# noway/nzcb-circom

Measured on AMD Instinct MI355X. Metric: PLONK proofs/sec for nzcp_live (~2^21 constraints) at 1/2/4/8 MI355X, higher is better.
Workload: dtype u32 limbs: BN254 Fr/Fq Montgomery, 8x32-bit and 9x29-bit (MSM, NTT twiddles, quotient); 1 GPU; nzcp_live fullProve: NZCPPubIdentity(1,351,0,4,2,4) witness on the GPU (600560 signals) + PLONK proof, n=2^21, nPublic=3, 2970 inputs; domain_size=2097152, n_public=3, n_constraints=1785813, n_vars=1782570, n_additions=1182010, proofs_per_gpu=140, total_proofs=140, parallelism=batch-shard x1 (no collective), proofs_in_flight_per_gpu=5

## Files before the change

### include/nzcb_internal.h

```cpp
#ifndef NZCB_INTERNAL_H
#define NZCB_INTERNAL_H

#include "nzcb.h"

#ifdef __cplusplus
extern "C" {
#endif

int nzcb_ctx_kernel_stats(nzcb_ctx* ctx, int enable, double out[4]);

int nzcb_debug_guard_check(int device, size_t* checked, int* damaged, nzcb_err* err);
int nzcb_debug_guard_selftest(int device, nzcb_err* err);

#define NZCB_FAULT_QUOTIENT 1
#define NZCB_DEBUG_GENERIC_K 2
#define NZCB_FAULT_LANE_ALLOC 3
int nzcb_debug_inject_fault(nzcb_ctx* ctx, int kind);

int nzcb_debug_signal_basis_cap(int per_constraint);
int nzcb_debug_signal_basis_info(const nzcb_ctx* ctx, uint64_t out[7]);
int nzcb_debug_commit_abc(nzcb_ctx* ctx, const uint8_t* witness, size_t n_witness, const uint8_t* blinding,
                          int signal_basis, uint8_t* out, nzcb_err* err);
int nzcb_debug_signal_rows(nzcb_ctx* ctx, int set, uint8_t* rows_out, uint32_t* signals_out, size_t cap,
                           nzcb_err* err);

int nzcb_debug_f29(int device, int op, const uint32_t* in, size_t count, uint32_t* out, nzcb_err* err);

int nzcb_debug_grand_product(int device, const uint8_t* abc , const uint8_t* sigma ,
                             const uint8_t* x , size_t n, const uint8_t* beta, const uint8_t* gamma,
                             const uint8_t* k1, const uint8_t* k2, int generic_k, uint8_t* z_out ,
                             uint8_t* totals_out , nzcb_err* err);
int nzcb_debug_div_pol1(int device, const uint8_t* p , size_t m, const uint8_t* d, const uint8_t* p0_adjust,
                        uint8_t* q_out , int* divides_out, nzcb_err* err);
int nzcb_debug_eval_many(int device, int np, const uint8_t* const* polys, const size_t* lens,
                         const uint8_t* xs , uint8_t* out , nzcb_err* err);
int nzcb_debug_quotient(int device, int power, int three, uint32_t npub, const uint8_t* abcz ,
                        const uint8_t* q , const uint8_t* s ,
                        const uint8_t* l , const uint8_t* apub , const uint8_t* beta,
                        const uint8_t* gamma, const uint8_t* alpha, const uint8_t* k1, const uint8_t* k2,
                        uint8_t* t_out , nzcb_err* err);

int nzcb_synth_setup(int power, int n_public, int n_inputs, uint64_t seed, uint32_t n_constraints,
                     const uint8_t* tau, int device, uint8_t** zkey_out, size_t* zkey_len, uint8_t** wtns_out,
                     size_t* wtns_len, nzcb_err* err);
#define NZCB_SYNTH_FREE_PUBLIC 1u
int nzcb_synth_setup_ex(int power, int n_public, int n_inputs, uint64_t seed, uint32_t n_constraints, uint32_t flags,
                        const uint8_t* tau, int device, uint8_t** zkey_out, size_t* zkey_len, uint8_t** wtns_out,
                        size_t* wtns_len, nzcb_err* err);
typedef struct nzcb_engine nzcb_engine;
nzcb_engine* nzcb_engine_create(int device, int max_log_ntt, size_t max_msm_points, nzcb_err* err);
void nzcb_engine_destroy(nzcb_engine* e);
int nzcb_engine_ntt(nzcb_engine* e, const uint8_t* in_lem, uint8_t* out_lem, int log_n, int inverse, nzcb_err* err);
int nzcb_engine_msm(nzcb_engine* e, const uint8_t* bases_lem, const uint8_t* scalars, size_t n, int scalars_mont,
                    uint8_t* out_affine, nzcb_err* err);
int nzcb_debug_ntt_coset(nzcb_engine* e, const uint8_t* in_lem, uint8_t* out_lem, int log_n, const uint8_t* c_lem,
                         int fold_len, nzcb_err* err);
int nzcb_engine_ntt_dev(nzcb_engine* e, const void* in, void* out, int log_n, int inverse, nzcb_err* err);
int nzcb_engine_msm_dev(nzcb_engine* e, const void* bases, const void* scalars, size_t n, int scalars_mont,
                        uint8_t* out_affine, nzcb_err* err);
int nzcb_engine_time_ntt(nzcb_engine* e, const void* in, void* out, int log_n, int inverse, int reps, double* ms,
                         nzcb_err* err);
int nzcb_engine_random_fr(nzcb_engine* e, void* dev_out, size_t n, uint64_t seed, nzcb_err* err);
int nzcb_engine_fixed_base(nzcb_engine* e, const void* dev_scalars_mont, size_t n, void* dev_out, nzcb_err* err);
int nzcb_engine_lagrange_basis(nzcb_engine* e, const void* dev_ptau, size_t ptau_n, int log_n, void* dev_out,
                               nzcb_err* err);
int nzcb_engine_time_msm(nzcb_engine* e, const void* bases, const void* scalars, size_t n, int scalars_mont, int reps,
                         double* ms, double* acc_ms, nzcb_err* err);
int nzcb_engine_msm_fixed_dev(nzcb_engine* e, const void* bases, size_t n_table, const void* scalars, size_t n,
                              int scalars_mont, uint8_t* out_affine, nzcb_err* err);
int nzcb_engine_msm_table_dev(nzcb_engine* e, const void* bases, size_t n_table, const void* scalars, size_t n,
                              int scalars_mont, int window, int sparse, int fold, uint8_t* out_affine,
                              nzcb_err* err);
int nzcb_debug_msm_plan(nzcb_engine* e, const void* bases, size_t n_table, const void* scalars, size_t n,
                        int scalars_mont, int window, int fold, uint32_t* info, uint32_t* offsets, size_t offsets_cap,
                        uint32_t* seg, size_t seg_cap, uint8_t* out_affine, nzcb_err* err);
int nzcb_engine_msm_sets_dev(nzcb_engine* e, const void* bases, size_t n_table, const void* const* scalars, int sets,
                             size_t n, int scalars_mont, int sparse, uint8_t* out_affine, nzcb_err* err);
int nzcb_engine_time_msm2(nzcb_engine* e, const void* bases, const void* scalars, size_t n, int scalars_mont,
                          int fixed_base, int reps, double* out, nzcb_err* err);
int nzcb_engine_fr_mul(nzcb_engine* e, const uint8_t* a_lem, const uint8_t* b_lem, uint8_t* out_lem, size_t n,
                       int field_q, nzcb_err* err);

int nzcb_engine_g1_lincomb(int device, const uint8_t* points, const uint8_t* scalars, const uint32_t* group_end,
                           size_t groups, uint8_t* out, nzcb_err* err);
int nzcb_engine_verify_batch(const uint8_t* vk, const uint8_t* proofs, const uint8_t* pubs, size_t pub_stride,
                             int n_public, int count, int transcript_public, int device, const uint8_t* seed,
                             int* valid_out, uint8_t* points_out, int* pairing_checks, nzcb_err* err);
int nzcb_debug_verify_batch_timings(double* ms, int cap);

nzcb_r1cs* nzcb_engine_r1cs_create(const uint8_t* r1cs, size_t len, int device, uint32_t long_row_threshold,
                                   int witness_tile, nzcb_err* err);
int nzcb_debug_r1cs_check_timings(double* ms, int cap);

nzcb_p256_key* nzcb_engine_p256_key_create(const uint8_t pub_xy[64], int device, int window, nzcb_err* err);
#define NZCB_P256_OP_ADD 0
#define NZCB_P256_OP_SUB 1
#define NZCB_P256_OP_MUL 2
#define NZCB_P256_OP_SQR 3
#define NZCB_P256_OP_INV 4
int nzcb_debug_p256_field(int device, int op, int field, const uint8_t* a, const uint8_t* b, size_t count,
                          uint8_t* out, nzcb_err* err);
int nzcb_debug_p256_mul2(nzcb_p256_key* k, const uint8_t* u1, const uint8_t* u2, size_t count, uint8_t* out_xy,
                         nzcb_err* err);
int nzcb_debug_p256_timings(double* ms, int cap);

int nzcb_debug_nzcp_decode_timings(double* ms, int cap);

int nzcb_engine_srs_check(int device, const uint8_t* points, uint64_t m, const uint8_t* g2, const uint8_t* seed,
                          uint32_t chunk_points, nzcb_key_finding* finding, uint8_t* lr_out ,
                          nzcb_err* err);
int nzcb_debug_key_check_timings(double* ms, int cap);

int nzcb_debug_ptau_timings(double* ms, int cap);
int nzcb_debug_ptau_batch_top(int level);

int nzcb_engine_groth16_rows(int device, int g2, const void* points, uint64_t n_points, const uint64_t* row_off,
                             uint64_t n_rows, const uint32_t* idx, const uint8_t* coefs, uint8_t* out,
                             nzcb_err* err);
int nzcb_debug_groth16_schedule(int chunk, int fan_in, int* prev_chunk, int* prev_fan_in);
int nzcb_debug_groth16_timings(double* out, int cap);

#ifdef __cplusplus
}
#endif
#endif
```

### nzcb-circom_amd/csrc/prover.hip

```cpp
#include <rocprofiler-sdk-roctx/roctx.h>
#include "devcall.h"
#include "lagrange.h"
#include "prover.h"
#include "sigbasis.h"
#include "transcript.h"

#include <cstring>
#include <cerrno>
#include <string>
#include <sys/random.h>

#include "keccak.h"

namespace nzcb {

static constexpr int kT = 256;
static constexpr uint32_t kZeroRef = 0xffffffffu;

__global__ void k_wit_to_mont(const Fr* __restrict__ in, Fr* __restrict__ out, size_t n) {
  size_t i = (size_t)blockIdx.x * blockDim.x + threadIdx.x;
  if (i >= n) return;
  out[i] = (i == 0) ? Fr::zero() : to_mont(in[i]);
}

__global__ void k_additions(const AddRec* __restrict__ recs, uint32_t count, Fr* __restrict__ wit) {
  uint32_t i = blockIdx.x * blockDim.x + threadIdx.x;
  if (i >= count) return;
  const AddRec r = recs[i];
  Fr a = r.ai == kZeroRef ? Fr::zero() : wit[r.ai];
  Fr b = r.bi == kZeroRef ? Fr::zero() : wit[r.bi];
  wit[r.dst] = r.ac * a + r.bc * b;
}


__global__ void k_build_abc(const uint32_t* __restrict__ am, const uint32_t* __restrict__ bm,
                            const uint32_t* __restrict__ cm, uint32_t nc, uint32_t n, const Fr* __restrict__ wit,
                            uint32_t nvars, Fr* __restrict__ A, Fr* __restrict__ B, Fr* __restrict__ C,
                            uint32_t npub, Fr* __restrict__ mb_apub, Fr* __restrict__ mb_pubw) {
  uint32_t i = blockIdx.x * blockDim.x + threadIdx.x;
  if (i < npub) {
    host_put(mb_pubw + i, 1 + i < nvars ? wit[1 + i] : Fr::zero());
  }
  if (i >= n) {
    if (i < npub) host_put_done();
    return;
  }
  Fr a = Fr::zero(), b = Fr::zero(), c = Fr::zero();
  if (i < nc) {
    uint32_t ia = am[i], ib = bm[i], ic = cm[i];
    if (ia < nvars) a = wit[ia];
    if (ib < nvars) b = wit[ib];
    if (ic < nvars) c = wit[ic];
  }
  A[i] = a;
  B[i] = b;
  C[i] = c;
  if (i < npub) {
    host_put(mb_apub + i, a);
    host_put_done();
  }
}

__global__ void k_tops(const Fr* __restrict__ pa, const Fr* __restrict__ pb, const Fr* __restrict__ pc,
                       const Fr* __restrict__ pz, size_t n, const uint32_t* __restrict__ flags, Fr* __restrict__ mb) {
  const int t = threadIdx.x;
  if (t < 24) {
    const int k = t / 6, j = t % 6;
    const Fr* src = k == 0 ? pa + (n - 4) : k == 1 ? pb + (n - 4) : k == 2 ? pc + (n - 4) : pz + (n - 3);
    host_put(mb + t, src[j]);
  } else if (t == 24) {
    Fr f = Fr::zero();
    f.v[0] = *flags;
    host_put(mb + 24, f);
  }
  host_put_done();
}

struct BlindIdx {
  int idx[3];
  int count;
};

__global__ void k_blind(Fr* pol, size_t n, const Fr* __restrict__ bl, BlindIdx bi) {
  if (threadIdx.x != 0 || blockIdx.x != 0) return;
  for (int k = 0; k < bi.count; k++) {
    Fr b = bl[bi.idx[k]];
    pol[n + k] = b;
    pol[k] = pol[k] - b;
  }
}

__global__ void k_abc_tail(Fr* A, Fr* B, Fr* C, size_t n, const Fr* __restrict__ bl) {
  if (threadIdx.x != 0 || blockIdx.x != 0) return;
  A[n] = bl[2];
  A[n + 1] = bl[1];
  B[n] = bl[4];
  B[n + 1] = bl[3];
  C[n] = bl[6];
  C[n + 1] = bl[5];
}

__global__ void k_sig_stage(const uint32_t* __restrict__ idx, uint32_t stride, uint32_t c0, uint32_t c1, uint32_t c2,
                            const Fr* __restrict__ wit, const Fr* __restrict__ bl, Fr* __restrict__ out) {
  const size_t i = (size_t)blockIdx.x * blockDim.x + threadIdx.x;
  if (i >= (size_t)3 * stride) return;
  const uint32_t set = (uint32_t)(i / stride), j = (uint32_t)(i - (size_t)set * stride);
  const uint32_t cnt = set == 0 ? c0 : set == 1 ? c1 : c2;
  Fr v = Fr::zero();
  if (j < cnt) v = from_mont(wit[idx[i]]);
  else if (j == cnt) v = from_mont(bl[2 + 2 * set]);
  else if (j == cnt + 1) v = from_mont(bl[1 + 2 * set]);
  out[i] = v;
}

static bool signal_commit_enabled() {
  static const bool v = [] {
    const char* e = std::getenv("NZCB_SIGNAL_COMMIT");
    return !e || std::atoi(e) != 0;
  }();
  return v;
}

static bool abc_sets_enabled() {
  static const bool v = [] {
    const char* e = std::getenv("NZCB_ABC_SETS");
    return !e || std::atoi(e) != 0;
  }();
  return v;
}

static bool lagrange_commit_enabled() {
  static const bool v = [] {
    const char* e = std::getenv("NZCB_LAGRANGE_COMMIT");
    return !e || std::atoi(e) != 0;
  }();
  return v;
}

__device__ __forceinline__ Fr root4(const Fr* __restrict__ lo, const Fr* __restrict__ hi, size_t i) {
  return lo[i & 4095] * hi[i >> 12];
}

struct PermArgs {
  F29 beta, beta_s;
  F29 k1beta, k1beta_s, k2beta, k2beta_s;
  F29 gamma256;
  int k23;
};
static void shoup_pair(const Fr& c, F29& w, F29& ws) {
  Fr m = c;
  for (int k = 0; k < 5; k++) m = m + m;
  w = split29(from_mont(c));
  ws = mul_lo261(split29(m), f29_const(Fr29::NINV));
}

static F29 fr29_operand(Fr c) {
  for (int k = 0; k < 5; k++) c = c + c;
  return split29(c);
}

#ifndef NZ_KPER
#define NZ_KPER 4
#endif
static constexpr int kPer = NZ_KPER;
static constexpr int kTileN = kT * kPer;
static constexpr int kStageWords = kTileN * 8 + kTileN / 4;

__device__ __forceinline__ int stage_word(int e) { return e * 8 + e / 4; }

template <class F, class U>
__device__ __forceinline__ void stage_use(F&& f, size_t base, size_t len, uint32_t* lds, U&& use) {
#pragma unroll
  for (int k = 0; k < kPer; k++) {
    const int e = k * kT + (int)threadIdx.x;
    const size_t g = base + (size_t)e;
    const Fr v = g < len ? f(g) : Fr::zero();
#pragma unroll
    for (int w = 0; w < 8; w++) lds[stage_word(e) + w] = v.v[w];
  }
  __syncthreads();
#pragma unroll
  for (int j = 0; j < kPer; j++) {
    const int e = kPer * (int)threadIdx.x + j;
    Fr x;
#pragma unroll
    for (int w = 0; w < 8; w++) x.v[w] = lds[stage_word(e) + w];
    use(j, x);
  }
  __syncthreads();
}
template <class F>
__device__ __forceinline__ void stage_in(F&& f, size_t base, size_t len, uint32_t* lds, Fr (&out)[kPer]) {
  stage_use(f, base, len, lds, [&](int j, const Fr& x) { out[j] = x; });
}

__device__ __forceinline__ void stage_out(const Fr (&v)[kPer], size_t base, size_t len, uint32_t* lds, Fr* dst) {
#pragma unroll
  for (int j = 0; j < kPer; j++) {
    const int e = kPer * (int)threadIdx.x + j;
#pragma unroll
    for (int w = 0; w < 8; w++) lds[stage_word(e) + w] = v[j].v[w];
  }
  __syncthreads();
#pragma unroll
  for (int k = 0; k < kPer; k++) {
    const int e = k * kT + (int)threadIdx.x;
    const size_t g = base + (size_t)e;
    Fr x;
#pragma unroll
    for (int w = 0; w < 8; w++) x.v[w] = lds[stage_word(e) + w];
    if (g < len) dst[g] = x;
  }
  __syncthreads();
}

__device__ __forceinline__ Fr shfl_fr(const Fr& v, int src) {
  Fr o;
#pragma unroll
  for (int w = 0; w < 8; w++) o.v[w] = __shfl(v.v[w], src, 64);
  return o;
}
__device__ __forceinline__ F29 shfl_fr(const F29& v, int src) {
  F29 o;
#pragma unroll
  for (int w = 0; w < 9; w++) o.v[w] = __shfl(v.v[w], src, 64);
  return o;
}
struct MulOp {
  using T = Fr;
  static constexpr bool kCheap = false;
  __device__ Fr operator()(const Fr& a, const Fr& b) const { return a * b; }
  __device__ static Fr id() { return Fr::one(); }
};
struct AddOp {
  using T = Fr;
  static constexpr bool kCheap = true;
  __device__ Fr operator()(const Fr& a, const Fr& b) const { return a + b; }
  __device__ static Fr id() { return Fr::zero(); }
};
struct Mul29Op {
  using T = F29;
  static constexpr bool kCheap = false;
  __device__ F29 operator()(const F29& a, const F29& b) const { return mul29<Fr29>(a, b); }
  __device__ static F29 id() { return f29_const(Fr29::ONE); }
};
template <bool kSuffix, class Op, int NT = kT>
__device__ __forceinline__ typename Op::T block_scan_excl(const typename Op::T& v, typename Op::T* sh,
                                                          typename Op::T* total) {
  using T = typename Op::T;
  constexpr int NW = NT / 64;
  static_assert(NW >= 1 && NW <= 64 && NT % 64 == 0, "whole waves, at most 64");
  const Op op;
  const int lane = (int)(threadIdx.x & 63), wv = (int)(threadIdx.x >> 6);
  T inc = v;
#pragma unroll
  for (int d = 1; d < 64; d <<= 1) {
    const int src = kSuffix ? lane + d : lane - d;
    const T o = shfl_fr(inc, src & 63);
    if (kSuffix ? lane + d < 64 : lane >= d) inc = op(inc, o);
  }
  T ex = shfl_fr(inc, (kSuffix ? lane + 1 : lane - 1) & 63);
  if (kSuffix ? lane == 63 : lane == 0) ex = Op::id();
  if (kSuffix ? lane == 0 : lane == 63) sh[wv] = inc;
  __syncthreads();
  if constexpr (NW <= 4 && Op::kCheap) {
#pragma unroll
    for (int k = 0; k < NW; k++)
      if (kSuffix ? k > wv : k < wv) ex = op(ex, sh[k]);
    if (total && threadIdx.x == 0) {
      T t = sh[0];
#pragma unroll
      for (int k = 1; k < NW; k++) t = op(t, sh[k]);
      *total = t;
    }
    __syncthreads();
  } else {
    T tot_all = Op::id();
    if (wv == 0) {
      T w = lane < NW ? sh[lane] : Op::id();
#pragma unroll
      for (int d = 1; d < NW; d <<= 1) {
        const int src = kSuffix ? lane + d : lane - d;
        const T o = shfl_fr(w, src & 63);
        if (kSuffix ? lane + d < NW : (lane >= d && lane < NW)) w = op(w, o);
      }
      T wex = shfl_fr(w, (kSuffix ? lane + 1 : lane - 1) & 63);
      if (kSuffix ? lane == NW - 1 : lane == 0) wex = Op::id();
      tot_all = shfl_fr(w, kSuffix ? 0 : NW - 1);
      if (lane < NW) sh[lane] = wex;
    }
    __syncthreads();
    ex = op(ex, sh[wv]);
    if (total && threadIdx.x == 0) *total = tot_all;
    __syncthreads();
  }
  return ex;
}
__device__ __forceinline__ Fr block_prod_excl(const Fr& v, Fr* sh, Fr& total) {
  return block_scan_excl<false, MulOp>(v, sh, &total);
}
__device__ __forceinline__ Fr block_prod_excl_suffix(const Fr& v, Fr* sh) {
  return block_scan_excl<true, MulOp>(v, sh, nullptr);
}
__device__ __forceinline__ Fr block_sum_excl_suffix(const Fr& v, Fr* sh, Fr& total) {
  return block_scan_excl<true, AddOp>(v, sh, &total);
}

#ifndef NZ_PERM_WAVES
#define NZ_PERM_WAVES 2
#endif
__device__ __forceinline__ F29 add3_nn29(const F29& a, const F29& b, const F29& c) {
  F29 r;
#pragma unroll
  for (int l = 0; l < 9; l++) r.v[l] = a.v[l] + b.v[l] + c.v[l];
  return r;
}
__global__ void __launch_bounds__(kT) __attribute__((amdgpu_waves_per_eu(NZ_PERM_WAVES, 8)))
k_perm_tile(const Fr* __restrict__ A, const Fr* __restrict__ B, const Fr* __restrict__ C,
            const Fr* __restrict__ sig_h, size_t n, const Fr* __restrict__ w_h, PermArgs pa, Fr* __restrict__ Z,
            Fr* __restrict__ ntot, Fr* __restrict__ dtot) {
  __shared__ uint32_t stg[kStageWords];
  __shared__ F29 sh[kT / 64];
  const int tid = threadIdx.x;
  const size_t base = (size_t)blockIdx.x * kTileN;
  const size_t e0 = base + (size_t)kPer * tid;
  const F29 beta = pa.beta, beta_s = pa.beta_s, gamma = pa.gamma256;
  const bool k23 = pa.k23 != 0;
  F29 num[kPer], den[kPer], bw[kPer], bs[kPer];
#pragma unroll 1
  for (int k = 0; k < 3; k++) {
    stage_use([&](size_t g) { return sig_h[(size_t)k * n + g]; }, base, n, stg,
              [&](int j, const Fr& x) { bs[j] = mul_shoup(split29(x), beta, beta_s); });
    if (k == 0 || !k23) {
      const F29 kb = k == 0 ? beta : (k == 1 ? pa.k1beta : pa.k2beta);
      const F29 kbs = k == 0 ? beta_s : (k == 1 ? pa.k1beta_s : pa.k2beta_s);
#pragma unroll
      for (int j = 0; j < kPer; j++) bw[j] = mul_shoup(split29(e0 + j < n ? w_h[e0 + j] : Fr::zero()), kb, kbs);
    }
    const Fr* col = k == 0 ? A : B;
    if (k == 2) col = C;
    stage_use([&](size_t g) { return col[g]; }, base, n, stg,
              [&](int j, const Fr& x) {
                F29 kbw = bw[j];
                if (k23 && k == 1) {
#pragma unroll
                  for (int l = 0; l < 9; l++) kbw.v[l] = bw[j].v[l] << 1;
                } else if (k23 && k == 2) {
#pragma unroll
                  for (int l = 0; l < 9; l++) kbw.v[l] = (bw[j].v[l] << 1) + bw[j].v[l];
                }
                const F29 xs = split29(x);
                if (k == 0) {
                  num[j] = add3_29(xs, kbw, gamma);
                  den[j] = add3_29(xs, bs[j], gamma);
                } else {
                  num[j] = mul29<Fr29>(num[j], add3_nn29(xs, kbw, gamma));
                  den[j] = mul29<Fr29>(den[j], add3_nn29(xs, bs[j], gamma));
                }
              });
  }
  const F29 one = f29_const(Fr29::ONE);
#pragma unroll
  for (int j = 0; j < kPer; j++)
    if (e0 + j >= n) num[j] = den[j] = one;
  F29 ntl = num[0];
#pragma unroll
  for (int j = 1; j < kPer; j++) ntl = mul29<Fr29>(ntl, num[j]);
  bs[kPer - 1] = den[kPer - 1];
#pragma unroll
  for (int j = kPer - 2; j >= 0; j--) bs[j] = mul29<Fr29>(bs[j + 1], den[j]);
  F29 nt;
  const F29 np = block_scan_excl<false, Mul29Op>(ntl, sh, &nt);
  const F29 ds = block_scan_excl<true, Mul29Op>(bs[0], sh, nullptr);
  F29 pre = mul29<Fr29>(mul29<Fr29>(np, ds), f29_const(Fr29::C256));
  Fr out[kPer];
#pragma unroll
  for (int j = 0; j < kPer; j++) {
    out[j] = join_fr29(mul29<Fr29>(pre, bs[j]));
    if (j + 1 < kPer) pre = mul29<Fr29>(pre, num[j]);
  }
  stage_out(out, base, n, stg, Z);
  if (tid == 0) {
    ntot[blockIdx.x] = fr_from261(nt);
    dtot[blockIdx.x] = fr_from261(mul29<Fr29>(ds, bs[0]));
  }
}

__global__ void __launch_bounds__(1024)
k_perm_factors(const Fr* __restrict__ ntot, const Fr* __restrict__ dtot, int ntiles, Fr* __restrict__ F,
               Fr* __restrict__ totals) {
  __shared__ Fr sh[1024 / 64];
  const int tid = threadIdx.x;
  const int per = (ntiles + 1023) / 1024;
  const int t0 = min(tid * per, ntiles), t1 = min(t0 + per, ntiles);
  Fr pn = Fr::one(), pd = Fr::one();
  for (int t = t0; t < t1; t++) {
    pn = pn * ntot[t];
    pd = pd * dtot[t];
  }
  Fr nall, dall;
  const Fr npre = block_scan_excl<false, MulOp, 1024>(pn, sh, &nall);
  const Fr dsuf = block_scan_excl<true, MulOp, 1024>(pd, sh, &dall);
  if (tid == 0) {
    host_put(totals, nall);
    host_put(totals + 1, dall);
    host_put_done();
  }
  Fr run = npre;
  for (int t = t0; t < t1; t++) {
    F[t] = run;
    run = run * ntot[t];
  }
  Fr sd = dsuf;
  for (int t = t1 - 1; t >= t0; t--) {
    F[t] = F[t] * sd;
    sd = sd * dtot[t];
  }
}

__global__ void __launch_bounds__(kT)
k_apply_tiles(Fr* __restrict__ x, size_t m, const Fr* __restrict__ F, Fr inv_d) {
  const Fr f = F[blockIdx.x] * inv_d;
  const size_t base = (size_t)blockIdx.x * kTileN + threadIdx.x;
#pragma unroll
  for (int k = 0; k < kPer; k++) {
    const size_t i = base + (size_t)k * kT;
    if (i < m) x[i] = x[i] * f;
  }
}

struct LinTab {
  Fr P[kT + 1];
  Fr Pinv[kT + 1];
  Fr dp[kPer + 1];
};
static_assert(sizeof(LinTab) % sizeof(Fr) == 0, "LinTab is stored as Fr words");

template <bool kWrite>
__global__ void __launch_bounds__(kT)
k_lin_tile(const Fr* __restrict__ src, size_t m, const LinTab* __restrict__ tab, const Fr* __restrict__ carry,
           Fr* __restrict__ out) {
  __shared__ uint32_t stg[kStageWords];
  __shared__ Fr sh[kT / 64];
  const int tid = threadIdx.x;
  const size_t base = (size_t)blockIdx.x * kTileN;
  Fr x[kPer];
  stage_in([&](size_t g) { return src[g + 1]; }, base, m - 1, stg, x);
  const Fr d = tab->dp[1];
  Fr y = Fr::zero();
#pragma unroll
  for (int j = kPer - 1; j >= 0; j--) {
    y = x[j] + d * y;
    x[j] = y;
  }
  Fr total;
  Fr ex = block_sum_excl_suffix(y * tab->P[tid], sh, total);
  if (!kWrite) {
    if (tid == 0) out[blockIdx.x] = total;
    return;
  }
  if (carry) ex = ex + carry[blockIdx.x + 1] * tab->P[kT];
  const Fr next = ex * tab->Pinv[tid + 1];
#pragma unroll
  for (int j = 0; j < kPer; j++) x[j] = x[j] + tab->dp[kPer - j] * next;
  stage_out(x, base, m, stg, out);
}

__global__ void k_pow_tiles(Fr D, Fr Di, int count, Fr* __restrict__ Q, Fr* __restrict__ Qinv) {
  const int T = blockIdx.x * blockDim.x + threadIdx.x;
  if (T >= count) return;
  Fr a = Fr::one(), b = Fr::one(), pa = D, pb = Di;
  for (int e = T; e; e >>= 1) {
    if (e & 1) {
      a = a * pa;
      b = b * pb;
    }
    pa = sqr(pa);
    pb = sqr(pb);
  }
  Q[T] = a;
  Qinv[T] = b;
}

__global__ void __launch_bounds__(1024) k_tile_heads(Fr* __restrict__ h, int m, const Fr* __restrict__ Q,
                                                     const Fr* __restrict__ Qinv) {
  __shared__ Fr sh[1024 / 64];
  const int tid = threadIdx.x;
  const int per = (m + 1023) / 1024;
  const int t0 = min(tid * per, m), t1 = min(t0 + per, m);
  Fr run = Fr::zero();
  for (int T = t0; T < t1; T++) run = run + h[T] * Q[T];
  Fr suf = block_scan_excl<true, AddOp, 1024>(run, sh, nullptr);
  for (int T = t1 - 1; T >= t0; T--) {
    suf = suf + h[T] * Q[T];
    h[T] = suf * Qinv[T];
  }
  if (tid == 0) h[m] = Fr::zero();
}

__global__ void k_stride4(const Fr* __restrict__ src, size_t n, Fr* __restrict__ dst) {
  const size_t i = (size_t)blockIdx.x * blockDim.x + threadIdx.x;
  if (i < n) dst[i] = src[4 * i];
}

struct QArgs {
  Fr beta, gamma, alpha, alpha2, bk1, bk2;
  Fr zhinv[4];
};

__global__ void __launch_bounds__(kT)
k_quotient_coset(const Fr* __restrict__ A, const Fr* __restrict__ B, const Fr* __restrict__ C,
                 const Fr* __restrict__ Z, const Fr* __restrict__ cq, const Fr* __restrict__ cs,
                 const Fr* __restrict__ cl, uint32_t npub, const Fr* __restrict__ Apub, size_t n,
                 const Fr* __restrict__ xlo, const Fr* __restrict__ xhi, QArgs q, Fr* __restrict__ T) {
  const size_t n4 = 4 * n;
  size_t i = (size_t)blockIdx.x * blockDim.x + threadIdx.x;
  if (i >= n4) return;
  const Fr a = A[i], b = B[i], c = C[i];
  const Fr x = xlo[i & 4095] * xhi[i >> 12];
  Fr gate = a * b * cq[i] + a * cq[n4 + i] + b * cq[2 * n4 + i] + c * cq[3 * n4 + i] + cq[4 * n4 + i];
  for (uint32_t j = 0; j < npub; j++) gate = gate - cl[j * n4 + i] * Apub[j];
  const Fr z = Z[i];
  const Fr bx = q.beta * x;
  Fr num = (a + bx + q.gamma) * (b + q.bk1 * x + q.gamma);
  num = num * (c + q.bk2 * x + q.gamma) * z;
  Fr den = (a + q.beta * cs[i] + q.gamma) * (b + q.beta * cs[n4 + i] + q.gamma);
  den = den * (c + q.beta * cs[2 * n4 + i] + q.gamma) * Z[(i + 4) & (n4 - 1)];
  const Fr e4 = (z - Fr::one()) * cl[i] * q.alpha2;
  T[i] = (gate + q.alpha * (num - den) + e4) * q.zhinv[i & 3];
}

constexpr uint32_t kQ29MaxPub = 8;

static bool quot3_enabled() {
  static const bool on = [] {
    const char* e = std::getenv("NZCB_QUOT3");
    return !(e && e[0] == '0');
  }();
  return on;
}
struct QArgs29 {
  F29 beta, bk1, bk2, alpha2, zhinv[4];
  F29 gamma, negone;
  int k23;
  F29 alpha;
};

template <int K>
__device__ __forceinline__ F29 q29_pi_chunk(const Fr* __restrict__ cl, const Fr* __restrict__ Apub, uint32_t j0,
                                            size_t n4, size_t i) {
  F29 pa[K], pb[K];
#pragma unroll
  for (int k = 0; k < K; k++) {
    pa[k] = split29(cl[(size_t)(j0 + k) * n4 + i]);
    pb[k] = split29(neg(Apub[j0 + k]));
  }
  return mulsum29<Fr29, K>(pa, pb);
}

__device__ __forceinline__ F29 q29_pi(const Fr* __restrict__ cl, const Fr* __restrict__ Apub, uint32_t j0,
                                      uint32_t cnt, size_t n4, size_t i) {
  switch (cnt) {
    case 1: return q29_pi_chunk<1>(cl, Apub, j0, n4, i);
    case 2: return q29_pi_chunk<2>(cl, Apub, j0, n4, i);
    case 3: return q29_pi_chunk<3>(cl, Apub, j0, n4, i);
    default: return q29_pi_chunk<4>(cl, Apub, j0, n4, i);
  }
}

template <bool THREE>
__global__ void __launch_bounds__(kT) __attribute__((amdgpu_waves_per_eu(4, 8)))
k_quotient_coset29(const Fr* __restrict__ A, const Fr* __restrict__ B, const Fr* __restrict__ C,
                   const Fr* __restrict__ Z, const Fr* __restrict__ cq, const Fr* __restrict__ cs,
                   const Fr* __restrict__ cl, uint32_t npub, const Fr* __restrict__ Apub, size_t n,
                   const Fr* __restrict__ xlo, const Fr* __restrict__ xhi, const Fr* __restrict__ bxlo, QArgs29 q,
                   Fr* __restrict__ T) {
  const size_t n4 = (THREE ? 3 : 4) * n;
  size_t i = (size_t)blockIdx.x * blockDim.x + threadIdx.x;
  if (i >= n4) return;
  size_t ix, izw;
  int cj;
  if (THREE) {
    const int lg = __ffsll((long long)n) - 1;
    const size_t j = i >> lg, m = i & (n - 1);
    ix = 4 * m + j;
    izw = j * n + ((m + 1) & (n - 1));
    cj = (int)j;
  } else {
    ix = i;
    izw = (i + 4) & (n4 - 1);
    cj = (int)(i & 3);
  }
  const F29 a = split29(A[i]), b = split29(B[i]), c = split29(C[i]);
  F29 gate;
  {
    const F29 ga[4] = {mul29<Fr29>(a, b), a, b, c};
    const F29 gb[4] = {split29(cq[i]), split29(cq[n4 + i]), split29(cq[2 * n4 + i]), split29(cq[3 * n4 + i])};
    gate = add29(mulsum29<Fr29, 4>(ga, gb), split29(cq[4 * n4 + i]));
  }
  if (npub > 0) gate = add29(gate, q29_pi(cl, Apub, 0, npub < 4 ? npub : 4, n4, i));
  if (npub > 4) gate = add29(gate, q29_pi(cl, Apub, 4, npub - 4, n4, i));
  const F29 z = split29(Z[i]);
  const bool bxt = THREE && q.k23;
  const F29 x = mul29<Fr29>(split29((bxt ? bxlo : xlo)[ix & 4095]), split29(xhi[ix >> 12]));
  const F29 bx = bxt ? x : mul29<Fr29>(q.beta, x);
  const F29 bx2 = q.k23 ? add29(bx, bx) : mul29<Fr29>(q.bk1, x);
  const F29 bx3 = q.k23 ? add29(bx2, bx) : mul29<Fr29>(q.bk2, x);
  const F29 f1 = add29(add29(a, bx), q.gamma);
  const F29 f2 = add29(add29(b, bx2), q.gamma);
  const F29 f3 = add29(add29(c, bx3), q.gamma);
  const F29 num = mul29<Fr29>(mul29<Fr29>(mul29<Fr29>(f1, f2), f3), z);
  const F29 g1 = add29(add29(a, mul29<Fr29>(q.beta, split29(cs[i]))), q.gamma);
  const F29 g2 = add29(add29(b, mul29<Fr29>(q.beta, split29(cs[n4 + i]))), q.gamma);
  const F29 g3 = add29(add29(c, mul29<Fr29>(q.beta, split29(cs[2 * n4 + i]))), q.gamma);
  const F29 den = mul29<Fr29>(mul29<Fr29>(mul29<Fr29>(g1, g2), g3), split29(Z[izw]));
  const F29 pa[2] = {q.alpha, q.alpha2};
  const F29 pb[2] = {sub29(num, den, Fr29::K2), mul29<Fr29>(add29(z, q.negone), split29(cl[i]))};
  const F29 S = add29(gate, mulsum29<Fr29, 2>(pa, pb));
  T[i] = THREE ? canon_fr29(S) : join_fr29(mul29<Fr29>(S, q.zhinv[cj]));
}

__global__ void __launch_bounds__(kT)
k_beta_xlo(const Fr* __restrict__ xlo, F29 beta, size_t count, Fr* __restrict__ bxlo) {
  const size_t i = (size_t)blockIdx.x * blockDim.x + threadIdx.x;
  if (i < count) bxlo[i] = join_fr29(mul29<Fr29>(beta, split29(xlo[i])));
}

__global__ void __launch_bounds__(kT)
k_gate_h(const Fr* __restrict__ A, const Fr* __restrict__ B, const Fr* __restrict__ C, const Fr* __restrict__ qh,
         size_t n, uint32_t npub, uint32_t* __restrict__ flags) {
  const size_t m = (size_t)blockIdx.x * blockDim.x + threadIdx.x;
  if (m >= n) return;
  const Fr a = A[m], b = B[m], c = C[m];
  Fr g = qh[m] * a * b + qh[n + m] * a + qh[2 * n + m] * b + qh[3 * n + m] * c + qh[4 * n + m];
  if (m < npub) g = g - a;
  if (!g.is_zero()) atomicOr(flags, 1u);
}

struct T3Args {
  Fr c0[6], c1[6], c2[6], q3[6];
  Fr i4, two_over_d, inv_d2;
};
__global__ void __launch_bounds__(kT)
k_t_combine(const Fr* __restrict__ V, size_t n, T3Args a, Fr* __restrict__ t) {
  const size_t k = (size_t)blockIdx.x * blockDim.x + threadIdx.x;
  if (k >= n) return;
  Fr v0 = V[k], v1 = V[n + k], v2 = V[2 * n + k];
  if (k < 6) {
    v0 = v0 - a.c0[k];
    v1 = v1 - a.c1[k];
    v2 = v2 - a.c2[k];
  }
  const Fr sm = v0 + v2, dl = v0 - v2, im = dl * a.i4, v12 = v1 + v1;
  t[k] = sm + v12 - im;
  t[n + k] = dl * a.two_over_d;
  t[2 * n + k] = (sm - v12 + im) * a.inv_d2;
  if (k < 6) t[3 * n + k] = a.q3[k];
}

__global__ void k_root_n(Fr* __restrict__ out, const Fr* __restrict__ rlo, const Fr* __restrict__ rhi, size_t n) {
  const size_t i = (size_t)blockIdx.x * blockDim.x + threadIdx.x;
  if (i < n) out[i] = root4(rlo, rhi, 4 * i);
}

__global__ void k_fault_bump(Fr* x) {
  if (threadIdx.x == 0) x[0] = x[0] + Fr::one();
}

__global__ void k_dbl_pow(Fr* __restrict__ x, size_t m, int e) {
  size_t i = (size_t)blockIdx.x * blockDim.x + threadIdx.x;
  if (i >= m) return;
  Fr v = x[i];
  for (int k = 0; k < e; k++) v = v + v;
  x[i] = v;
}

static F29 f29_exp(Fr v, int extra) {
  for (int k = 0; k < extra; k++) v = v + v;
  return split29(v);
}

static constexpr int kEvalMax = 8;
static constexpr int kEvalBits = 16;
struct EvalSet {
  const Fr* p[kEvalMax];
  uint64_t len[kEvalMax];
  Fr x[kEvalMax];
  Fr x4096[kEvalMax];
  F29 x29[kEvalMax];
  F29 y29[kEvalMax];
  int np;
  int nbits;
};

__device__ __forceinline__ F29 fr29_operand_dev(Fr c) {
#pragma unroll
  for (int k = 0; k < 5; k++) c = c + c;
  return split29(c);
}

static constexpr int kEvalChunk2 = 16;

__global__ void __launch_bounds__(kT) k_eval_pows(EvalSet es, F29* __restrict__ pw, Fr* __restrict__ pw2) {
  const int j = blockIdx.x, t = threadIdx.x;
  Fr a = Fr::one(), q = es.x[j];
  for (int e = t; e; e >>= 1) {
    if (e & 1) a = a * q;
    q = q * q;
  }
  pw[(size_t)j * kT + t] = fr29_operand_dev(a);
  if (t < es.nbits) {
    Fr z = es.x4096[j];
    for (int k = 0; k < t; k++) z = z * z;
    pw2[j * kEvalBits + t] = z;
  }
}

__device__ __forceinline__ Fr block_sum_fr(const Fr& v, Fr* sh) {
  Fr x = v;
#pragma unroll
  for (int m = 32; m >= 1; m >>= 1) x = x + shfl_fr(x, (int)(threadIdx.x & 63) ^ m);
  if ((threadIdx.x & 63) == 0) sh[threadIdx.x >> 6] = x;
  __syncthreads();
  Fr t = sh[0];
#pragma unroll
  for (int k = 1; k < kT / 64; k++) t = t + sh[k];
  __syncthreads();
  return t;
}

template <int NP>
__global__ void __launch_bounds__(kT) k_eval_multi(EvalSet es, const F29* __restrict__ pw, const Fr* __restrict__ pw2,
                                                   Fr* __restrict__ partial, int nblocks) {
  static_assert(NP <= kEvalMax && kEvalMax <= 4 * (kT / 64), "one 16-lane group per point");
  __shared__ Fr sh[kT / 64];
  __shared__ Fr bpow[kEvalMax];
  __shared__ Fr bsum[kEvalMax];
  {
    const int l = (int)(threadIdx.x & 63), k = l & 15, j = 4 * (int)(threadIdx.x >> 6) + (l >> 4);
    Fr f = Fr::one();
    if (j < NP && k < es.nbits && ((blockIdx.x >> k) & 1u)) f = pw2[j * kEvalBits + k];
    for (int m = 8; m >= 1; m >>= 1) f = f * shfl_fr(f, l ^ m);
    if (j < NP && k == 0) bpow[j] = f;
  }
  const size_t s = (size_t)blockIdx.x * kT * kEvalChunk2 + threadIdx.x;
  F29 acc[NP];
#pragma unroll
  for (int j = 0; j < NP; j++)
#pragma unroll
    for (int l = 0; l < 9; l++) acc[j].v[l] = 0;
  for (int m = kEvalChunk2 - 1; m >= 0; m--) {
    const size_t i = s + (size_t)m * kT;
#pragma unroll
    for (int j = 0; j < NP; j++)
      if (i < es.len[j]) {
        const F29 t = mul29<Fr29>(acc[j], es.y29[j]), c = split29(es.p[j][i]);
#pragma unroll
        for (int l = 0; l < 9; l++) acc[j].v[l] = t.v[l] + c.v[l];
      }
  }
#pragma unroll
  for (int j = 0; j < NP; j++) {
    const Fr r = block_sum_fr(join_fr29(mul29<Fr29>(acc[j], pw[(size_t)j * kT + threadIdx.x])), sh);
    if (threadIdx.x == 0) bsum[j] = r;
  }
  if (threadIdx.x < NP) partial[(size_t)threadIdx.x * nblocks + blockIdx.x] = bsum[threadIdx.x] * bpow[threadIdx.x];
}

__global__ void __launch_bounds__(kT) k_eval_sum(const Fr* __restrict__ partial, int nblocks, Fr* __restrict__ out) {
  __shared__ Fr sh[kT / 64];
  const int j = blockIdx.x;
  Fr acc = Fr::zero();
  for (int b = (int)threadIdx.x; b < nblocks; b += kT) acc = acc + partial[(size_t)j * nblocks + b];
  const Fr r = block_sum_fr(acc, sh);
  if (threadIdx.x == 0) {
    host_put(out + j, r);
    host_put_done();
  }
}

struct RArgs {
  Fr coefz, coef_ab, ea, eb, ec, coefs3;
};

__global__ void k_pol_r(const Fr* __restrict__ pz, const Fr* __restrict__ qm, const Fr* __restrict__ ql,
                        const Fr* __restrict__ qr, const Fr* __restrict__ qo, const Fr* __restrict__ qc,
                        const Fr* __restrict__ s3, size_t n, RArgs r, Fr* __restrict__ out) {
  size_t i = (size_t)blockIdx.x * blockDim.x + threadIdx.x;
  if (i >= n + 3) return;
  Fr v = r.coefz * pz[i];
  if (i < n) {
    v = v + r.coef_ab * qm[i] + r.ea * ql[i] + r.eb * qr[i] + r.ec * qo[i] + qc[i];
    v = v - r.coefs3 * s3[i];
  }
  out[i] = v;
}

struct WArgs {
  Fr xim, xi2m, v[7], w0sub;
};

__global__ void k_pol_wxi(const Fr* __restrict__ t, const Fr* __restrict__ pr, const Fr* __restrict__ pa,
                          const Fr* __restrict__ pb, const Fr* __restrict__ pc, const Fr* __restrict__ s1,
                          const Fr* __restrict__ s2, size_t n, WArgs wa, Fr* __restrict__ out) {
  size_t i = (size_t)blockIdx.x * blockDim.x + threadIdx.x;
  if (i >= n + 6) return;
  Fr w = wa.xi2m * t[2 * n + i];
  if (i < n) w = w + wa.xim * t[n + i] + t[i];
  if (i < n + 3) w = w + wa.v[1] * pr[i];
  if (i < n + 2) w = w + wa.v[2] * pa[i] + wa.v[3] * pb[i] + wa.v[4] * pc[i];
  if (i < n) w = w + wa.v[5] * s1[i] + wa.v[6] * s2[i];
  if (i == 0) w = w - wa.w0sub;
  out[i] = w;
}

__global__ void k_div_check(const Fr* __restrict__ src, Fr p0_adjust, const Fr* __restrict__ q, Fr d,
                            uint32_t* flags, uint32_t bit, uint32_t* __restrict__ mb_flags) {
  if (threadIdx.x || blockIdx.x) return;
  Fr p0 = src[0] - p0_adjust;
  if (!(p0 + d * q[0]).is_zero()) atomicOr(flags, bit);
  host_put(mb_flags, *flags);
  host_put_done();
}

__global__ void k_root_table(Fr* __restrict__ out, Fr base, Fr scale, size_t count) {
  size_t i = (size_t)blockIdx.x * blockDim.x + threadIdx.x;
  if (i >= count) return;
  out[i] = scale * pow_u64(base, i);
}

__global__ void k_factor29_table(F29* __restrict__ out, const Fr* __restrict__ lo, const Fr* __restrict__ hi, Fr scale,
                                 size_t count) {
  size_t i = (size_t)blockIdx.x * blockDim.x + threadIdx.x;
  if (i >= count) return;
  Fr v = lo[i & 4095] * hi[i >> 12] * scale;
#pragma unroll
  for (int k = 0; k < 5; k++) v = v + v;
  out[i] = split29(v);
}

static std::string fr_dec(const Fr& m) {
  Fr x = from_mont(m);
  uint32_t v[8];
  std::memcpy(v, x.v, 32);
  std::string s;
  bool nz = true;
  while (nz) {
    uint64_t rem = 0;
    nz = false;
    for (int i = 7; i >= 0; i--) {
      uint64_t cur = (rem << 32) | v[i];
      v[i] = (uint32_t)(cur / 10);
      rem = cur % 10;
      if (v[i]) nz = true;
    }
    s.push_back((char)('0' + rem));
  }
  return std::string(s.rbegin(), s.rend());
}

static Fr fr_small(uint64_t k) {
  Fr x = Fr::zero();
  x.v[0] = (uint32_t)k;
  x.v[1] = (uint32_t)(k >> 32);
  return to_mont(x);
}

static bool k_is_23(const Fr& k1, const Fr& k2) { return k1 == fr_small(2) && k2 == fr_small(3); }

static PermArgs perm_args(const Fr& beta, const Fr& gamma, const Fr& k1, const Fr& k2, bool generic_k) {
  PermArgs pa;
  shoup_pair(beta, pa.beta, pa.beta_s);
  shoup_pair(k1 * beta, pa.k1beta, pa.k1beta_s);
  shoup_pair(k2 * beta, pa.k2beta, pa.k2beta_s);
  pa.gamma256 = f29_exp(gamma, 0);
  pa.k23 = !generic_k && k_is_23(k1, k2) ? 1 : 0;
  return pa;
}

static size_t perm_tiles(size_t n) { return (n + kTileN - 1) / kTileN; }

static void perm_launch(const Fr* A, const Fr* B, const Fr* C, const Fr* sig_h, size_t n, const Fr* w_h,
                        const PermArgs& pa, Fr* Z, Fr* scan, Fr* totals, hipStream_t s) {
  const size_t ntiles = perm_tiles(n);
  if (ntiles > 1024 * 64) throw Error(NZCB_ERR_INTERNAL, "round 2: domain too large for the tile factors");
  Fr* ntot = scan;
  Fr* dtot = ntot + ntiles;
  Fr* fac = dtot + ntiles;
  hipLaunchKernelGGL(k_perm_tile, dim3((unsigned)ntiles), dim3(kT), 0, s, A, B, C, sig_h, n, w_h, pa, Z, ntot, dtot);
  hipLaunchKernelGGL(k_perm_factors, dim3(1), dim3(1024), 0, s, (const Fr*)ntot, (const Fr*)dtot, (int)ntiles, fac,
                     totals);
  NZ_HIP(hipGetLastError());
}

static void perm_apply(Fr* Z, size_t n, const Fr* scan, const Fr& den_total, hipStream_t s) {
  const size_t ntiles = perm_tiles(n);
  hipLaunchKernelGGL(k_apply_tiles, dim3((unsigned)ntiles), dim3(kT), 0, s, Z, n, scan + 2 * ntiles,
                     inverse(den_total));
  NZ_HIP(hipGetLastError());
}

static QArgs quot_args(const Fr& beta, const Fr& gamma, const Fr& alpha, const Fr& k1, const Fr& k2,
                       const Fr (&zh_inv)[4]) {
  QArgs q;
  q.beta = beta;
  q.gamma = gamma;
  q.alpha = alpha;
  q.alpha2 = alpha * alpha;
  q.bk1 = beta * k1;
  q.bk2 = beta * k2;
  for (int k = 0; k < 4; k++) q.zhinv[k] = zh_inv[k];
  return q;
}
static QArgs29 quot_args29(const Fr& beta, const Fr& gamma, const Fr& alpha, const Fr& k1, const Fr& k2,
                           const Fr (&zh_inv)[4]) {
  QArgs29 q29;
  q29.beta = f29_exp(beta, 5);
  q29.k23 = k_is_23(k1, k2) ? 1 : 0;
  q29.bk1 = f29_exp(beta * k1, 5);
  q29.bk2 = f29_exp(beta * k2, 5);
  q29.alpha2 = f29_exp(alpha * alpha, 5);
  for (int k = 0; k < 4; k++) q29.zhinv[k] = f29_exp(zh_inv[k], 5);
  q29.gamma = f29_exp(gamma, 0);
  q29.negone = f29_exp(neg(Fr::one()), 0);
  q29.alpha = f29_exp(alpha, 20);
  return q29;
}

static void root_table(DevBuf<Fr>& out, size_t cnt, const Fr& base, const Fr& scale, hipStream_t s) {
  out.alloc(cnt);
  hipLaunchKernelGGL(k_root_table, dim3(grid_for(cnt, kT)), dim3(kT), 0, s, out.p, base, scale, cnt);
  NZ_HIP(hipGetLastError());
}

static void quot_x_tables(int power, DevBuf<Fr>& x_lo, DevBuf<Fr>& root_hi, Fr (&zh_inv)[4], hipStream_t s) {
  const size_t n = (size_t)1 << power, n4 = 4 * n;
  const Fr w4 = fr_root_of_unity(power + 2), g = fr_small(5), one = Fr::one();
  root_table(x_lo, 4096, w4, g, s);
  root_table(root_hi, (n4 + 4095) / 4096, pow_u64(w4, 4096), one, s);
  Fr gn = pow_u64(g, n), w4n = pow_u64(w4, n), p = gn;
  for (int k = 0; k < 4; k++) {
    zh_inv[k] = inverse(p - one);
    p = p * w4n;
  }
}

static void quot29_prescale(Fr* cq, Fr* cl, uint32_t nl, size_t npts, Fr* x_lo, hipStream_t s) {
  auto scale = [&](Fr* p, size_t m, int e) {
    hipLaunchKernelGGL(k_dbl_pow, dim3(grid_for(m, kT, 1u << 30)), dim3(kT), 0, s, p, m, e);
  };
  scale(cq, npts, 10);
  scale(cq + npts, 3 * npts, 5);
  scale(cl, (size_t)nl * npts, 5);
  scale(x_lo, 4096, 5);
  NZ_HIP(hipGetLastError());
}

static void quot_launch(bool three, const Fr* A4, const Fr* B4, const Fr* C4, const Fr* Z4, const Fr* cq, const Fr* cs,
                        const Fr* cl, uint32_t npub, const Fr* Apub, size_t n, const Fr* x_lo, const Fr* root_hi,
                        Fr* bx_lo, const Fr& beta, const Fr& gamma, const Fr& alpha, const Fr& k1, const Fr& k2,
                        const Fr (&zh_inv)[4], Fr* T, hipStream_t s) {
  if (three && npub > kQ29MaxPub) throw Error(NZCB_ERR_INTERNAL, "round 3: three cosets with too many public inputs");
  if (npub > kQ29MaxPub) {
    const QArgs q = quot_args(beta, gamma, alpha, k1, k2, zh_inv);
    hipLaunchKernelGGL(k_quotient_coset, dim3(grid_for(4 * n, kT, 1u << 30)), dim3(kT), 0, s, A4, B4, C4, Z4, cq, cs,
                       cl, npub, Apub, n, x_lo, root_hi, q, T);
  } else {
    const QArgs29 q29 = quot_args29(beta, gamma, alpha, k1, k2, zh_inv);
    if (three) {
      if (q29.k23)
        hipLaunchKernelGGL(k_beta_xlo, dim3(grid_for(4096, kT)), dim3(kT), 0, s, x_lo, q29.beta, (size_t)4096, bx_lo);
      hipLaunchKernelGGL((k_quotient_coset29<true>), dim3(grid_for(3 * n, kT, 1u << 30)), dim3(kT), 0, s, A4, B4, C4,
                         Z4, cq, cs, cl, npub, Apub, n, x_lo, root_hi, (const Fr*)bx_lo, q29, T);
    } else {
      hipLaunchKernelGGL((k_quotient_coset29<false>), dim3(grid_for(4 * n, kT, 1u << 30)), dim3(kT), 0, s, A4, B4, C4,
                         Z4, cq, cs, cl, npub, Apub, n, x_lo, root_hi, (const Fr*)nullptr, q29, T);
    }
  }
  NZ_HIP(hipGetLastError());
}

static EvalSet eval_set(int np, const Fr* const* polys, const size_t* lens, const Fr* xs, size_t* nblocks_out) {
  if (np < 1 || np > kEvalMax) throw Error(NZCB_ERR_INTERNAL, "eval_many: bad count");
  EvalSet es{};
  size_t maxlen = 0;
  for (int j = 0; j < np; j++) {
    es.p[j] = polys[j];
    es.len[j] = lens[j];
    es.x[j] = xs[j];
    es.x29[j] = fr29_operand(xs[j]);
    es.y29[j] = fr29_operand(pow_u64(xs[j], kT));
    es.x4096[j] = pow_u64(xs[j], (uint64_t)kT * kEvalChunk2);
    maxlen = std::max(maxlen, lens[j]);
  }
  es.np = np;
  const size_t nblocks = (maxlen + (size_t)kT * kEvalChunk2 - 1) / ((size_t)kT * kEvalChunk2);
  if (nblocks > ((size_t)1 << kEvalBits)) throw Error(NZCB_ERR_INTERNAL, "eval_many: polynomial too long");
  es.nbits = 1;
  while (((size_t)1 << es.nbits) < nblocks) es.nbits++;
  *nblocks_out = nblocks;
  return es;
}

static void eval_launch(const EvalSet& es, size_t nblocks, Fr* part, F29* pw, Fr* pw2, Fr* out, hipStream_t s) {
  const int np = es.np;
  hipLaunchKernelGGL(k_eval_pows, dim3((unsigned)np), dim3(kT), 0, s, es, pw, pw2);
  if (np == 7)
    hipLaunchKernelGGL(k_eval_multi<7>, dim3((unsigned)nblocks), dim3(kT), 0, s, es, (const F29*)pw, (const Fr*)pw2,
                       part, (int)nblocks);
  else if (np == 1)
    hipLaunchKernelGGL(k_eval_multi<1>, dim3((unsigned)nblocks), dim3(kT), 0, s, es, (const F29*)pw, (const Fr*)pw2,
                       part, (int)nblocks);
  else
    throw Error(NZCB_ERR_INTERNAL, "eval_many: 1 or 7 evaluations");
  NZ_HIP(hipGetLastError());
  hipLaunchKernelGGL(k_eval_sum, dim3(np), dim3(kT), 0, s, (const Fr*)part, (int)nblocks, out);
  NZ_HIP(hipGetLastError());
}

static void lin_tables_build(LinTab& t, const Fr& d, LinTab* dev, Fr* q, int qn, hipStream_t s) {
  t.dp[0] = Fr::one();
  for (int j = 1; j <= kPer; j++) t.dp[j] = t.dp[j - 1] * d;
  const Fr dk = t.dp[kPer], dki = inverse(dk);
  t.P[0] = t.Pinv[0] = Fr::one();
  for (int i = 1; i <= kT; i++) {
    t.P[i] = t.P[i - 1] * dk;
    t.Pinv[i] = t.Pinv[i - 1] * dki;
  }
  NZ_HIP(hipMemcpyAsync(dev, &t, sizeof(LinTab), hipMemcpyHostToDevice, s));
  hipLaunchKernelGGL(k_pow_tiles, dim3((qn + 255) / 256), dim3(256), 0, s, t.P[kT], t.Pinv[kT], qn, q, q + qn);
  NZ_HIP(hipGetLastError());
}

static size_t lin_tiles(size_t m) { return (m + kTileN - 1) / kTileN; }

static void div_pol1_launch(const Fr* src, size_t m, const LinTab* lt, const Fr& d, const Fr* q, size_t qn, Fr* heads,
                            const Fr& p0_adjust, Fr* dst, uint32_t* flags, uint32_t flag_bit, uint32_t* mb_flags,
                            hipStream_t s) {
  const size_t ntiles = lin_tiles(m);
  if (ntiles + 1 > qn) throw Error(NZCB_ERR_INTERNAL, "divPol1: more tiles than its power tables");
  hipLaunchKernelGGL(k_lin_tile<false>, dim3((unsigned)ntiles), dim3(kT), 0, s, src, m, lt, (const Fr*)nullptr, heads);
  hipLaunchKernelGGL(k_tile_heads, dim3(1), dim3(1024), 0, s, heads, (int)ntiles, q, q + qn);
  NZ_HIP(hipGetLastError());
  hipLaunchKernelGGL(k_lin_tile<true>, dim3((unsigned)ntiles), dim3(kT), 0, s, src, m, lt, (const Fr*)heads, dst);
  hipLaunchKernelGGL(k_div_check, dim3(1), dim3(64), 0, s, src, p0_adjust, (const Fr*)dst, d, flags, flag_bit,
                     mb_flags);
  NZ_HIP(hipGetLastError());
}

Prover::~Prover() {
  for (int i = 0; i < kSlots; i++) {
    if (aux[i]) {
      (void)hipStreamSynchronize(aux[i]);
      (void)hipStreamDestroy(aux[i]);
    }
    if (ready[i]) (void)hipEventDestroy(ready[i]);
  }
  if (side_ready) (void)hipEventDestroy(side_ready);
  if (side_done) (void)hipEventDestroy(side_done);
  if (pows_done) (void)hipEventDestroy(pows_done);
  if (top_host) (void)hipHostFree(top_host);
  for (auto& e : span_ev) {
    (void)hipEventDestroy(e.first);
    (void)hipEventDestroy(e.second);
  }
}

size_t Prover::span_begin(int kind, hipStream_t s) {
  if (spans_used == span_ev.size()) {
    hipEvent_t a, b;
    NZ_HIP(hipEventCreate(&a));
    NZ_HIP(hipEventCreate(&b));
    span_ev.emplace_back(a, b);
    span_kind.push_back(0);
  }
  span_kind[spans_used] = kind;
  NZ_HIP(hipEventRecord(span_ev[spans_used].first, s));
  return spans_used++;
}
void Prover::span_end(size_t i, hipStream_t s) { NZ_HIP(hipEventRecord(span_ev[i].second, s)); }
void Prover::span_totals(double* msm_ms, double* ntt_ms) {
  *msm_ms = *ntt_ms = 0;
  for (size_t i = 0; i < spans_used; i++) {
    NZ_HIP(hipEventSynchronize(span_ev[i].second));
    float ms = 0;
    NZ_HIP(hipEventElapsedTime(&ms, span_ev[i].first, span_ev[i].second));
    (span_kind[i] ? *ntt_ms : *msm_ms) += ms;
  }
}

MsmShard::~MsmShard() {
  (void)hipSetDevice(device);
  for (auto& s : st)
    if (s) {
      (void)hipStreamSynchronize(s);
      (void)hipStreamDestroy(s);
    }
}

void Prover::set_msm_devices(const std::vector<int>& devices) {
  GuardScope guards;
  if (devices.empty() || devices[0] != eng->device)
    throw Error(NZCB_ERR_ARG, "msm devices must start with the context's device");
  shards.clear();
  own_hi = own_lhi = 0;
  const size_t N = ptau.n;
  const size_t L = lcommit ? ltau.n : 0;
  const size_t k = devices.size();
  if (k == 1) return;
  own_hi = N / k;
  own_lhi = L / k;
  for (size_t i = 1; i < k; i++) {
    auto sh = std::make_unique<MsmShard>();
    sh->device = devices[i];
    sh->lo = N * i / k;
    sh->hi = N * (i + 1) / k;
    sh->llo = L * i / k;
    sh->lhi = L * (i + 1) / k;
    const size_t cnt = sh->hi - sh->lo, lcnt = sh->lhi - sh->llo, mx = std::max(cnt, lcnt);
    NZ_HIP(hipSetDevice(sh->device));
    for (int j = 0; j < MsmShard::kSlots; j++) {
      NZ_HIP(hipStreamCreateWithFlags(&sh->st[j], hipStreamNonBlocking));
      sh->sc[j].reset(new MsmScratch());
      sh->sc[j]->init(mx, true, 1, false);
      sh->scal[j].alloc(mx);
    }
    {
      DevBuf<G1Affine> part(cnt);
      NZ_HIP(hipMemcpyPeerAsync(part.p, sh->device, ptau.p + sh->lo, eng->device, cnt * sizeof(G1Affine), sh->st[0]));
      sh->table.build(part.p, cnt, fixed_base_window(), sh->st[0]);
      NZ_HIP(hipStreamSynchronize(sh->st[0]));
    }
    if (lcnt) {
      DevBuf<G1Affine> part(lcnt);
      NZ_HIP(hipMemcpyPeerAsync(part.p, sh->device, ltau.p + sh->llo, eng->device, lcnt * sizeof(G1Affine),
                                sh->st[0]));
      sh->ltable.build(part.p, lcnt, lagrange_window(), sh->st[0]);
      sh->ltable.sparse = lagrange_sparse();
      NZ_HIP(hipStreamSynchronize(sh->st[0]));
    }
    shards.push_back(std::move(sh));
  }
  NZ_HIP(hipSetDevice(eng->device));
}

double Prover::ms_since(std::chrono::steady_clock::time_point t0) {
  return std::chrono::duration<double, std::milli>(std::chrono::steady_clock::now() - t0).count();
}

Prover::Prover(const uint8_t* zkey_bytes, size_t len, int device) {
  GuardScope guards;
  Zkey z = parse_zkey(zkey_bytes, len);
  n = z.domainSize;
  n4 = 4 * n;
  power = z.power;
  nVars = z.nVars;
  nPublic = z.nPublic;
  nAdditions = z.nAdditions;
  nConstraints = z.nConstraints;
  if (nAdditions > nVars) throw Error(NZCB_ERR_FORMAT, "nAdditions > nVars");
  nWit = nVars - nAdditions;
  k1 = z.k1;
  k2 = z.k2;
  wn = fr_root_of_unity(power);
  w2 = fr_root_of_unity(2);
  eng.reset(new Engine(device, power + 2, 0));
  init_slots();
  hipStream_t s = st();
  auto up = [&](auto& buf, const Section& sec) {
    using T = typename std::remove_reference<decltype(*buf.p)>::type;
    buf.alloc(sec.len / sizeof(T) ? sec.len / sizeof(T) : 1);
    if (sec.len) NZ_HIP(hipMemcpyAsync(buf.p, sec.p, sec.len, hipMemcpyHostToDevice, s));
  };
  up(ptau, z.ptau);
  ptab.build(ptau.p, ptau.n, fixed_base_window(), s, true);
  lcommit = lagrange_commit_enabled() && ptau.n >= (size_t)n + 2;
  if (lcommit) {
    ltau.alloc((size_t)n + 2);
    lagrange_basis(ptau.p, ptau.n, power, ltau.p, s);
    ltab.build(ltau.p, ltau.n, lagrange_window(), s);
    ltab.sparse = lagrange_sparse();
  }
  up(qm, z.qm);
  up(ql, z.ql);
  up(qr, z.qr);
  up(qo, z.qo);
  up(qc, z.qc);
  up(sigma, z.sigma);
  sig_h.alloc((size_t)3 * n);
  w_h.alloc(n);
  for (int k = 0; k < 3; k++)
    hipLaunchKernelGGL(k_stride4, dim3(grid_for(n, kT, 1u << 30)), dim3(kT), 0, s, sigma.p + (size_t)k * 5 * n + n,
                       (size_t)n, sig_h.p + (size_t)k * n);
  NZ_HIP(hipGetLastError());
  up(lagrange, z.lagrange);
  up(amap, z.amap);
  up(bmap, z.bmap);
  up(cmap, z.cmap);
  {
    std::vector<uint32_t> level(nAdditions, 0);
    std::vector<AddRec> recs(nAdditions);
    uint32_t maxlev = 0;
    for (uint32_t k = 0; k < nAdditions; k++) {
      const uint8_t* p = z.additions.p + (size_t)k * 72;
      AddRec r;
      std::memcpy(&r.ai, p, 4);
      std::memcpy(&r.bi, p + 4, 4);
      std::memcpy(r.ac.v, p + 8, 32);
      std::memcpy(r.bc.v, p + 40, 32);
      r.dst = nWit + k;
      r.pad = 0;
      uint32_t lv = 0;
      for (uint32_t* ref : {&r.ai, &r.bi}) {
        if (*ref >= nVars) *ref = kZeroRef;
        else if (*ref >= nWit) {
          uint32_t kk = *ref - nWit;
          if (kk >= k) *ref = kZeroRef;
          else lv = std::max(lv, level[kk] + 1);
        }
      }
      level[k] = lv;
      maxlev = std::max(maxlev, lv);
      recs[k] = r;
    }
    std::vector<uint32_t> cnt(maxlev + 2, 0);
    for (uint32_t k = 0; k < nAdditions; k++) cnt[level[k] + 1]++;
    for (uint32_t l = 1; l < cnt.size(); l++) cnt[l] += cnt[l - 1];
    add_level_start.assign(cnt.begin(), cnt.end());
    std::vector<AddRec> sorted(nAdditions);
    std::vector<uint32_t> cur(cnt.begin(), cnt.end());
    for (uint32_t k = 0; k < nAdditions; k++) sorted[cur[level[k]]++] = recs[k];
    adds.alloc(nAdditions ? nAdditions : 1);
    if (nAdditions)
      NZ_HIP(hipMemcpyAsync(adds.p, sorted.data(), nAdditions * sizeof(AddRec), hipMemcpyHostToDevice, s));
    NZ_HIP(hipStreamSynchronize(s));
  }
  if (lcommit && signal_commit_enabled() && abc_sets_enabled()) build_signal_basis(z);
  Fr w4 = fr_root_of_unity(power + 2);
  size_t nlo = 4096, nhi = (n4 + 4095) / 4096;
  const Fr one = Fr::one();
  auto table = [&](DevBuf<Fr>& out, size_t cnt, const Fr& base, const Fr& scale) { root_table(out, cnt, base, scale, s); };
  table(root_lo, nlo, w4, one);
  quot_x_tables(power, x_lo, root_hi, zh_inv, s);
  hipLaunchKernelGGL(k_root_n, dim3(grid_for(n, kT, 1u << 30)), dim3(kT), 0, s, w_h.p, root_lo.p, root_hi.p,
                     (size_t)n);
  NZ_HIP(hipGetLastError());
  const Fr g = fr_small(5), gi = inverse(g);
  table(g_lo, nlo, g, one);
  table(g_hi, nhi, pow_u64(g, 4096), one);
  table(gi_lo, nlo, gi, one);
  table(gi_hi, nhi, pow_u64(gi, 4096), one);
  quot3 = quot3_enabled() && nPublic <= kQ29MaxPub && power >= 6;
  {
    const Fr two = one + one;
    g29.alloc((size_t)n + 8);
    hipLaunchKernelGGL(k_factor29_table, dim3(grid_for((size_t)n + 8, kT, 1u << 30)), dim3(kT), 0, s, g29.p, g_lo.p,
                       g_hi.p, one, (size_t)n + 8);
    if (!quot3) {
      gi29.alloc(n4);
      hipLaunchKernelGGL(k_factor29_table, dim3(grid_for(n4, kT, 1u << 30)), dim3(kT), 0, s, gi29.p, gi_lo.p,
                         gi_hi.p, inverse(pow_u64(two, (uint64_t)power + 2)), (size_t)n4);
    }
    NZ_HIP(hipGetLastError());
  }
  alloc_workspace();
  if (quot3) {
    q_h.alloc((size_t)5 * n);
    const DevBuf<Fr>* qs[5] = {&qm, &ql, &qr, &qo, &qc};
    for (int k = 0; k < 5; k++)
      hipLaunchKernelGGL(k_stride4, dim3(grid_for(n, kT, 1u << 30)), dim3(kT), 0, s, qs[k]->p + n, (size_t)n,
                         q_h.p + (size_t)k * n);
    NZ_HIP(hipGetLastError());
  }
  if (quot3) {
    const size_t nhi3 = (n + 4095) / 4096;
    ctw3.alloc((size_t)3 * (n - 1));
    itw3.alloc((size_t)3 * n);
    const Fr inv4n = inverse(fr_small(n4));
    DevBuf<Fr> lo, hi;
    for (int j = 0; j < 3; j++) {
      const Fr cj = g * pow_u64(w4, (uint64_t)j), cji = inverse(cj);
      d3[j] = pow_u64(cj, n);
      ntt_coset_twiddles(eng->ntt_tables, cj, power, ctw3.p + (size_t)j * (n - 1), s);
      table(lo, nlo, cji, one);
      table(hi, nhi3, pow_u64(cji, 4096), one);
      hipLaunchKernelGGL(k_factor29_table, dim3(grid_for(n, kT, 1u << 30)), dim3(kT), 0, s, itw3.p + (size_t)j * n,
                         lo.p, hi.p, inv4n * zh_inv[j], (size_t)n);
      NZ_HIP(hipGetLastError());
      NZ_HIP(hipStreamSynchronize(s));
    }
    for (int k = 0; k < 3; k++)
      NZ_HIP(hipMemcpy(sig_top[k], sigma.p + (size_t)k * 5 * n + (n - 4), 4 * sizeof(Fr), hipMemcpyDeviceToHost));
  }
  if (quot3) {
    const uint32_t nl = nPublic > 0 ? nPublic : 1;
    const size_t n3 = (size_t)3 * n;
    cq3.alloc(5 * n3);
    cs3.alloc(3 * n3);
    cl3.alloc(nl * n3);
    auto coset3 = [&](const Fr* coefs, Fr* out) {
      for (int j = 0; j < 3; j++) {
        NttIo io;
        io.in_len = n;
        io.tw = ctw3.p + (size_t)j * (n - 1);
        ntt(eng->ntt_tables, coefs, out + (size_t)j * n, power, false, s, nullptr, &io);
      }
    };
    const DevBuf<Fr>* qs[5] = {&qm, &ql, &qr, &qo, &qc};
    for (int k = 0; k < 5; k++) coset3(qs[k]->p, cq3.p + (size_t)k * n3);
    for (int k = 0; k < 3; k++) coset3(sigma.p + (size_t)k * 5 * n, cs3.p + (size_t)k * n3);
    for (uint32_t j = 0; j < nl; j++) coset3(lagrange.p + (size_t)j * 5 * n, cl3.p + (size_t)j * n3);
    NZ_HIP(hipGetLastError());
    quot29_prescale(cq3.p, cl3.p, nl, n3, x_lo.p, s);
  } else {
    const uint32_t nl = nPublic > 0 ? nPublic : 1;
    cq.alloc((size_t)5 * n4);
    cs.alloc((size_t)3 * n4);
    cl.alloc((size_t)nl * n4);
    auto coset_eval = [&](const Fr* coefs, Fr* out) {
      NttIo io;
      io.in_len = n;
      io.in_f = g29.p;
      ntt(eng->ntt_tables, coefs, out, power + 2, false, s, nullptr, &io);
    };
    const DevBuf<Fr>* qs[5] = {&qm, &ql, &qr, &qo, &qc};
    for (int k = 0; k < 5; k++) coset_eval(qs[k]->p, cq.p + (size_t)k * n4);
    for (int k = 0; k < 3; k++) coset_eval(sigma.p + (size_t)k * 5 * n, cs.p + (size_t)k * n4);
    for (uint32_t j = 0; j < nl; j++) coset_eval(lagrange.p + (size_t)j * 5 * n, cl.p + (size_t)j * n4);
    NZ_HIP(hipGetLastError());
    if (nPublic <= kQ29MaxPub) quot29_prescale(cq.p, cl.p, nl, n4, x_lo.p, s);
  }
  NZ_HIP(hipStreamSynchronize(s));
}

void Prover::build_signal_basis(const Zkey& z) {
  hipStream_t s = st();
  if (z.additions.len < (uint64_t)nAdditions * 72 || z.amap.len < (uint64_t)nConstraints * 4 ||
      z.bmap.len < (uint64_t)nConstraints * 4 || z.cmap.len < (uint64_t)nConstraints * 4) {
    sig_note = "signal basis: the key's maps are shorter than its header says; A, B, C are committed from the "
               "Lagrange basis";
    return;
  }
  NZ_HIP(hipStreamSynchronize(s));
  SigBasis sb = sig_basis_build(eng->device, ltau.p, n, nWit, nVars, nConstraints, z.additions.p, nAdditions,
                                z.amap.p, z.bmap.p, z.cmap.p, (size_t)n + 2);
  sig_terms = sb.terms;
  if (!sb.ok) {
    sig_note = sb.note;
    return;
  }
  for (int k = 0; k < 3; k++) sig_cnt[k] = sb.cnt[k];
  sig_stride = sb.stride;
  DevBuf<G1Affine> bases(sb.bases.size());
  NZ_HIP(hipMemcpyAsync(bases.p, sb.bases.data(), sb.bases.size() * sizeof(G1Affine), hipMemcpyHostToDevice, s));
  sig_idx.alloc(sb.idx.size());
  NZ_HIP(hipMemcpyAsync(sig_idx.p, sb.idx.data(), sb.idx.size() * sizeof(uint32_t), hipMemcpyHostToDevice, s));
  stab.build(bases.p, bases.n, lagrange_window(), s);
  stab.sparse = lagrange_sparse();
  NZ_HIP(hipStreamSynchronize(s));
  sigcommit = true;
}

void Prover::init_slots() {
  for (int i = 0; i < kSlots; i++) {
    msc[i].reset(new MsmScratch());
#ifdef NZCB_AB_GENERIC
    msc[i]->init((size_t)n + 6, true, i == 0 ? 3 : 1, true);
#else
    msc[i]->init((size_t)n + 6, true, i == 0 ? 3 : 1, false);
#endif
    NZ_HIP(hipStreamCreateWithFlags(&aux[i], hipStreamNonBlocking));
    NZ_HIP(hipEventCreateWithFlags(&ready[i], hipEventDisableTiming));
  }
  NZ_HIP(hipEventCreateWithFlags(&side_ready, hipEventDisableTiming));
  NZ_HIP(hipEventCreateWithFlags(&side_done, hipEventDisableTiming));
  NZ_HIP(hipEventCreateWithFlags(&pows_done, hipEventDisableTiming));
  mb_apub = kMbEvals + kMbEvalMax;
  mb_pubw = mb_apub + nPublic;
  mb_words = mb_pubw + nPublic;
  NZ_HIP(hipHostMalloc((void**)&top_host, mb_words * sizeof(Fr), hipHostMallocCoherent));
  std::memset((void*)top_host, 0, mb_words * sizeof(Fr));
}

void Prover::alloc_workspace() {
  wit.alloc(nVars ? nVars : 1);
  wtns_in.alloc(nWit ? nWit : 1);
  A.alloc(n + 2); B.alloc(n + 2); C.alloc(n + 2); Z.alloc(n);
  if (sigcommit) sig_scal.alloc(3 * sig_stride);
  pol_a.alloc(n + 2); pol_b.alloc(n + 2); pol_c.alloc(n + 2); pol_z.alloc(n + 3);
  const size_t ne = quot3 ? (size_t)3 * n : n4;
  A4.alloc(ne); B4.alloc(ne); C4.alloc(ne); Z4.alloc(ne);
  T.alloc(ne); Tz.alloc(ne); t.alloc(quot3 ? ne + 6 : n4);
  if (quot3) bx_lo.alloc(4096);
  pol_r.alloc(n + 3); pol_wxi.alloc(n + 6); pol_wxiw.alloc(n + 3);
  blind.alloc(13);
  scan_tmp.alloc(3 * ((size_t)n / kTileN + 2) + 64);
  lin_qn = (size_t)n / kTileN + 3;
  lin_tab.alloc(2 * sizeof(LinTab) / sizeof(Fr) + 4 * lin_qn);
  lin_host.resize(2 * sizeof(LinTab) / sizeof(Fr));
  size_t nblocks = ((size_t)3 * n + 6 + (size_t)kT * kEvalChunk2 - 1) / ((size_t)kT * kEvalChunk2) + 1;
  eval_part.alloc((size_t)kEvalMax * nblocks + kEvalMax);
  eval_pw.alloc((size_t)kEvalMax * kT + (kEvalMax * kEvalBits * sizeof(Fr) + sizeof(F29) - 1) / sizeof(F29));
  host_part.resize(std::max<size_t>(nblocks, kEvalMax));
  flags.p = (uint32_t*)(blind.p + 12);
  flags.n = 1;
  flags.owned = false;
  const int zlog = quot3 ? power : power + 2;
  if (zlog > 8) ntt_scr2.alloc((size_t)9 << zlog);
}

Prover::Prover(const Prover& pk, int lane) {
  GuardScope guards;
  lane_id = lane;
  n = pk.n; n4 = pk.n4; nVars = pk.nVars; nPublic = pk.nPublic; nAdditions = pk.nAdditions;
  nConstraints = pk.nConstraints; nWit = pk.nWit; power = pk.power;
  k1 = pk.k1; k2 = pk.k2; wn = pk.wn; w2 = pk.w2;
  add_level_start = pk.add_level_start;
  transcript_public = pk.transcript_public;
  for (int k = 0; k < 4; k++) zh_inv[k] = pk.zh_inv[k];
  NZ_HIP(hipSetDevice(pk.eng->device));
  eng.reset(new Engine(pk.eng->device, power + 2, 0));
  init_slots();
  ptau.alias(pk.ptau);
  ptab.q.alias(pk.ptab.q);
  ptab.n = pk.ptab.n; ptab.stride = pk.ptab.stride; ptab.c = pk.ptab.c; ptab.nw = pk.ptab.nw;
  ptab.mont_folded = pk.ptab.mont_folded;
  lcommit = pk.lcommit;
  ltau.alias(pk.ltau);
  ltab.q.alias(pk.ltab.q);
  ltab.n = pk.ltab.n; ltab.stride = pk.ltab.stride; ltab.c = pk.ltab.c; ltab.nw = pk.ltab.nw;
  ltab.sparse = pk.ltab.sparse;
  sigcommit = pk.sigcommit;
  sig_note = pk.sig_note;
  sig_terms = pk.sig_terms;
  sig_stride = pk.sig_stride;
  for (int k = 0; k < 3; k++) sig_cnt[k] = pk.sig_cnt[k];
  sig_idx.alias(pk.sig_idx);
  stab.q.alias(pk.stab.q);
  stab.n = pk.stab.n; stab.stride = pk.stab.stride; stab.c = pk.stab.c; stab.nw = pk.stab.nw;
  stab.sparse = pk.stab.sparse;
  qm.alias(pk.qm); ql.alias(pk.ql); qr.alias(pk.qr); qo.alias(pk.qo); qc.alias(pk.qc);
  sigma.alias(pk.sigma); sig_h.alias(pk.sig_h); q_h.alias(pk.q_h); w_h.alias(pk.w_h); lagrange.alias(pk.lagrange);
  amap.alias(pk.amap); bmap.alias(pk.bmap); cmap.alias(pk.cmap); adds.alias(pk.adds);
  root_lo.alias(pk.root_lo); root_hi.alias(pk.root_hi); x_lo.alias(pk.x_lo);
  g_lo.alias(pk.g_lo); g_hi.alias(pk.g_hi); gi_lo.alias(pk.gi_lo); gi_hi.alias(pk.gi_hi);
  g29.alias(pk.g29); gi29.alias(pk.gi29);
  cq.alias(pk.cq); cs.alias(pk.cs); cl.alias(pk.cl);
  quot3 = pk.quot3;
  cq3.alias(pk.cq3); cs3.alias(pk.cs3); cl3.alias(pk.cl3);
  ctw3.alias(pk.ctw3); itw3.alias(pk.itw3);
  for (int j = 0; j < 3; j++) d3[j] = pk.d3[j];
  std::memcpy(sig_top, pk.sig_top, sizeof(sig_top));
  alloc_workspace();
}

void Prover::launch_gate_check(hipStream_t s) {
  hipLaunchKernelGGL(k_gate_h, dim3(grid_for(n, kT, 1u << 30)), dim3(kT), 0, s, A.p, B.p, C.p, q_h.p, (size_t)n,
                     nPublic, flags.p);
  NZ_HIP(hipGetLastError());
}

void Prover::copy_tops(hipStream_t s) {
  hipLaunchKernelGGL(k_tops, dim3(1), dim3(32), 0, s, pol_a.p, pol_b.p, pol_c.p, pol_z.p, (size_t)n,
                     (const uint32_t*)flags.p, top_host);
  NZ_HIP(hipGetLastError());
  NZ_HIP(hipStreamSynchronize(s));
  if (top_host[kMbFlags].v[0] & 1u) throw Error(NZCB_ERR_T_DIV, "T Polynomial is not divisible");
}

void Prover::round3_quot3(const Fr& beta, const Fr& gamma, const Fr& alpha, hipStream_t s) {
  const bool side = lcommit;
  if (side) copy_tops(s);
  quot_launch(true, A4.p, B4.p, C4.p, Z4.p, cq3.p, cs3.p, cl3.p, nPublic, A.p, (size_t)n, x_lo.p, root_hi.p, bx_lo.p,
              beta, gamma, alpha, k1, k2, zh_inv, T.p, s);
  if (!side) launch_gate_check(s);
  for (int j = 0; j < 3; j++) {
    NttIo io;
    io.out_f = itw3.p + (size_t)j * n;
    io.out_f_has_scale = true;
    {
      const size_t sp = prof_gpu ? span_begin(1, s) : 0;
      ntt(eng->ntt_tables, T.p + (size_t)j * n, Tz.p + (size_t)j * n, power, true, s, nullptr, &io);
      if (prof_gpu) span_end(sp, s);
    }
  }
  NZ_HIP(hipGetLastError());
  if (!side) copy_tops(s);
  Fr top[4][6];
  std::memcpy(top, top_host, sizeof(top));
  Fr p1[4][6], p2[4][6];
  const Fr w = wn, wi = inverse(wn);
  const Fr wpow[6] = {w * w, w, Fr::one(), wi, wi * wi, wi * wi * wi};
  for (int u = 0; u < 6; u++) {
    for (int f3 = 0; f3 < 3; f3++) {
      p1[f3][u] = top[f3][5 - u];
      p2[f3][u] = top[f3][5 - u];
      if (u >= 2) p2[f3][u] = p2[f3][u] + beta * sig_top[f3][5 - u];
    }
    p1[3][u] = top[3][5 - u];
    p2[3][u] = top[3][5 - u] * wpow[u];
  }
  auto conv = [](const Fr (&x)[6], const Fr (&y)[6], Fr (&out)[6]) {
    for (int s2 = 0; s2 < 6; s2++) {
      Fr acc = Fr::zero();
      for (int u = 0; u <= s2; u++) acc = acc + x[u] * y[s2 - u];
      out[s2] = acc;
    }
  };
  Fr e1[6], e2[6], e3[6], h1[6], h2[6], h3[6];
  conv(p1[0], p1[1], e1);
  conv(e1, p1[2], e2);
  conv(e2, p1[3], e3);
  conv(p2[0], p2[1], h1);
  conv(h1, p2[2], h2);
  conv(h2, p2[3], h3);
  T3Args ta;
  const Fr D = d3[0], D3 = D * D * D, i4 = d3[1] * inverse(D), quarter = inverse(fr_small(4));
  for (int k = 0; k < 6; k++) {
    ta.q3[k] = alpha * (e3[5 - k] - h3[5 - k]);
    const Fr c = D3 * ta.q3[k] * quarter;
    ta.c0[k] = c;
    ta.c1[k] = neg(i4 * c);
    ta.c2[k] = neg(c);
  }
  ta.i4 = i4;
  ta.two_over_d = fr_small(2) * inverse(D);
  ta.inv_d2 = inverse(D * D);
  hipLaunchKernelGGL(k_t_combine, dim3(grid_for(n, kT, 1u << 30)), dim3(kT), 0, s, Tz.p, (size_t)n, ta, t.p);
  NZ_HIP(hipGetLastError());
}

void Prover::to4t(const Fr* evals, Fr* coefs, Fr* evals4, const int* bidx, int nb, hipStream_t s) {
  if (!s) s = st();
  to4t_coefs(evals, coefs, bidx, nb, s);
  to4t_evals4(coefs, evals4, nb, s);
}

void Prover::to4t_coefs(const Fr* evals, Fr* coefs, const int* bidx, int nb, hipStream_t s, uint32_t* scr) {
  auto t0 = std::chrono::steady_clock::now();
  {
    const size_t sp = prof_gpu ? span_begin(1, s) : 0;
    ntt(eng->ntt_tables, evals, coefs, power, true, s, nullptr, nullptr, scr);
    if (prof_gpu) span_end(sp, s);
  }
  BlindIdx bi;
  bi.count = nb;
  for (int k = 0; k < nb; k++) bi.idx[k] = bidx[k];
  hipLaunchKernelGGL(k_blind, dim3(1), dim3(64), 0, s, coefs, (size_t)n, blind.p, bi);
  NZ_HIP(hipGetLastError());
  ntt_ms += ms_since(t0);
}

void Prover::to4t_evals4(const Fr* coefs, Fr* evals4, int nb, hipStream_t s, uint32_t* scr) {
  auto t0 = std::chrono::steady_clock::now();
  if (quot3) {
    for (int j = 0; j < 3; j++) {
      NttIo io;
      io.in_len = n;
      io.tw = ctw3.p + (size_t)j * (n - 1);
      io.fold_len = (size_t)nb;
      io.fold_n = n;
      io.fold_f = fr29_operand(d3[j]);
      {
        const size_t sp = prof_gpu ? span_begin(1, s) : 0;
        ntt(eng->ntt_tables, coefs, evals4 + (size_t)j * n, power, false, s, nullptr, &io, scr);
        if (prof_gpu) span_end(sp, s);
      }
    }
    NZ_HIP(hipGetLastError());
    ntt_ms += ms_since(t0);
    return;
  }
  NttIo io;
  io.in_len = (size_t)n + nb;
  io.in_f = g29.p;
  {
    const size_t sp = prof_gpu ? span_begin(1, s) : 0;
    ntt(eng->ntt_tables, coefs, evals4, power + 2, false, s, nullptr, &io, scr);
    if (prof_gpu) span_end(sp, s);
  }
  NZ_HIP(hipGetLastError());
  ntt_ms += ms_since(t0);
}

void Prover::commit_start(int slot, const Fr* coefs, size_t len, const MsmBaseTable* tab, const G1Affine* bases,
                          bool on_main) {
  static const char* const kEnq[kSlots] = {"mark: commit enqueue slot 0", "mark: commit enqueue slot 1",
                                           "mark: commit enqueue slot 2"};
  roctxMarkA(kEnq[slot]);
  NZ_HIP(hipEventRecord(ready[slot], st()));
  hipStream_t ms = on_main ? st() : aux[slot];
  if (!on_main) NZ_HIP(hipStreamWaitEvent(ms, ready[slot], 0));
  const bool lag = tab != nullptr && tab == &ltab;
  slot_lag[slot] = lag;
  slot_split[slot] = false;
  if (!shards.empty() && (!lag || own_lhi)) {
    for (auto& sh : shards) {
      const size_t lo = lag ? sh->llo : sh->lo, hi = lag ? sh->lhi : sh->hi;
      const size_t cnt = len > lo ? std::min(len, hi) - lo : 0;
      NZ_HIP(hipSetDevice(sh->device));
      if (cnt) {
        NZ_HIP(hipStreamWaitEvent(sh->st[slot], ready[slot], 0));
        NZ_HIP(hipMemcpyPeerAsync(sh->scal[slot].p, sh->device, coefs + lo, eng->device, cnt * sizeof(Fr),
                                  sh->st[slot]));
      }
      msm_enqueue(*sh->sc[slot], nullptr, sh->scal[slot].p, cnt, true, sh->st[slot],
                  lag ? &sh->ltable : &sh->table);
    }
    NZ_HIP(hipSetDevice(eng->device));
    len = std::min(len, lag ? own_lhi : own_hi);
    slot_split[slot] = true;
  }
  if (split_send && (!lag || split_own_l)) {
    NZ_HIP(hipEventSynchronize(ready[slot]));
    if (split_send(split_user, slot | (lag ? NZCB_MSM_LAGRANGE : 0), coefs, len) != 0)
      throw Error(NZCB_ERR_INTERNAL, "msm split: sending the scalars to the other ranks failed");
    len = std::min(len, lag ? split_own_l : split_own);
    slot_split[slot] = true;
  }
  const size_t sp = prof_gpu ? span_begin(0, ms) : 0;
  msm_enqueue(*msc[slot], bases ? bases : ptau.p, coefs, len, true, ms, tab ? tab : &ptab);
  if (prof_gpu) span_end(sp, ms);
  static const bool serial = std::getenv("NZCB_SERIAL") != nullptr;
  if (serial) NZ_HIP(hipStreamSynchronize(ms));
  static const char* const kDone[kSlots] = {"mark: commit enqueued slot 0", "mark: commit enqueued slot 1",
                                            "mark: commit enqueued slot 2"};
  roctxMarkA(kDone[slot]);
}

namespace {
void affine_to_le(const G1Affine& a, uint8_t* out) {
  const Fq x = a.is_inf() ? Fq::zero() : from_mont(a.x);
  const Fq y = a.is_inf() ? Fq::zero() : from_mont(a.y);
  std::memcpy(out, x.v, 32);
  std::memcpy(out + 32, y.v, 32);
}

G1xyzz xyzz_from_le(const uint8_t* in) {
  G1Affine a;
  Fq x, y;
  std::memcpy(x.v, in, 32);
  std::memcpy(y.v, in + 32, 32);
  if (x.is_zero() && y.is_zero()) return G1xyzz::inf();
  if (reduce_once(x) != x || reduce_once(y) != y) throw Error(NZCB_ERR_ARG, "msm split: partial not reduced");
  a.x = to_mont(x);
  a.y = to_mont(y);
  return xyzz_from_affine(a);
}
}

G1Affine Prover::commit_finish(int slot) {
  auto t0 = std::chrono::steady_clock::now();
  G1xyzz r = msm_finish(*msc[slot], aux[slot]);
  static const char* const kRes[kSlots] = {"mark: commit result slot 0", "mark: commit result slot 1",
                                           "mark: commit result slot 2"};
  roctxMarkA(kRes[slot]);
  const bool split = slot_split[slot];
  for (auto& sh : shards) {
    if (!split) break;
    NZ_HIP(hipSetDevice(sh->device));
    r = xyzz_add(r, msm_finish(*sh->sc[slot], sh->st[slot]));
  }
  if (!shards.empty()) NZ_HIP(hipSetDevice(eng->device));
  if (split && split_gather) {
    const G1Affine own = xyzz_to_affine(r);
    uint8_t own_le[64];
    affine_to_le(own, own_le);
    std::vector<uint8_t> parts((size_t)split_world * 64);
    if (split_gather(split_user, slot | (slot_lag[slot] ? NZCB_MSM_LAGRANGE : 0), own_le, parts.data()) != 0)
      throw Error(NZCB_ERR_INTERNAL, "msm split: gathering the partial sums failed");
    r = G1xyzz::inf();
    for (int k = 0; k < split_world; k++) r = xyzz_add(r, xyzz_from_le(parts.data() + 64 * (size_t)k));
  }
  msm_ms += ms_since(t0);
  return xyzz_to_affine(r);
}

void Prover::commit_start_abc(size_t len, bool signal_basis) {
  roctxMarkA("mark: commit enqueue A, B, C");
  const Fr* sc[3] = {A.p, B.p, C.p};
  const size_t sp = prof_gpu ? span_begin(0, st()) : 0;
  if (signal_basis && sigcommit) {
    const uint32_t stride = (uint32_t)sig_stride;
    hipLaunchKernelGGL(k_sig_stage, dim3(grid_for((size_t)3 * stride, kT, 1u << 30)), dim3(kT), 0, st(), sig_idx.p,
                       stride, sig_cnt[0], sig_cnt[1], sig_cnt[2], wit.p, blind.p, sig_scal.p);
    NZ_HIP(hipGetLastError());
    const Fr* ss[3] = {sig_scal.p, sig_scal.p + stride, sig_scal.p + 2 * (size_t)stride};
    const uint32_t base[3] = {0, stride, 2 * stride};
    msm_enqueue_sets(*msc[0], ss, 3, stride, false, st(), &stab, base);
  } else {
    msm_enqueue_sets(*msc[0], sc, 3, len, true, st(), &ltab);
  }
  if (prof_gpu) span_end(sp, st());
  roctxMarkA("mark: commit enqueued A, B, C");
}

void Prover::commit_finish_abc(G1Affine& a, G1Affine& b, G1Affine& c) {
  auto t0 = std::chrono::steady_clock::now();
  G1xyzz r[3];
  msm_finish_sets(*msc[0], st(), r);
  roctxMarkA("mark: commit result A, B, C");
  a = xyzz_to_affine(r[0]);
  b = xyzz_to_affine(r[1]);
  c = xyzz_to_affine(r[2]);
  msm_ms += ms_since(t0);
}

void Prover::debug_commit_abc(const uint8_t* witness, size_t n_witness, const uint8_t* blinding, bool signal_basis,
                              uint8_t* out) {
  if (!witness || !blinding || !out || n_witness != nWit) throw Error(NZCB_ERR_ARG, "commit A, B, C: bad argument");
  if (!lcommit || !shards.empty() || split_send || msc[0]->max_lsets < 3)
    throw Error(NZCB_ERR_ARG, "commit A, B, C: the context does not commit them in one schedule");
  if (signal_basis && !sigcommit) throw Error(NZCB_ERR_ARG, "commit A, B, C: the context has no signal basis");
  NZ_HIP(hipSetDevice(eng->device));
  if (side_done) NZ_HIP(hipEventSynchronize(side_done));
  load_witness(witness, blinding, false);
  hipLaunchKernelGGL(k_abc_tail, dim3(1), dim3(64), 0, st(), A.p, B.p, C.p, (size_t)n, blind.p);
  NZ_HIP(hipGetLastError());
  commit_start_abc(n + 2, signal_basis);
  G1Affine p[3];
  commit_finish_abc(p[0], p[1], p[2]);
  std::memcpy(out, p, sizeof p);
}

void Prover::debug_signal_rows(int set, uint8_t* rows_out, uint32_t* signals_out) {
  if (set < 0 || set > 2 || !sigcommit) throw Error(NZCB_ERR_ARG, "signal rows: no such set or no signal basis");
  NZ_HIP(hipSetDevice(eng->device));
  const uint32_t cnt = sig_cnt[set];
  if (!cnt) return;
  if (!rows_out || !signals_out) throw Error(NZCB_ERR_ARG, "null argument");
  std::vector<G1Affine> q(cnt);
  NZ_HIP(hipMemcpy(q.data(), stab.q.p + (size_t)set * sig_stride, cnt * sizeof(G1Affine), hipMemcpyDeviceToHost));
  NZ_HIP(hipMemcpy(signals_out, sig_idx.p + (size_t)set * sig_stride, cnt * sizeof(uint32_t), hipMemcpyDeviceToHost));
  Fq thirty_two = Fq::zero();
  thirty_two.v[0] = 32;
  const Fq k = inverse(to_mont(thirty_two));
  for (uint32_t i = 0; i < cnt; i++) {
    q[i].x = q[i].x * k;
    q[i].y = q[i].y * k;
  }
  std::memcpy(rows_out, q.data(), cnt * sizeof(G1Affine));
}

void Prover::set_msm_split(int world, size_t own_points, size_t own_lagrange, nzcb_msm_send_fn send,
                           nzcb_msm_gather_fn gather, void* user) {
  if (world <= 1 || !send || !gather) {
    split_send = nullptr;
    split_gather = nullptr;
    split_world = 1;
    split_own = split_own_l = 0;
    return;
  }
  if (!shards.empty()) throw Error(NZCB_ERR_ARG, "msm split: a context splits over devices or over ranks, not both");
  if (own_points == 0 || own_points > ptau.n) throw Error(NZCB_ERR_ARG, "msm split: bad own point count");
  if (own_lagrange > (lcommit ? ltau.n : 0))
    throw Error(NZCB_ERR_ARG, "msm split: bad own Lagrange point count (A, B, C are committed from coefficients "
                              "when the context has no Lagrange basis)");
  split_send = send;
  split_gather = gather;
  split_user = user;
  split_world = world;
  split_own = own_points;
  split_own_l = own_lagrange;
}

void Prover::eval_many(int np, const Fr* const* polys, const size_t* lens, const Fr* xs, Fr* out,
                       const std::function<void()>& overlap) {
  hipStream_t s = st();
  size_t nblocks = 0;
  const EvalSet es = eval_set(np, polys, lens, xs, &nblocks);
  if ((size_t)np * nblocks + kEvalMax > eval_part.n) throw Error(NZCB_ERR_INTERNAL, "eval partial buffer too small");
  eval_launch(es, nblocks, eval_part.p, eval_pw.p, (Fr*)(eval_pw.p + (size_t)kEvalMax * kT),
              top_host + kMbEvals, s);
  if (overlap) overlap();
  NZ_HIP(hipStreamSynchronize(s));
  for (int j = 0; j < np; j++) out[j] = top_host[kMbEvals + j];
}

void Prover::lin_tables(int k, const Fr& d, hipStream_t s) {
  lin_tables_build(((LinTab*)lin_host.data())[k], d, (LinTab*)lin_tab.p + k, lin_tile_pows(k), (int)lin_qn, s);
}

Fr* Prover::lin_tile_pows(int k) { return lin_tab.p + 2 * sizeof(LinTab) / sizeof(Fr) + (size_t)k * 2 * lin_qn; }

void Prover::div_pol1(const Fr* src, size_t m, int tab, const Fr& p0_adjust, Fr* dst, uint32_t flag_bit) {
  const LinTab& ht = ((const LinTab*)lin_host.data())[tab];
  div_pol1_launch(src, m, (const LinTab*)lin_tab.p + tab, ht.dp[1], lin_tile_pows(tab), lin_qn, scan_tmp.p, p0_adjust,
                  dst, flags.p, flag_bit, (uint32_t*)(top_host + kMbFlags), st());
}

namespace {
struct RoctxPhases {
  bool open = false;
  explicit RoctxPhases(const char* proof) { roctxRangePush(proof); }
  void next(const char* phase) {
    if (open) roctxRangePop();
    roctxRangePush(phase);
    open = true;
  }
  ~RoctxPhases() {
    if (open) roctxRangePop();
    roctxRangePop();
  }
};
}

namespace {
Fr random_fr() {
  for (;;) {
    uint8_t b[32];
    size_t got = 0;
    while (got < sizeof(b)) {
      ssize_t k = getrandom(b + got, sizeof(b) - got, 0);
      if (k < 0) {
        if (errno == EINTR || errno == EAGAIN) continue;
        throw Error(NZCB_ERR_INTERNAL, std::string("getrandom failed: ") + std::strerror(errno) +
                                           " (no entropy for the blinding scalars)");
      }
      got += (size_t)k;
    }
    b[31] &= 0x3f;
    Fr x;
    std::memcpy(x.v, b, 32);
    if (reduce_once(x) == x) return to_mont(x);
  }
}
}

void Prover::load_witness(const uint8_t* witness, const uint8_t* blinding, bool witness_on_device) {
  hipStream_t s = st();
  Fr bl[13];
  bl[0] = Fr::zero();
  bl[12] = Fr::zero();
  for (int i = 1; i <= 11; i++) bl[i] = blinding ? fr_from_le_normal(blinding + 32 * (i - 1)) : random_fr();
  NZ_HIP(hipMemcpyAsync(blind.p, bl, sizeof(bl), hipMemcpyHostToDevice, s));
  const Fr* wsrc = (const Fr*)witness;
  if (!witness_on_device) {
    NZ_HIP(hipMemcpyAsync(wtns_in.p, witness, (size_t)nWit * 32, hipMemcpyHostToDevice, s));
    wsrc = wtns_in.p;
  } else {
    hipPointerAttribute_t at;
    if (hipPointerGetAttributes(&at, witness) == hipSuccess && at.device != eng->device) {
      NZ_HIP(hipMemcpyPeerAsync(wtns_in.p, eng->device, witness, at.device, (size_t)nWit * 32, s));
      wsrc = wtns_in.p;
    }
  }
  hipLaunchKernelGGL(k_wit_to_mont, dim3(grid_for(nWit, kT, 1u << 30)), dim3(kT), 0, s, wsrc, wit.p,
                     (size_t)nWit);
  for (size_t l = 0; l + 1 < add_level_start.size(); l++) {
    uint32_t a0 = add_level_start[l], a1 = add_level_start[l + 1];
    if (a1 > a0)
      hipLaunchKernelGGL(k_additions, dim3(grid_for(a1 - a0, kT, 1u << 30)), dim3(kT), 0, s, adds.p + a0, a1 - a0,
                         wit.p);
  }
  hipLaunchKernelGGL(k_build_abc, dim3(grid_for(std::max<size_t>(n, nPublic), kT, 1u << 30)), dim3(kT), 0, s,
                     amap.p, bmap.p, cmap.p, nConstraints, n, wit.p, nVars, A.p, B.p, C.p, nPublic,
                     top_host + mb_apub, top_host + mb_pubw);
  NZ_HIP(hipGetLastError());
  NZ_HIP(hipStreamSynchronize(s));
}

void Prover::prove(const uint8_t* witness, size_t n_witness, const uint8_t* blinding, uint8_t* proof_out,
                   uint8_t* pub_out, bool witness_on_device) {
  if (n_witness != nWit) {
    throw Error(NZCB_ERR_WITNESS_LEN, "Invalid witness length. Circuit: " + std::to_string(nVars) +
                                          ", witness: " + std::to_string(n_witness) + ", " +
                                          std::to_string(nAdditions));
  }
  NZ_HIP(hipSetDevice(eng->device));
  hipStream_t s = st();
  msm_ms = ntt_ms = 0;
  spans_used = 0;
  if (side_done) NZ_HIP(hipEventSynchronize(side_done));
  static const char* kLaneMark[17] = {"lane 0", "lane 1", "lane 2", "lane 3", "lane 4", "lane 5", "lane 6", "lane 7",
                                      "lane 8", "lane 9", "lane 10", "lane 11", "lane 12", "lane 13", "lane 14",
                                      "lane 15", "lane 16"};
  roctxMarkA(kLaneMark[lane_id < 16 ? lane_id : 16]);
  RoctxPhases ranges("plonk_prove");
  ranges.next("witness: calculateAdditions + buildABC");
  auto T0 = std::chrono::steady_clock::now();
  auto lg = [&](const std::string& m) { if (log) log(m); };
  if (!sig_note.empty() && !sig_note_logged && log) {
    lg(sig_note);
    sig_note_logged = true;
  }
  lg("Reading Wtns");
  load_witness(witness, blinding, witness_on_device);
  tm[1] = ms_since(T0);

  ranges.next("round1: to4T + commit A, B, C");
  auto t1 = std::chrono::steady_clock::now();
  G1Affine pA, pB, pC, pZ, pT1, pT2, pT3, pWxi, pWxiw;
  {
    const int ba[2] = {2, 1}, bb[2] = {4, 3}, bc[2] = {6, 5};
    const bool abc_sets = lcommit && shards.empty() && !split_send && msc[0]->max_lsets >= 3 && abc_sets_enabled();
    if (lcommit) {
      hipLaunchKernelGGL(k_abc_tail, dim3(1), dim3(64), 0, s, A.p, B.p, C.p, (size_t)n, blind.p);
      NZ_HIP(hipGetLastError());
      NZ_HIP(hipEventRecord(side_ready, s));
      if (abc_sets) {
        lg("multiexp A");
        lg("multiexp B");
        lg("multiexp C");
        commit_start_abc(n + 2, true);
      } else {
      lg("multiexp A");
      commit_start(0, A.p, n + 2, &ltab, ltau.p);
      lg("multiexp B");
      commit_start(1, B.p, n + 2, &ltab, ltau.p);
      lg("multiexp C");
      }
      hipStream_t ss = aux[2];
      if (!abc_sets) commit_start(2, C.p, n + 2, &ltab, ltau.p, true);
      NZ_HIP(hipStreamWaitEvent(ss, side_ready, 0));
      to4t(A.p, pol_a.p, A4.p, ba, 2, ss);
      to4t(B.p, pol_b.p, B4.p, bb, 2, ss);
      to4t(C.p, pol_c.p, C4.p, bc, 2, ss);
      if (quot3) launch_gate_check(ss);
      NZ_HIP(hipEventRecord(side_done, ss));
    } else {
      to4t(A.p, pol_a.p, A4.p, ba, 2);
      lg("multiexp A");
      commit_start(0, pol_a.p, n + 2);
      to4t(B.p, pol_b.p, B4.p, bb, 2);
      lg("multiexp B");
      commit_start(1, pol_b.p, n + 2);
      to4t(C.p, pol_c.p, C4.p, bc, 2);
      lg("multiexp C");
      commit_start(2, pol_c.p, n + 2);
    }
    if (lcommit && abc_sets) {
      commit_finish_abc(pA, pB, pC);
    } else {
      pA = commit_finish(0);
      pB = commit_finish(1);
      pC = commit_finish(2);
    }
  }
  tm[2] = ms_since(t1);

  ranges.next("round2: grand product Z + commit");
  auto t2 = std::chrono::steady_clock::now();
  Fr beta, gamma;
  const Fr* Apub = top_host + mb_apub;
  {
    std::vector<uint8_t> tr;
    if (transcript_public) {
      for (uint32_t i = 0; i < nPublic; i++) {
        uint8_t be[32];
        fr_to_be(Apub[i], be);
        tr.insert(tr.end(), be, be + 32);
      }
    }
    for (const G1Affine* p : {&pA, &pB, &pC}) {
      uint8_t u[64];
      g1_uncompressed(*p, u);
      tr.insert(tr.end(), u, u + 64);
    }
    beta = hash_to_fr(tr);
    lg("beta: " + fr_dec(beta));
    std::vector<uint8_t> tr2(32);
    fr_to_be(beta, tr2.data());
    gamma = hash_to_fr(tr2);
    lg("gamma: " + fr_dec(gamma));
  }
  {
    bool generic_k = false;
    if (fault == NZCB_DEBUG_GENERIC_K) {
      fault = 0;
      generic_k = true;
    }
    const PermArgs pa = perm_args(beta, gamma, k1, k2, generic_k);
    perm_launch(A.p, B.p, C.p, sig_h.p, (size_t)n, w_h.p, pa, Z.p, scan_tmp.p, top_host + kMbTotals, s);
    NZ_HIP(hipStreamSynchronize(s));
    const Fr tt[2] = {top_host[kMbTotals], top_host[kMbTotals + 1]};
    if (tt[0] != tt[1]) throw Error(NZCB_ERR_COPY, "Copy constraints does not match");
    perm_apply(Z.p, (size_t)n, scan_tmp.p, tt[1], s);
    const int bz[3] = {9, 8, 7};
    to4t_coefs(Z.p, pol_z.p, bz, 3, s, ntt_scr2.p);
    lg("multiexp Z");
    commit_start(0, pol_z.p, n + 3);
    to4t_evals4(pol_z.p, Z4.p, 3, s, ntt_scr2.p);
    pZ = commit_finish(0);
  }
  tm[3] = ms_since(t2);

  ranges.next("round3: quotient t + commit T1, T2, T3");
  auto t3 = std::chrono::steady_clock::now();
  Fr alpha;
  {
    std::vector<uint8_t> tr(64);
    g1_uncompressed(pZ, tr.data());
    alpha = hash_to_fr(tr);
    lg("alpha: " + fr_dec(alpha));
  }
  {
    auto tq = std::chrono::steady_clock::now();
    NZ_HIP(hipStreamWaitEvent(s, side_done, 0));
    if (quot3) {
      round3_quot3(beta, gamma, alpha, s);
    } else {
      quot_launch(false, A4.p, B4.p, C4.p, Z4.p, cq.p, cs.p, cl.p, nPublic, A.p, (size_t)n, x_lo.p, root_hi.p, nullptr,
                  beta, gamma, alpha, k1, k2, zh_inv, T.p, s);
    }
    if (!quot3) {
      NttIo io;
      io.out_f = gi29.p;
      io.out_f_has_scale = true;
      io.out_limit = (size_t)3 * n + 6;
      io.out_flags = flags.p;
      {
        const size_t sp = prof_gpu ? span_begin(1, s) : 0;
        ntt(eng->ntt_tables, T.p, t.p, power + 2, true, s, nullptr, &io);
        if (prof_gpu) span_end(sp, s);
      }
      NZ_HIP(hipGetLastError());
      uint32_t f = 0;
      NZ_HIP(hipMemcpyAsync(&f, flags.p, 4, hipMemcpyDeviceToHost, s));
      NZ_HIP(hipStreamSynchronize(s));
      if (f & 1u) throw Error(NZCB_ERR_T_DIV, "T Polynomial is not divisible");
    }
    ntt_ms += ms_since(tq);
    if (fault == NZCB_FAULT_QUOTIENT) {
      fault = 0;
      hipLaunchKernelGGL(k_fault_bump, dim3(1), dim3(64), 0, s, t.p + 1);
      NZ_HIP(hipGetLastError());
    }
    lg("multiexp T1");
    commit_start(0, t.p, n);
    lg("multiexp T2");
    commit_start(1, t.p + n, n);
    lg("multiexp T3");
    commit_start(2, t.p + 2 * (size_t)n, n + 6);
    pT1 = commit_finish(0);
    pT2 = commit_finish(1);
    pT3 = commit_finish(2);
  }
  tm[4] = ms_since(t3);

  ranges.next("round4: evaluations");
  auto t4 = std::chrono::steady_clock::now();
  Fr xi, ea, eb, ec, es1, es2, et, ezw, er, xim;
  {
    std::vector<uint8_t> tr(192);
    g1_uncompressed(pT1, tr.data());
    g1_uncompressed(pT2, tr.data() + 64);
    g1_uncompressed(pT3, tr.data() + 128);
    xi = hash_to_fr(tr);
    lg("xi: " + fr_dec(xi));
    {
      const Fr* polys[7] = {pol_a.p, pol_b.p, pol_c.p, sigma.p, sigma.p + 5 * (size_t)n, t.p, pol_z.p};
      const size_t lens[7] = {n + 2, n + 2, n + 2, n, n, 3 * (size_t)n + 6, n + 3};
      const Fr xs[7] = {xi, xi, xi, xi, xi, xi, xi * wn};
      Fr ev[7];
      eval_many(7, polys, lens, xs, ev, [&] {
        lin_tables(0, xi, aux[2]);
        lin_tables(1, xi * wn, aux[2]);
        NZ_HIP(hipEventRecord(pows_done, aux[2]));
      });
      NZ_HIP(hipStreamWaitEvent(s, pows_done, 0));
      ea = ev[0];
      eb = ev[1];
      ec = ev[2];
      es1 = ev[3];
      es2 = ev[4];
      et = ev[5];
      ezw = ev[6];
    }
    Fr coef_ab = ea * eb;
    Fr betaxi = beta * xi;
    Fr e2 = (ea + betaxi + gamma) * (eb + betaxi * k1 + gamma);
    e2 = e2 * (ec + betaxi * k2 + gamma) * alpha;
    Fr e3 = (ea + beta * es1 + gamma) * (eb + beta * es2 + gamma);
    e3 = e3 * beta * ezw * alpha;
    xim = xi;
    for (int i = 0; i < power; i++) xim = sqr(xim);
    Fr eval_l1 = (xim - Fr::one()) * inverse((xi - Fr::one()) * fr_small(n));
    Fr e4 = eval_l1 * (alpha * alpha);
    RArgs ra{e2 + e4, coef_ab, ea, eb, ec, e3};
    hipLaunchKernelGGL(k_pol_r, dim3(grid_for(n + 3, kT, 1u << 30)), dim3(kT), 0, s, pol_z.p, qm.p, ql.p, qr.p,
                       qo.p, qc.p, sigma.p + 10 * (size_t)n, (size_t)n, ra, pol_r.p);
    NZ_HIP(hipGetLastError());
    {
      const Fr* polys[1] = {pol_r.p};
      const size_t lens[1] = {n + 3};
      eval_many(1, polys, lens, &xi, &er);
    }
    {
      const Fr zh = xim - Fr::one(), nf = fr_small(n);
      Fr pi = Fr::zero(), wj = Fr::one();
      for (uint32_t j = 0; j < nPublic; j++) {
        pi = pi - Apub[j] * wj * zh * inverse(nf * (xi - wj));
        wj = wj * wn;
      }
      const Fr perm = alpha * (ea + beta * es1 + gamma) * (eb + beta * es2 + gamma) * (ec + gamma) * ezw;
      if (et * zh != er + pi - perm - e4)
        throw Error(NZCB_ERR_INTERNAL, "quotient check failed: t(xi) Z_H(xi) differs from the numerator at xi");
    }
  }
  tm[5] = ms_since(t4);

  ranges.next("round5: Wxi, Wxiw + commit");
  auto t5 = std::chrono::steady_clock::now();
  {
    std::vector<uint8_t> tr(7 * 32);
    const Fr* ev[7] = {&ea, &eb, &ec, &es1, &es2, &ezw, &er};
    for (int i = 0; i < 7; i++) fr_to_be(*ev[i], tr.data() + 32 * i);
    WArgs wa;
    wa.v[0] = Fr::zero();
    wa.v[1] = hash_to_fr(tr);
    lg("v: " + fr_dec(wa.v[1]));
    for (int i = 2; i <= 6; i++) wa.v[i] = wa.v[i - 1] * wa.v[1];
    wa.xim = xim;
    wa.xi2m = xim * xim;
    wa.w0sub = et + wa.v[1] * er + wa.v[2] * ea + wa.v[3] * eb + wa.v[4] * ec + wa.v[5] * es1 + wa.v[6] * es2;
    hipLaunchKernelGGL(k_pol_wxi, dim3(grid_for(n + 6, kT, 1u << 30)), dim3(kT), 0, s, t.p, pol_r.p, pol_a.p,
                       pol_b.p, pol_c.p, sigma.p, sigma.p + 5 * (size_t)n, (size_t)n, wa, T.p);
    NZ_HIP(hipGetLastError());
    div_pol1(T.p, n + 6, 0, Fr::zero(), pol_wxi.p, 4u);
    lg("multiexp Wxi");
    commit_start(0, pol_wxi.p, n + 6);
    div_pol1(pol_z.p, n + 3, 1, ezw, pol_wxiw.p, 4u);
    lg("multiexp Wxiw");
    commit_start(1, pol_wxiw.p, n + 3);
    NZ_HIP(hipStreamSynchronize(s));
    const uint32_t f = top_host[kMbFlags].v[0];
    pWxi = commit_finish(0);
    pWxiw = commit_finish(1);
    if (f & 4u) throw Error(NZCB_ERR_DIVPOL, "Polinomial does not divide");
  }
  tm[6] = ms_since(t5);
  tm[0] = ms_since(T0);
  tm[7] = msm_ms;
  tm[8] = ntt_ms;
  tm[9] = tm[10] = -1;
  if (prof_gpu) span_totals(&tm[9], &tm[10]);

  const G1Affine* pts[9] = {&pA, &pB, &pC, &pZ, &pT1, &pT2, &pT3, &pWxi, &pWxiw};
  for (int i = 0; i < 9; i++) {
    uint8_t* o = proof_out + 64 * i;
    if (pts[i]->is_inf()) {
      std::memset(o, 0, 64);
    } else {
      Fq x = from_mont(pts[i]->x), y = from_mont(pts[i]->y);
      std::memcpy(o, x.v, 32);
      std::memcpy(o + 32, y.v, 32);
    }
  }
  const Fr* ev[7] = {&ea, &eb, &ec, &es1, &es2, &ezw, &er};
  for (int i = 0; i < 7; i++) fr_to_le_normal(*ev[i], proof_out + 9 * 64 + 32 * i);
  for (uint32_t i = 0; i < nPublic; i++) {
    fr_to_le_normal(top_host[mb_pubw + i], pub_out + 32 * (size_t)i);
  }
}

namespace {

constexpr size_t kDebugMax = (size_t)1 << 26;

void need_canonical(const uint8_t* p, size_t count, const char* what) {
  for (size_t i = 0; i < count; i++) {
    Fr x;
    std::memcpy(x.v, p + 32 * i, 32);
    if (reduce_once(x) != x) throw Error(NZCB_ERR_ARG, std::string(what) + ": a word is not below r");
  }
}
Fr lem_word(const uint8_t* p, const char* what) {
  need_canonical(p, 1, what);
  Fr x;
  std::memcpy(x.v, p, 32);
  return x;
}

Fr* upload(CallScope& cs, const uint8_t* src, size_t count) {
  Fr* d = cs.alloc<Fr>(count * sizeof(Fr));
  if (count) NZ_HIP(hipMemcpyAsync(d, src, count * sizeof(Fr), hipMemcpyHostToDevice, cs.st));
  return d;
}

struct Mailbox {
  Fr* p = nullptr;
  explicit Mailbox(size_t words) {
    NZ_HIP(hipHostMalloc((void**)&p, words * sizeof(Fr), hipHostMallocCoherent));
    std::memset((void*)p, 0, words * sizeof(Fr));
  }
  ~Mailbox() {
    if (p) (void)hipHostFree(p);
  }
  Mailbox(const Mailbox&) = delete;
  Mailbox& operator=(const Mailbox&) = delete;
};

void debug_grand_product(int device, const uint8_t* abc, const uint8_t* sigma, const uint8_t* x, size_t n,
                         const uint8_t* beta, const uint8_t* gamma, const uint8_t* k1, const uint8_t* k2, int generic_k,
                         uint8_t* z_out, uint8_t* totals_out) {
  if (!abc || !sigma || !x || !beta || !gamma || !k1 || !k2 || !z_out || !totals_out || n < 1 || n > kDebugMax)
    throw Error(NZCB_ERR_ARG, "grand product: null argument or n outside 1..2^26");
  need_canonical(abc, 3 * n, "grand product: abc");
  need_canonical(sigma, 3 * n, "grand product: sigma");
  need_canonical(x, n, "grand product: x");
  const Fr b = lem_word(beta, "grand product: beta"), g = lem_word(gamma, "grand product: gamma");
  const Fr f1 = lem_word(k1, "grand product: k1"), f2 = lem_word(k2, "grand product: k2");
  CallScope cs(device, nullptr, 0);
  Mailbox mail(2);
  const Fr* dabc = upload(cs, abc, 3 * n);
  const Fr* dsig = upload(cs, sigma, 3 * n);
  const Fr* dx = upload(cs, x, n);
  Fr* dz = cs.alloc<Fr>(n * sizeof(Fr));
  Fr* scan = cs.alloc<Fr>(3 * perm_tiles(n) * sizeof(Fr));
  perm_launch(dabc, dabc + n, dabc + 2 * n, dsig, n, dx, perm_args(b, g, f1, f2, generic_k != 0), dz, scan, mail.p,
              cs.st);
  NZ_HIP(hipStreamSynchronize(cs.st));
  const Fr tt[2] = {mail.p[0], mail.p[1]};
  perm_apply(dz, n, scan, tt[1], cs.st);
  NZ_HIP(hipMemcpyAsync(z_out, dz, n * sizeof(Fr), hipMemcpyDeviceToHost, cs.st));
  NZ_HIP(hipStreamSynchronize(cs.st));
  std::memcpy(totals_out, tt, sizeof(tt));
}

void debug_div_pol1(int device, const uint8_t* p, size_t m, const uint8_t* d, const uint8_t* p0_adjust, uint8_t* q_out,
                    int* divides_out) {
  if (!p || !d || !p0_adjust || !q_out || !divides_out || m < 2 || m > kDebugMax)
    throw Error(NZCB_ERR_ARG, "divPol1: null argument or m outside 2..2^26");
  need_canonical(p, m, "divPol1: p");
  const Fr dv = lem_word(d, "divPol1: d"), adj = lem_word(p0_adjust, "divPol1: p0_adjust");
  LinTab host;
  CallScope cs(device, nullptr, 0);
  Mailbox mail(1);
  const Fr* src = upload(cs, p, m);
  const size_t qn = lin_tiles(m) + 2;
  LinTab* lt = cs.alloc<LinTab>(sizeof(LinTab));
  Fr* q = cs.alloc<Fr>(2 * qn * sizeof(Fr));
  Fr* heads = cs.alloc<Fr>((lin_tiles(m) + 1) * sizeof(Fr));
  Fr* dst = cs.alloc<Fr>(m * sizeof(Fr));
  uint32_t* flags = cs.alloc<uint32_t>(sizeof(uint32_t));
  NZ_HIP(hipMemsetAsync(flags, 0, sizeof(uint32_t), cs.st));
  lin_tables_build(host, dv, lt, q, (int)qn, cs.st);
  div_pol1_launch(src, m, lt, dv, q, qn, heads, adj, dst, flags, 4u, (uint32_t*)mail.p, cs.st);
  NZ_HIP(hipMemcpyAsync(q_out, dst, m * sizeof(Fr), hipMemcpyDeviceToHost, cs.st));
  NZ_HIP(hipStreamSynchronize(cs.st));
  *divides_out = (mail.p[0].v[0] & 4u) ? 0 : 1;
}

void debug_eval_many(int device, int np, const uint8_t* const* polys, const size_t* lens, const uint8_t* xs,
                     uint8_t* out) {
  if ((np != 1 && np != 7) || !polys || !lens || !xs || !out)
    throw Error(NZCB_ERR_ARG, "evaluations: null argument or np not 1 or 7");
  for (int j = 0; j < np; j++) {
    if (!polys[j] || lens[j] < 1 || lens[j] > kDebugMax)
      throw Error(NZCB_ERR_ARG, "evaluations: null polynomial or length outside 1..2^26");
    need_canonical(polys[j], lens[j], "evaluations: coefficients");
  }
  need_canonical(xs, (size_t)np, "evaluations: xs");
  CallScope cs(device, nullptr, 0);
  Mailbox mail(kEvalMax);
  const Fr* dp[kEvalMax];
  Fr xv[kEvalMax];
  for (int j = 0; j < np; j++) {
    dp[j] = upload(cs, polys[j], lens[j]);
    std::memcpy(xv[j].v, xs + 32 * (size_t)j, 32);
  }
  size_t nblocks = 0;
  const EvalSet es = eval_set(np, dp, lens, xv, &nblocks);
  Fr* part = cs.alloc<Fr>((size_t)np * nblocks * sizeof(Fr));
  F29* pw = cs.alloc<F29>((size_t)kEvalMax * kT * sizeof(F29));
  Fr* pw2 = cs.alloc<Fr>((size_t)kEvalMax * kEvalBits * sizeof(Fr));
  eval_launch(es, nblocks, part, pw, pw2, mail.p, cs.st);
  NZ_HIP(hipStreamSynchronize(cs.st));
  std::memcpy(out, mail.p, (size_t)np * sizeof(Fr));
}

void debug_quotient(int device, int power, int three, uint32_t npub, const uint8_t* abcz, const uint8_t* q,
                    const uint8_t* sg, const uint8_t* l, const uint8_t* apub, const uint8_t* beta, const uint8_t* gamma,
                    const uint8_t* alpha, const uint8_t* k1, const uint8_t* k2, uint8_t* t_out) {
  if (!abcz || !q || !sg || !l || (npub && !apub) || !beta || !gamma || !alpha || !k1 || !k2 || !t_out || power < 2 ||
      power > 24 || npub > 64)
    throw Error(NZCB_ERR_ARG, "quotient: null argument, power outside 2..24 or more than 64 public inputs");
  if (three && npub > kQ29MaxPub)
    throw Error(NZCB_ERR_ARG, "quotient: the three-coset form takes at most 8 public inputs");
  const size_t n = (size_t)1 << power, P = (three ? 3 : 4) * n;
  const uint32_t nl = npub > 0 ? npub : 1;
  need_canonical(abcz, 4 * P, "quotient: abcz");
  need_canonical(q, 5 * P, "quotient: q");
  need_canonical(sg, 3 * P, "quotient: s");
  need_canonical(l, nl * P, "quotient: l");
  need_canonical(apub, npub, "quotient: apub");
  const Fr b = lem_word(beta, "quotient: beta"), g = lem_word(gamma, "quotient: gamma");
  const Fr a = lem_word(alpha, "quotient: alpha");
  const Fr f1 = lem_word(k1, "quotient: k1"), f2 = lem_word(k2, "quotient: k2");
  CallScope cs(device, nullptr, 0);
  const Fr* dabcz = upload(cs, abcz, 4 * P);
  Fr* dq = upload(cs, q, 5 * P);
  const Fr* ds = upload(cs, sg, 3 * P);
  Fr* dl = upload(cs, l, nl * P);
  const Fr* dapub = upload(cs, apub, npub);
  Fr* bx_lo = three ? cs.alloc<Fr>(4096 * sizeof(Fr)) : nullptr;
  Fr* dt = cs.alloc<Fr>(P * sizeof(Fr));
  DevBuf<Fr> x_lo, root_hi;
  Fr zh_inv[4];
  try {
    quot_x_tables(power, x_lo, root_hi, zh_inv, cs.st);
    if (npub <= kQ29MaxPub) quot29_prescale(dq, dl, nl, P, x_lo.p, cs.st);
    quot_launch(three != 0, dabcz, dabcz + P, dabcz + 2 * P, dabcz + 3 * P, dq, ds, dl, npub, dapub, n, x_lo.p, root_hi.p,
                bx_lo, b, g, a, f1, f2, zh_inv, dt, cs.st);
    NZ_HIP(hipMemcpyAsync(t_out, dt, P * sizeof(Fr), hipMemcpyDeviceToHost, cs.st));
    NZ_HIP(hipStreamSynchronize(cs.st));
  } catch (...) {
    (void)hipStreamSynchronize(cs.st);
    throw;
  }
}

}

}

using namespace nzcb;

extern "C" int nzcb_debug_grand_product(int device, const uint8_t* abc, const uint8_t* sigma, const uint8_t* x, size_t n,
                                        const uint8_t* beta, const uint8_t* gamma, const uint8_t* k1, const uint8_t* k2,
                                        int generic_k, uint8_t* z_out, uint8_t* totals_out, nzcb_err* err) {
  return guarded(err, [&] { debug_grand_product(device, abc, sigma, x, n, beta, gamma, k1, k2, generic_k, z_out, totals_out); });
}

extern "C" int nzcb_debug_div_pol1(int device, const uint8_t* p, size_t m, const uint8_t* d, const uint8_t* p0_adjust,
                                   uint8_t* q_out, int* divides_out, nzcb_err* err) {
  return guarded(err, [&] { debug_div_pol1(device, p, m, d, p0_adjust, q_out, divides_out); });
}

extern "C" int nzcb_debug_eval_many(int device, int np, const uint8_t* const* polys, const size_t* lens,
                                    const uint8_t* xs, uint8_t* out, nzcb_err* err) {
  return guarded(err, [&] { debug_eval_many(device, np, polys, lens, xs, out); });
}

extern "C" int nzcb_debug_quotient(int device, int power, int three, uint32_t npub, const uint8_t* abcz,
                                   const uint8_t* q, const uint8_t* s, const uint8_t* l, const uint8_t* apub,
                                   const uint8_t* beta, const uint8_t* gamma, const uint8_t* alpha, const uint8_t* k1,
                                   const uint8_t* k2, uint8_t* t_out, nzcb_err* err) {
  return guarded(err, [&] {
    debug_quotient(device, power, three, npub, abcz, q, s, l, apub, beta, gamma, alpha, k1, k2, t_out);
  });
}
```

### nzcb-circom_amd/nzcb/__init__.py

```python
from __future__ import annotations

import ctypes
import json
import os
from ctypes import POINTER, c_char, c_double, c_int, c_size_t, c_uint8, c_uint32, c_uint64, c_void_p

_HERE = os.path.dirname(os.path.abspath(__file__))
LIB_PATH = os.environ.get("NZCB_LIB", os.path.join(os.path.dirname(_HERE), "lib", "libnzcb.so"))

PROOF_BYTES = 9 * 64 + 7 * 32
BLINDING_BYTES = 11 * 32
VK_BYTES = 8 + 2 * 32 + 8 * 64 + 4 * 32 + 32
PROOF_POINTS = ("A", "B", "C", "Z", "T1", "T2", "T3", "Wxi", "Wxiw")
PROOF_EVALS = ("eval_a", "eval_b", "eval_c", "eval_s1", "eval_s2", "eval_zw", "eval_r")
VK_POINTS = ("Qm", "Ql", "Qr", "Qo", "Qc", "S1", "S2", "S3")

ERROR_NAMES = {
    0: "OK", 1: "ARG", 2: "FORMAT", 3: "NOT_PLONK", 4: "CURVE", 5: "WITNESS_LEN", 6: "COPY",
    7: "T_DIV", 8: "TZ", 9: "DIVPOL", 10: "HIP", 11: "INTERNAL",
}

EXPORTED_SYMBOLS = [
    "nzcb_version", "nzcb_device_count", "nzcb_ctx_create", "nzcb_ctx_destroy", "nzcb_ctx_set_logger",
    "nzcb_ctx_set_transcript_public", "nzcb_ctx_info", "nzcb_prove", "nzcb_prove_witness", "nzcb_prove_device",
    "nzcb_ctx_kernel_stats",
    "nzcb_ctx_last_timings", "nzcb_proof_to_json", "nzcb_public_to_json", "nzcb_synth_setup", "nzcb_free",
    "nzcb_engine_create", "nzcb_engine_destroy", "nzcb_engine_ntt", "nzcb_engine_msm", "nzcb_dev_alloc",
    "nzcb_dev_free", "nzcb_memcpy_h2d", "nzcb_memcpy_d2h", "nzcb_engine_ntt_dev", "nzcb_engine_msm_dev",
    "nzcb_engine_time_ntt", "nzcb_engine_fr_mul", "nzcb_engine_random_fr", "nzcb_engine_fixed_base",
    "nzcb_engine_time_msm", "nzcb_engine_msm_fixed_dev", "nzcb_engine_msm_table_dev", "nzcb_engine_msm_sets_dev", "nzcb_engine_time_msm2", "nzcb_ctx_set_lanes",
    "nzcb_ctx_lanes", "nzcb_prove_batch", "nzcb_vk_from_zkey", "nzcb_vk_from_zkey_file", "nzcb_vk_to_json", "nzcb_verify",
    "nzcb_proof_to_calldata", "nzcb_vk_to_solidity", "nzcb_engine_lagrange_basis", "nzcb_ctx_set_msm_devices", "nzcb_nzcp_input_signals", "nzcb_nzcp_witness",
    "nzcb_nzcp_witness_dev", "nzcb_synth_setup_ex", "nzcb_memcpy_d2d",
    "nzcb_plonk_setup", "nzcb_prove_batch_status", "nzcb_wprog_remap", "nzcb_prove_logged", "nzcb_memcpy_d2d_async",
    "nzcb_debug_guard_check", "nzcb_debug_guard_selftest", "nzcb_debug_inject_fault", "nzcb_debug_f29",
    "nzcb_debug_ntt_coset", "nzcb_debug_msm_plan",
    "nzcb_msm_table_create_lagrange",
    "nzcb_verify_batch", "nzcb_engine_g1_lincomb", "nzcb_engine_verify_batch", "nzcb_debug_verify_batch_timings",
    "nzcb_r1cs_create", "nzcb_r1cs_create_file", "nzcb_r1cs_info", "nzcb_r1cs_check", "nzcb_r1cs_destroy",
    "nzcb_engine_r1cs_create", "nzcb_debug_r1cs_check_timings",
    "nzcb_p256_key_create", "nzcb_p256_verify", "nzcb_p256_key_destroy", "nzcb_engine_p256_key_create",
    "nzcb_debug_p256_field", "nzcb_debug_p256_mul2", "nzcb_debug_p256_timings",
    "nzcb_nzcp_pass_layout", "nzcb_nzcp_decode", "nzcb_nzcp_decode_dev", "nzcb_debug_nzcp_decode_timings",
    "nzcb_ptau_check", "nzcb_ptau_check_file", "nzcb_zkey_check", "nzcb_zkey_check_file", "nzcb_engine_srs_check",
    "nzcb_debug_key_check_timings",
    "nzcb_ptau_new", "nzcb_ptau_new_file", "nzcb_ptau_contribute", "nzcb_ptau_contribute_file",
    "nzcb_ptau_prepare_phase2", "nzcb_ptau_prepare_phase2_file", "nzcb_debug_ptau_timings",
    "nzcb_debug_ptau_batch_top",
    "nzcb_groth16_setup", "nzcb_groth16_setup_file", "nzcb_groth16_contribute", "nzcb_groth16_contribute_file",
    "nzcb_groth16_vk_to_json", "nzcb_groth16_vk_to_json_file", "nzcb_engine_groth16_rows",
    "nzcb_debug_groth16_schedule", "nzcb_debug_groth16_timings",
    "nzcb_debug_signal_basis_cap", "nzcb_debug_signal_basis_info", "nzcb_debug_commit_abc", "nzcb_debug_signal_rows",
    "nzcb_debug_grand_product", "nzcb_debug_div_pol1", "nzcb_debug_eval_many", "nzcb_debug_quotient",
]

NZCB_FAULT_QUOTIENT = 1
NZCB_DEBUG_GENERIC_K = 2
NZCB_FAULT_LANE_ALLOC = 3
VERIFY_HOST = -1
R1CS_HOST = -1
WITNESS_WTNS, WITNESS_HOST, WITNESS_DEVICE = 0, 1, 2
P256_HOST = -1
SIG_OK, SIG_INVALID, SIG_RANGE = 0, 1, 2
NZCP_HOST = -1
PASS_MAX_URI = 2048
PASS_STATUS_NAMES = ("OK", "LENGTH", "PREFIX", "BASE32", "TRUNCATED", "CBOR", "NOT_COSE", "HEADER",
                     "CLAIMS")
PASS_HAS_ALG, PASS_HAS_KID, PASS_HAS_ISS, PASS_HAS_NBF, PASS_HAS_EXP, PASS_HAS_CTI, PASS_HAS_SIG = (
    1, 2, 4, 8, 16, 32, 64)
KEY_HOST = -1
PTAU_HOST = -1
GROTH16_HOST = -1
KEY_STATUS_NAMES = ("OK", "G2", "RANGE", "CURVE", "GENERATOR", "SEQUENCE", "COSETS", "NONCANONICAL", "LAGRANGE",
                    "EVALS", "COMMIT")
KEY_PARTS = ("Qm", "Ql", "Qr", "Qo", "Qc", "S1", "S2", "S3")
P256_OPS = {"add": 0, "sub": 1, "mul": 2, "sqr": 3, "inv": 4}


def lagrange_commit_enabled() -> bool:
    import re
    e = os.environ.get("NZCB_LAGRANGE_COMMIT")
    if e is None:
        return True
    m = re.match(r"\s*[+-]?\d+", e)
    return bool(m) and int(m.group()) != 0


def signal_basis_cap(per_constraint: int = -1) -> int:
    return load().nzcb_debug_signal_basis_cap(per_constraint)


def guard_check(device: int = -1) -> int:
    err, checked, bad = _Err(), c_size_t(0), c_int(0)
    _check(load().nzcb_debug_guard_check(device, ctypes.byref(checked), ctypes.byref(bad), ctypes.byref(err)), err)
    return checked.value


F29_WORDS = {1: (27, 9), 2: (54, 18), 3: (18, 9), 4: (36, 18), 5: (18, 18), 6: (36, 9), 7: (10, 9)}


def f29_check(op: int, words, device: int = 0):
    win, wout = F29_WORDS[op]
    count = len(words) // win
    assert count * win == len(words)
    arr = (c_uint32 * max(1, len(words)))(*words)
    out = (c_uint32 * max(1, count * wout))()
    err = _Err()
    _check(load().nzcb_debug_f29(device, op, arr, count, out, ctypes.byref(err)), err)
    return list(out)[:count * wout]


def debug_grand_product(abc: bytes, sigma: bytes, x: bytes, beta: bytes, gamma: bytes, k1: bytes, k2: bytes,
                        generic_k: bool = False, device: int = 0):
    n = len(x) // 32
    assert len(x) == 32 * n and len(abc) == 96 * n and len(sigma) == 96 * n
    z, tot, err = _out(32 * n), _out(64), _Err()
    _check(load().nzcb_debug_grand_product(device, abc, sigma, x, n, beta, gamma, k1, k2, int(generic_k), z, tot,
                                           ctypes.byref(err)), err)
    return bytes(z)[:32 * n], bytes(tot)


def debug_div_pol1(p: bytes, d: bytes, p0_adjust: bytes = bytes(32), device: int = 0):
    m = len(p) // 32
    assert len(p) == 32 * m
    q, ok, err = _out(32 * m), c_int(-1), _Err()
    _check(load().nzcb_debug_div_pol1(device, p, m, d, p0_adjust, q, ctypes.byref(ok), ctypes.byref(err)), err)
    return bytes(q)[:32 * m], bool(ok.value)


def debug_eval_many(polys, xs: bytes, device: int = 0) -> bytes:
    np_ = len(polys)
    assert len(xs) == 32 * np_ and all(len(p) % 32 == 0 for p in polys)
    arr = (ctypes.c_char_p * max(np_, 1))(*polys)
    lens = (c_size_t * max(np_, 1))(*[len(p) // 32 for p in polys])
    out, err = _out(32 * np_), _Err()
    _check(load().nzcb_debug_eval_many(device, np_, arr, lens, xs, out, ctypes.byref(err)), err)
    return bytes(out)[:32 * np_]


def debug_quotient(power: int, three: bool, npub: int, abcz: bytes, q: bytes, s: bytes, l: bytes, apub: bytes,
                   beta: bytes, gamma: bytes, alpha: bytes, k1: bytes, k2: bytes, device: int = 0) -> bytes:
    pts = (3 if three else 4) << power
    assert len(abcz) == 128 * pts and len(q) == 160 * pts and len(s) == 96 * pts
    assert len(l) == 32 * pts * max(npub, 1) and len(apub) == 32 * npub
    out, err = _out(32 * pts), _Err()
    _check(load().nzcb_debug_quotient(device, power, int(three), npub, abcz, q, s, l, apub, beta, gamma, alpha, k1, k2,
                                      out, ctypes.byref(err)), err)
    return bytes(out)[:32 * pts]


def guard_selftest(device: int = 0) -> None:
    err = _Err()
    _check(load().nzcb_debug_guard_selftest(device, ctypes.byref(err)), err)


class NzcbError(RuntimeError):
    def __init__(self, code: int, msg: str):
        super().__init__(msg)
        self.code = code
        self.name = ERROR_NAMES.get(code, str(code))


class _Err(ctypes.Structure):
    _fields_ = [("code", c_int), ("msg", c_char * 256)]


class NzcpParams(ctypes.Structure):
    _fields_ = [("is_live", ctypes.c_int32), ("max_tbs_bytes", ctypes.c_int32),
                ("max_array_len_vc", ctypes.c_int32), ("max_map_len_vc", ctypes.c_int32)]


class NzcpRecord(ctypes.Structure):
    _fields_ = [("status", ctypes.c_int32), ("detail", ctypes.c_int32), ("exp", ctypes.c_uint32),
                ("vc_pos", ctypes.c_int32), ("given_len", ctypes.c_int32), ("family_len", ctypes.c_int32),
                ("dob_len", ctypes.c_int32), ("nullifier_len", ctypes.c_int32),
                ("tbs_sha256", c_uint8 * 32), ("nullifier_sha512", c_uint8 * 64), ("nullifier", c_uint8 * 64),
                ("pub", (c_uint8 * 32) * 3)]


class NzcpPass(ctypes.Structure):
    _fields_ = [("status", ctypes.c_int32), ("detail", c_uint32), ("version", c_uint32), ("present", c_uint32),
                ("alg", ctypes.c_int32), ("kid_len", c_uint32), ("iss_len", c_uint32), ("cti_len", c_uint32),
                ("sig_len", c_uint32), ("cose_len", c_uint32), ("protected_off", c_uint32),
                ("protected_len", c_uint32), ("payload_off", c_uint32), ("payload_len", c_uint32),
                ("tbs_len", c_uint32), ("fits", c_uint32), ("nbf", c_uint64), ("exp", c_uint64),
                ("kid", c_uint8 * 32), ("cti", c_uint8 * 32), ("iss", c_uint8 * 64), ("sig", c_uint8 * 64),
                ("tbs_sha256", c_uint8 * 32)]


NZCP_LIVE = dict(is_live=1, max_tbs_bytes=351, max_array_len_vc=0, max_map_len_vc=4)
NZCP_EXAMPLE = dict(is_live=0, max_tbs_bytes=314, max_array_len_vc=0, max_map_len_vc=4)

LOG_FN = ctypes.CFUNCTYPE(None, c_void_p, ctypes.c_char_p)
MSM_SEND_FN = ctypes.CFUNCTYPE(c_int, c_void_p, c_int, c_void_p, c_size_t)
MSM_GATHER_FN = ctypes.CFUNCTYPE(c_int, c_void_p, c_int, POINTER(c_uint8), POINTER(c_uint8))
MSM_LAGRANGE = 0x100

class KeyFinding(ctypes.Structure):
    _fields_ = [("status", ctypes.c_int32), ("pairing_checks", c_uint32), ("index", ctypes.c_uint64),
                ("n_bad", ctypes.c_uint64), ("checked", ctypes.c_uint64)]


_lib = None


def load(path: str | None = None):
    global _lib
    if _lib is not None and path is None:
        return _lib
    if os.environ.get("GPU_MAX_HW_QUEUES", "4") == "4":
        os.environ["GPU_MAX_HW_QUEUES"] = "24"
    lib = ctypes.CDLL(path or LIB_PATH)
    u8p = POINTER(c_uint8)
    sigs = {
        "nzcb_version": (ctypes.c_char_p, []),
        "nzcb_device_count": (c_int, []),
        "nzcb_ctx_create": (c_void_p, [u8p, c_size_t, c_int, POINTER(_Err)]),
        "nzcb_ctx_destroy": (None, [c_void_p]),
        "nzcb_ctx_set_logger": (None, [c_void_p, LOG_FN, c_void_p]),
        "nzcb_ctx_set_transcript_public": (None, [c_void_p, c_int]),
        "nzcb_ctx_info": (c_int, [c_void_p, POINTER(c_uint32)]),
        "nzcb_prove": (c_int, [c_void_p, u8p, c_size_t, u8p, u8p, u8p, c_size_t, POINTER(_Err)]),
        "nzcb_prove_witness": (c_int, [c_void_p, u8p, c_size_t, u8p, u8p, u8p, c_size_t, POINTER(_Err)]),
        "nzcb_prove_device": (c_int, [c_void_p, c_void_p, c_size_t, u8p, u8p, u8p, c_size_t, POINTER(_Err)]),
        "nzcb_prove_logged": (c_int, [c_void_p, c_void_p, c_size_t, c_int, u8p, u8p, u8p, c_size_t, LOG_FN, c_void_p,
                                      POINTER(_Err)]),
        "nzcb_ctx_kernel_stats": (c_int, [c_void_p, c_int, POINTER(c_double)]),
        "nzcb_ctx_set_lanes": (c_int, [c_void_p, c_int, POINTER(_Err)]),
        "nzcb_ctx_set_msm_devices": (c_int, [c_void_p, POINTER(c_int), c_int, POINTER(_Err)]),
        "nzcb_vk_from_zkey": (c_int, [u8p, c_size_t, u8p, POINTER(_Err)]),
        "nzcb_vk_from_zkey_file": (c_int, [ctypes.c_char_p, u8p, POINTER(_Err)]),
        "nzcb_vk_to_json": (c_int, [u8p, ctypes.c_char_p, c_size_t]),
        "nzcb_verify": (c_int, [u8p, u8p, u8p, c_int, c_int, POINTER(c_int), POINTER(_Err)]),
        "nzcb_proof_to_calldata": (c_int, [u8p, u8p, c_int, ctypes.c_char_p, c_size_t]),
        "nzcb_vk_to_solidity": (c_int, [u8p, ctypes.c_char_p, c_int, ctypes.c_char_p, c_size_t]),
        "nzcb_engine_lagrange_basis": (c_int, [c_void_p, c_void_p, c_size_t, c_int, c_void_p, POINTER(_Err)]),
        "nzcb_ctx_lanes": (c_int, [c_void_p]),
        "nzcb_prove_batch": (c_int, [c_void_p, POINTER(c_void_p), c_size_t, c_int, c_int, u8p, u8p, u8p, c_size_t,
                                     POINTER(_Err)]),
        "nzcb_prove_batch_status": (c_int, [c_void_p, POINTER(c_void_p), c_size_t, c_int, c_int, u8p, u8p, u8p,
                                            c_size_t, POINTER(c_int), POINTER(_Err)]),
        "nzcb_ctx_last_timings": (c_int, [c_void_p, POINTER(c_double), c_int]),
        "nzcb_proof_to_json": (c_int, [u8p, ctypes.c_char_p, c_size_t]),
        "nzcb_public_to_json": (c_int, [u8p, c_int, ctypes.c_char_p, c_size_t]),
        "nzcb_synth_setup": (c_int, [c_int, c_int, c_int, c_uint64, c_uint32, u8p, c_int,
                                     POINTER(POINTER(c_uint8)), POINTER(c_size_t),
                                     POINTER(POINTER(c_uint8)), POINTER(c_size_t), POINTER(_Err)]),
        "nzcb_synth_setup_ex": (c_int, [c_int, c_int, c_int, c_uint64, c_uint32, c_uint32, u8p, c_int,
                                        POINTER(POINTER(c_uint8)), POINTER(c_size_t),
                                        POINTER(POINTER(c_uint8)), POINTER(c_size_t), POINTER(_Err)]),
        "nzcb_free": (None, [c_void_p]),
        "nzcb_engine_create": (c_void_p, [c_int, c_int, c_size_t, POINTER(_Err)]),
        "nzcb_engine_destroy": (None, [c_void_p]),
        "nzcb_engine_ntt": (c_int, [c_void_p, u8p, u8p, c_int, c_int, POINTER(_Err)]),
        "nzcb_debug_ntt_coset": (c_int, [c_void_p, u8p, u8p, c_int, u8p, c_int, POINTER(_Err)]),
        "nzcb_engine_msm": (c_int, [c_void_p, u8p, u8p, c_size_t, c_int, u8p, POINTER(_Err)]),
        "nzcb_dev_alloc": (c_void_p, [c_size_t]),
        "nzcb_dev_alloc_on": (c_void_p, [c_int, c_size_t]),
        "nzcb_dev_free": (None, [c_void_p]),
        "nzcb_memcpy_h2d": (c_int, [c_void_p, c_void_p, c_size_t]),
        "nzcb_memcpy_d2h": (c_int, [c_void_p, c_void_p, c_size_t]),
        "nzcb_memcpy_d2d": (c_int, [c_void_p, c_void_p, c_size_t]),
        "nzcb_memcpy_d2d_async": (c_int, [c_void_p, c_void_p, c_size_t, c_void_p]),
        "nzcb_engine_ntt_dev": (c_int, [c_void_p, c_void_p, c_void_p, c_int, c_int, POINTER(_Err)]),
        "nzcb_engine_msm_dev": (c_int, [c_void_p, c_void_p, c_void_p, c_size_t, c_int, u8p, POINTER(_Err)]),
        "nzcb_engine_time_ntt": (c_int, [c_void_p, c_void_p, c_void_p, c_int, c_int, c_int, POINTER(c_double),
                                         POINTER(_Err)]),
        "nzcb_engine_fr_mul": (c_int, [c_void_p, u8p, u8p, u8p, c_size_t, c_int, POINTER(_Err)]),
        "nzcb_engine_random_fr": (c_int, [c_void_p, c_void_p, c_size_t, c_uint64, POINTER(_Err)]),
        "nzcb_engine_fixed_base": (c_int, [c_void_p, c_void_p, c_size_t, c_void_p, POINTER(_Err)]),
        "nzcb_engine_time_msm": (c_int, [c_void_p, c_void_p, c_void_p, c_size_t, c_int, c_int, POINTER(c_double),
                                         POINTER(c_double), POINTER(_Err)]),
        "nzcb_engine_msm_fixed_dev": (c_int, [c_void_p, c_void_p, c_size_t, c_void_p, c_size_t, c_int, u8p,
                                              POINTER(_Err)]),
        "nzcb_engine_msm_table_dev": (c_int, [c_void_p, c_void_p, c_size_t, c_void_p, c_size_t, c_int, c_int, c_int,
                                              c_int, u8p, POINTER(_Err)]),
        "nzcb_engine_msm_sets_dev": (c_int, [c_void_p, c_void_p, c_size_t, POINTER(c_void_p), c_int, c_size_t, c_int,
                                             c_int, u8p, POINTER(_Err)]),
        "nzcb_debug_msm_plan": (c_int, [c_void_p, c_void_p, c_size_t, c_void_p, c_size_t, c_int, c_int, c_int,
                                        POINTER(c_uint32), POINTER(c_uint32), c_size_t, POINTER(c_uint32), c_size_t,
                                        u8p, POINTER(_Err)]),
        "nzcb_plonk_setup": (c_int, [ctypes.c_char_p, c_size_t, ctypes.c_char_p, c_size_t, c_int, POINTER(POINTER(c_uint8)),
                                     POINTER(c_size_t), POINTER(_Err)]),
        "nzcb_nzcp_input_signals": (c_size_t, [POINTER(NzcpParams)]),
        "nzcb_nzcp_witness": (c_int, [c_int, POINTER(NzcpParams), u8p, c_int, POINTER(NzcpRecord), POINTER(_Err)]),
        "nzcb_nzcp_witness_dev": (c_int, [c_int, POINTER(NzcpParams), c_void_p, c_int, c_void_p, c_void_p, c_size_t,
                                          c_void_p, POINTER(_Err)]),
        "nzcb_engine_time_msm2": (c_int, [c_void_p, c_void_p, c_void_p, c_size_t, c_int, c_int, c_int,
                                          POINTER(c_double), POINTER(_Err)]),
        "nzcb_ctx_create_devices": (c_void_p, [u8p, c_size_t, POINTER(c_int), c_int, POINTER(_Err)]),
        "nzcb_ctx_devices": (c_int, [c_void_p]),
        "nzcb_ctx_set_msm_split": (c_int, [c_void_p, c_int, c_size_t, c_size_t, MSM_SEND_FN, MSM_GATHER_FN,
                                           c_void_p, POINTER(_Err)]),
        "nzcb_msm_table_create": (c_void_p, [c_int, c_void_p, c_size_t, POINTER(_Err)]),
        "nzcb_msm_table_create_lagrange": (c_void_p, [c_int, c_void_p, c_size_t, c_int, c_size_t, c_size_t,
                                                      POINTER(_Err)]),
        "nzcb_msm_table_run": (c_int, [c_void_p, c_void_p, c_size_t, c_int, u8p, POINTER(_Err)]),
        "nzcb_msm_table_destroy": (None, [c_void_p]),
        "nzcb_ptau_synth": (c_int, [c_int, u8p, c_int, POINTER(POINTER(c_uint8)), POINTER(c_size_t), POINTER(_Err)]),
        "nzcb_wprog_create": (c_void_p, [ctypes.c_char_p, c_size_t, c_int, POINTER(_Err)]),
        "nzcb_wprog_destroy": (None, [c_void_p]),
        "nzcb_wprog_info": (c_int, [c_void_p, POINTER(c_uint32)]),
        "nzcb_wprog_run_dev": (c_int, [c_void_p, c_void_p, c_int, c_void_p, c_size_t, POINTER(ctypes.c_int32),
                                       c_void_p, POINTER(_Err)]),
        "nzcb_wprog_run": (c_int, [c_void_p, ctypes.c_char_p, c_int, u8p, POINTER(ctypes.c_int32), POINTER(_Err)]),
        "nzcb_wprog_remap": (c_int, [ctypes.c_char_p, c_size_t, ctypes.c_char_p, c_size_t, ctypes.c_char_p, c_size_t,
                                     POINTER(POINTER(c_uint8)), POINTER(c_size_t), POINTER(c_uint32), POINTER(_Err)]),
        "nzcb_debug_guard_check": (c_int, [c_int, POINTER(c_size_t), POINTER(c_int), POINTER(_Err)]),
        "nzcb_debug_guard_selftest": (c_int, [c_int, POINTER(_Err)]),
        "nzcb_debug_inject_fault": (c_int, [c_void_p, c_int]),
        "nzcb_debug_f29": (c_int, [c_int, c_int, POINTER(c_uint32), c_size_t, POINTER(c_uint32), POINTER(_Err)]),
        "nzcb_verify_batch": (c_int, [u8p, u8p, u8p, c_size_t, c_int, c_int, c_int, c_int, u8p, POINTER(c_int),
                                      POINTER(_Err)]),
        "nzcb_engine_g1_lincomb": (c_int, [c_int, u8p, u8p, POINTER(c_uint32), c_size_t, u8p, POINTER(_Err)]),
        "nzcb_engine_verify_batch": (c_int, [u8p, u8p, u8p, c_size_t, c_int, c_int, c_int, c_int, u8p, POINTER(c_int),
                                             u8p, POINTER(c_int), POINTER(_Err)]),
        "nzcb_debug_verify_batch_timings": (c_int, [POINTER(c_double), c_int]),
        "nzcb_r1cs_create": (c_void_p, [ctypes.c_char_p, c_size_t, c_int, POINTER(_Err)]),
        "nzcb_r1cs_create_file": (c_void_p, [ctypes.c_char_p, c_int, POINTER(_Err)]),
        "nzcb_engine_r1cs_create": (c_void_p, [ctypes.c_char_p, c_size_t, c_int, c_uint32, c_int, POINTER(_Err)]),
        "nzcb_r1cs_info": (c_int, [c_void_p, POINTER(c_uint32)]),
        "nzcb_r1cs_check": (c_int, [c_void_p, c_void_p, c_size_t, c_int, c_int, c_size_t, POINTER(c_uint32),
                                    POINTER(c_uint32), c_uint32, c_void_p, POINTER(_Err)]),
        "nzcb_r1cs_destroy": (None, [c_void_p]),
        "nzcb_debug_r1cs_check_timings": (c_int, [POINTER(c_double), c_int]),
        "nzcb_p256_key_create": (c_void_p, [ctypes.c_char_p, c_int, POINTER(_Err)]),
        "nzcb_engine_p256_key_create": (c_void_p, [ctypes.c_char_p, c_int, c_int, POINTER(_Err)]),
        "nzcb_p256_verify": (c_int, [c_void_p, c_void_p, c_size_t, c_void_p, c_size_t, c_int, c_int,
                                     POINTER(ctypes.c_int32), c_void_p, POINTER(_Err)]),
        "nzcb_p256_key_destroy": (None, [c_void_p]),
        "nzcb_debug_p256_field": (c_int, [c_int, c_int, c_int, ctypes.c_char_p, ctypes.c_char_p, c_size_t, u8p,
                                          POINTER(_Err)]),
        "nzcb_debug_p256_mul2": (c_int, [c_void_p, ctypes.c_char_p, ctypes.c_char_p, c_size_t, u8p, POINTER(_Err)]),
        "nzcb_debug_p256_timings": (c_int, [POINTER(c_double), c_int]),
        "nzcb_nzcp_pass_layout": (None, [POINTER(c_uint32)]),
        "nzcb_nzcp_decode": (c_int, [c_int, ctypes.c_char_p, POINTER(c_uint32), c_int, POINTER(NzcpParams),
                                     ctypes.c_char_p, POINTER(NzcpPass), u8p, u8p, c_size_t, POINTER(_Err)]),
        "nzcb_nzcp_decode_dev": (c_int, [c_int, c_void_p, c_void_p, c_int, POINTER(NzcpParams), c_void_p, c_void_p,
                                         c_void_p, c_void_p, c_size_t, c_void_p, POINTER(_Err)]),
        "nzcb_debug_nzcp_decode_timings": (c_int, [POINTER(c_double), c_int]),
        "nzcb_ptau_check": (c_int, [c_void_p, c_size_t, ctypes.c_uint64, c_int, u8p, POINTER(KeyFinding),
                                    POINTER(_Err)]),
        "nzcb_ptau_check_file": (c_int, [ctypes.c_char_p, ctypes.c_uint64, c_int, u8p, POINTER(KeyFinding),
                                         POINTER(_Err)]),
        "nzcb_zkey_check": (c_int, [c_void_p, c_size_t, c_int, u8p, POINTER(c_int), POINTER(KeyFinding),
                                    POINTER(KeyFinding), c_uint32, POINTER(c_uint32), POINTER(_Err)]),
        "nzcb_zkey_check_file": (c_int, [ctypes.c_char_p, c_int, u8p, POINTER(c_int), POINTER(KeyFinding),
                                         POINTER(KeyFinding), c_uint32, POINTER(c_uint32), POINTER(_Err)]),
        "nzcb_engine_srs_check": (c_int, [c_int, c_void_p, ctypes.c_uint64, u8p, u8p, c_uint32, POINTER(KeyFinding),
                                          u8p, POINTER(_Err)]),
        "nzcb_debug_key_check_timings": (c_int, [POINTER(c_double), c_int]),
        "nzcb_ptau_new": (c_int, [c_int, POINTER(POINTER(c_uint8)), POINTER(c_size_t), POINTER(_Err)]),
        "nzcb_ptau_new_file": (c_int, [c_int, ctypes.c_char_p, POINTER(_Err)]),
        "nzcb_ptau_contribute": (c_int, [c_void_p, c_size_t, u8p, ctypes.c_char_p, c_size_t, c_int,
                                         POINTER(POINTER(c_uint8)), POINTER(c_size_t), POINTER(_Err)]),
        "nzcb_ptau_contribute_file": (c_int, [ctypes.c_char_p, ctypes.c_char_p, u8p, ctypes.c_char_p, c_size_t,
                                              c_int, POINTER(_Err)]),
        "nzcb_ptau_prepare_phase2": (c_int, [c_void_p, c_size_t, c_int, POINTER(POINTER(c_uint8)),
                                             POINTER(c_size_t), POINTER(_Err)]),
        "nzcb_ptau_prepare_phase2_file": (c_int, [ctypes.c_char_p, ctypes.c_char_p, c_int, POINTER(_Err)]),
        "nzcb_debug_ptau_timings": (c_int, [POINTER(c_double), c_int]),
        "nzcb_debug_ptau_batch_top": (c_int, [c_int]),
        "nzcb_groth16_setup": (c_int, [c_void_p, c_size_t, c_void_p, c_size_t, c_int, POINTER(POINTER(c_uint8)),
                                       POINTER(c_size_t), POINTER(_Err)]),
        "nzcb_groth16_setup_file": (c_int, [ctypes.c_char_p, ctypes.c_char_p, ctypes.c_char_p, c_int, POINTER(_Err)]),
        "nzcb_groth16_contribute": (c_int, [c_void_p, c_size_t, u8p, ctypes.c_char_p, c_size_t, c_int,
                                            POINTER(POINTER(c_uint8)), POINTER(c_size_t), POINTER(_Err)]),
        "nzcb_groth16_contribute_file": (c_int, [ctypes.c_char_p, ctypes.c_char_p, u8p, ctypes.c_char_p, c_size_t,
                                                 c_int, POINTER(_Err)]),
        "nzcb_groth16_vk_to_json": (c_int, [c_void_p, c_size_t, ctypes.c_char_p, c_size_t]),
        "nzcb_groth16_vk_to_json_file": (c_int, [ctypes.c_char_p, ctypes.c_char_p, c_size_t]),
        "nzcb_engine_groth16_rows": (c_int, [c_int, c_int, c_void_p, ctypes.c_uint64, POINTER(ctypes.c_uint64),
                                             ctypes.c_uint64, POINTER(c_uint32), u8p, u8p, POINTER(_Err)]),
        "nzcb_debug_groth16_schedule": (c_int, [c_int, c_int, POINTER(c_int), POINTER(c_int)]),
        "nzcb_debug_groth16_timings": (c_int, [POINTER(c_double), c_int]),
        "nzcb_debug_signal_basis_cap": (c_int, [c_int]),
        "nzcb_debug_signal_basis_info": (c_int, [c_void_p, POINTER(c_uint64)]),
        "nzcb_debug_commit_abc": (c_int, [c_void_p, u8p, c_size_t, u8p, c_int, u8p, POINTER(_Err)]),
        "nzcb_debug_signal_rows": (c_int, [c_void_p, c_int, u8p, POINTER(c_uint32), c_size_t, POINTER(_Err)]),
        "nzcb_debug_grand_product": (c_int, [c_int, ctypes.c_char_p, ctypes.c_char_p, ctypes.c_char_p, c_size_t,
                                             ctypes.c_char_p, ctypes.c_char_p, ctypes.c_char_p, ctypes.c_char_p, c_int,
                                             u8p, u8p, POINTER(_Err)]),
        "nzcb_debug_div_pol1": (c_int, [c_int, ctypes.c_char_p, c_size_t, ctypes.c_char_p, ctypes.c_char_p, u8p,
                                        POINTER(c_int), POINTER(_Err)]),
        "nzcb_debug_eval_many": (c_int, [c_int, c_int, POINTER(ctypes.c_char_p), POINTER(c_size_t), ctypes.c_char_p,
                                         u8p, POINTER(_Err)]),
        "nzcb_debug_quotient": (c_int, [c_int, c_int, c_int, c_uint32, ctypes.c_char_p, ctypes.c_char_p,
                                        ctypes.c_char_p, ctypes.c_char_p, ctypes.c_char_p, ctypes.c_char_p,
                                        ctypes.c_char_p, ctypes.c_char_p, ctypes.c_char_p, ctypes.c_char_p, u8p,
                                        POINTER(_Err)]),
    }
    lib.missing_symbols = []
    for name, (res, args) in sigs.items():
        try:
            fn = getattr(lib, name)
        except AttributeError:
            lib.missing_symbols.append(name)
            continue
        fn.restype = res
        fn.argtypes = args
    if "nzcb_nzcp_pass_layout" not in lib.missing_symbols:
        lay = (c_uint32 * 3)()
        lib.nzcb_nzcp_pass_layout(lay)
        if list(lay) != [ctypes.sizeof(NzcpPass), NzcpPass.sig.offset, NzcpPass.tbs_sha256.offset]:
            raise OSError(f"NzcpPass does not mirror nzcb_nzcp_pass: the library reports {list(lay)}")
    _lib = lib
    return lib


def _buf(data: bytes):
    return (c_uint8 * len(data)).from_buffer_copy(data) if data else (c_uint8 * 1)()


def _out(n: int):
    return (c_uint8 * max(n, 1))()


def _check(rc: int, err: _Err):
    if rc != 0:
        raise NzcbError(rc, err.msg.decode(errors="replace"))


def version() -> str:
    return load().nzcb_version().decode()


def device_count() -> int:
    return load().nzcb_device_count()


def nzcp_input_signals(params: dict) -> int:
    return load().nzcb_nzcp_input_signals(ctypes.byref(NzcpParams(**params)))


def _record_dict(r: NzcpRecord) -> dict:
    return {
        "status": r.status, "detail": r.detail, "exp": r.exp, "vc_pos": r.vc_pos, "given_len": r.given_len,
        "family_len": r.family_len, "dob_len": r.dob_len, "nullifier_len": r.nullifier_len,
        "tbs_sha256": bytes(r.tbs_sha256), "nullifier_sha512": bytes(r.nullifier_sha512),
        "nullifier": bytes(r.nullifier), "out": [int.from_bytes(bytes(r.pub[k]), "little") for k in range(3)],
    }


def nzcp_witness(inputs: bytes, count: int, params: dict = NZCP_LIVE, device: int = 0) -> list:
    lib = load()
    prm = NzcpParams(**params)
    need = lib.nzcb_nzcp_input_signals(ctypes.byref(prm)) * 32 * count
    if len(inputs) != need:
        raise ValueError(f"nzcp inputs are {len(inputs)} bytes, expected {need}")
    recs = (NzcpRecord * max(count, 1))()
    err = _Err()
    _check(lib.nzcb_nzcp_witness(device, ctypes.byref(prm), _buf(inputs), count, recs, ctypes.byref(err)), err)
    return [_record_dict(recs[i]) for i in range(count)]


def nzcp_witness_dev(dev_inputs: int, count: int, params: dict = NZCP_LIVE, device: int = 0,
                     dev_records: int | None = None, dev_witness: int | None = None, witness_stride: int = 0,
                     stream: int | None = None):
    lib = load()
    err = _Err()
    _check(lib.nzcb_nzcp_witness_dev(device, ctypes.byref(NzcpParams(**params)), dev_inputs, count, dev_records,
                                     dev_witness, witness_stride, stream, ctypes.byref(err)), err)


def nzcp_records_from_bytes(raw: bytes, count: int) -> list:
    size = ctypes.sizeof(NzcpRecord)
    return [_record_dict(NzcpRecord.from_buffer_copy(raw[i * size:(i + 1) * size])) for i in range(count)]


def _pass_dict(r: NzcpPass) -> dict:
    has = lambda bit: bool(r.present & bit)
    return {
        "status": r.status, "status_name": PASS_STATUS_NAMES[r.status], "detail": r.detail, "version": r.version,
        "present": r.present, "alg": r.alg if has(PASS_HAS_ALG) else None,
        "kid": bytes(r.kid)[:min(r.kid_len, 32)] if has(PASS_HAS_KID) else None, "kid_len": r.kid_len,
        "iss": bytes(r.iss)[:min(r.iss_len, 64)].decode(errors="replace") if has(PASS_HAS_ISS) else None,
        "iss_len": r.iss_len, "nbf": r.nbf if has(PASS_HAS_NBF) else None,
        "exp": r.exp if has(PASS_HAS_EXP) else None,
        "cti": bytes(r.cti)[:min(r.cti_len, 32)] if has(PASS_HAS_CTI) else None, "cti_len": r.cti_len,
        "sig": bytes(r.sig) if has(PASS_HAS_SIG) else None, "sig_len": r.sig_len, "cose_len": r.cose_len,
        "protected_off": r.protected_off, "protected_len": r.protected_len, "payload_off": r.payload_off,
        "payload_len": r.payload_len, "tbs_len": r.tbs_len, "fits": r.fits, "tbs_sha256": bytes(r.tbs_sha256),
    }


def nzcp_passes_from_bytes(raw: bytes, count: int) -> list:
    size = ctypes.sizeof(NzcpPass)
    return [_pass_dict(NzcpPass.from_buffer_copy(raw[i * size:(i + 1) * size])) for i in range(count)]


def pack_uris(uris):
    raw = [u.encode("utf-8", "surrogateescape") if isinstance(u, str) else bytes(u) for u in uris]
    offs, at = [0], 0
    for b in raw:
        at += len(b)
        offs.append(at)
    if at > 1 << 31:
        raise ValueError("more than 2^31 bytes of URIs")
    return b"".join(raw), (c_uint32 * len(offs))(*offs)


def nzcp_decode_raw(uris, params: dict | None = None, data20=None, device: int = 0, want_tbs: int = 0,
                    offsets=None):
    lib = load()
    if offsets is None:
        blob, offs = pack_uris(uris)
    else:
        blob, offs = bytes(uris), (c_uint32 * len(offsets))(*offsets)
    count = len(offs) - 1
    if data20 is not None:
        data20 = b"".join(data20) if isinstance(data20, (list, tuple)) else bytes(data20)
        if len(data20) != 20 * count:
            raise ValueError("data is 20 bytes per pass")
    prm = NzcpParams(**params) if params else None
    recs = (NzcpPass * max(count, 1))()
    inputs = _out(lib.nzcb_nzcp_input_signals(ctypes.byref(prm)) * 32 * count) if prm else None
    tbs = _out(want_tbs * count) if want_tbs else None
    err = _Err()
    _check(lib.nzcb_nzcp_decode(device, blob, offs, count, ctypes.byref(prm) if prm else None, data20, recs, inputs,
                                tbs, want_tbs, ctypes.byref(err)), err)
    size = ctypes.sizeof(NzcpPass)
    return (bytes(recs)[:size * count],
            bytes(inputs)[:lib.nzcb_nzcp_input_signals(ctypes.byref(prm)) * 32 * count] if prm else None,
            bytes(tbs)[:want_tbs * count] if want_tbs else None)


def nzcp_decode(uris, params: dict | None = None, data20=None, device: int = 0):
    uris = list(uris)
    recs, inputs, _ = nzcp_decode_raw(uris, params, data20, device)
    out = nzcp_passes_from_bytes(recs, len(uris))
    return (out, inputs) if params else out


def nzcp_decode_dev(dev_uris: int, dev_offsets: int, count: int, dev_passes: int, params: dict | None = None,
                    dev_data20: int | None = None, dev_inputs: int | None = None, dev_tbs: int | None = None,
                    tbs_stride: int = 0, device: int = 0, stream: int | None = None):
    lib = load()
    err = _Err()
    prm = NzcpParams(**params) if params else None
    _check(lib.nzcb_nzcp_decode_dev(device, dev_uris, dev_offsets, count, ctypes.byref(prm) if prm else None,
                                    dev_data20, dev_passes, dev_inputs, dev_tbs, tbs_stride, stream,
                                    ctypes.byref(err)), err)


def nzcp_decode_timings() -> list:
    ms = (c_double * 2)()
    n = load().nzcb_debug_nzcp_decode_timings(ms, 2)
    return list(ms)[:n]


class Engine:

    def __init__(self, device: int = 0, max_log_ntt: int = 12, max_msm_points: int = 1 << 12):
        self.lib = load()
        err = _Err()
        self.h = self.lib.nzcb_engine_create(device, max_log_ntt, max_msm_points, ctypes.byref(err))
        if not self.h:
            raise NzcbError(err.code, err.msg.decode(errors="replace"))

    def close(self):
        if self.h:
            self.lib.nzcb_engine_destroy(self.h)
            self.h = None

    __del__ = close

    def ntt(self, data_lem: bytes, log_n: int, inverse: bool = False) -> bytes:
        n = 1 << log_n
        assert len(data_lem) == 32 * n
        out = _out(32 * n)
        err = _Err()
        _check(self.lib.nzcb_engine_ntt(self.h, _buf(data_lem), out, log_n, int(inverse), ctypes.byref(err)), err)
        return bytes(out)

    def ntt_coset(self, data_lem: bytes, log_n: int, c_lem: bytes) -> bytes:
        n = 1 << log_n
        fold = len(data_lem) // 32 - n
        assert len(data_lem) == 32 * (n + fold) and fold >= 0 and len(c_lem) == 32
        out = _out(32 * n)
        err = _Err()
        _check(self.lib.nzcb_debug_ntt_coset(self.h, _buf(data_lem), out, log_n, _buf(c_lem), fold,
                                             ctypes.byref(err)), err)
        return bytes(out)

    def msm(self, bases_lem: bytes, scalars: bytes, scalars_mont: bool = False) -> bytes:
        n = len(scalars) // 32
        assert len(bases_lem) == 64 * n
        out = _out(64)
        err = _Err()
        _check(self.lib.nzcb_engine_msm(self.h, _buf(bases_lem), _buf(scalars), n, int(scalars_mont), out,
                                        ctypes.byref(err)), err)
        return bytes(out)

    def field_mul(self, a_lem: bytes, b_lem: bytes, field_q: bool = False) -> bytes:
        n = len(a_lem) // 32
        out = _out(32 * n)
        err = _Err()
        _check(self.lib.nzcb_engine_fr_mul(self.h, _buf(a_lem), _buf(b_lem), out, n, int(field_q),
                                           ctypes.byref(err)), err)
        return bytes(out)

    def time_ntt(self, dev_in: int, dev_out: int, log_n: int, inverse: bool, reps: int) -> float:
        ms = c_double()
        err = _Err()
        _check(self.lib.nzcb_engine_time_ntt(self.h, dev_in, dev_out, log_n, int(inverse), reps, ctypes.byref(ms),
                                             ctypes.byref(err)), err)
        return ms.value

    def random_fr(self, dev_out: int, n: int, seed: int):
        err = _Err()
        _check(self.lib.nzcb_engine_random_fr(self.h, dev_out, n, seed, ctypes.byref(err)), err)

    def fixed_base(self, dev_scalars: int, n: int, dev_out: int):
        err = _Err()
        _check(self.lib.nzcb_engine_fixed_base(self.h, dev_scalars, n, dev_out, ctypes.byref(err)), err)

    def lagrange_basis(self, dev_ptau: int, ptau_n: int, log_n: int, dev_out: int):
        err = _Err()
        _check(self.lib.nzcb_engine_lagrange_basis(self.h, dev_ptau, ptau_n, log_n, dev_out, ctypes.byref(err)), err)

    def time_msm(self, dev_bases: int, dev_scalars: int, n: int, scalars_mont: bool, reps: int):
        ms = c_double()
        acc = c_double()
        err = _Err()
        _check(self.lib.nzcb_engine_time_msm(self.h, dev_bases, dev_scalars, n, int(scalars_mont), reps,
                                             ctypes.byref(ms), ctypes.byref(acc), ctypes.byref(err)), err)
        return ms.value, acc.value

    MSM_PHASES = ("keys", "sort", "offsets", "accumulate", "finalize", "reduce", "sums")

    def time_msm_phases(self, dev_bases: int, dev_scalars: int, n: int, scalars_mont: bool, fixed_base: bool,
                        reps: int) -> dict:
        out = (c_double * 13)()
        err = _Err()
        _check(self.lib.nzcb_engine_time_msm2(self.h, dev_bases, dev_scalars, n, int(scalars_mont), int(fixed_base),
                                              reps, out, ctypes.byref(err)), err)
        d = {"wall": out[0], "table_build": out[8], "entries": out[9]}
        d.update({k: out[1 + i] for i, k in enumerate(self.MSM_PHASES)})
        d["host_finish"] = out[10]
        d["host_enqueue"] = out[11]
        d["host_sort_call"] = out[12]
        return d

    def msm_fixed_dev(self, dev_bases: int, n_table: int, dev_scalars: int, n: int, scalars_mont: bool,
                      window: int = 0, sparse: bool = False, fold: bool = False) -> bytes:
        out = _out(64)
        err = _Err()
        if window or sparse or fold:
            _check(self.lib.nzcb_engine_msm_table_dev(self.h, dev_bases, n_table, dev_scalars, n, int(scalars_mont),
                                                      int(window), int(sparse), int(fold), out, ctypes.byref(err)),
                   err)
        else:
            _check(self.lib.nzcb_engine_msm_fixed_dev(self.h, dev_bases, n_table, dev_scalars, n, int(scalars_mont),
                                                      out, ctypes.byref(err)), err)
        return bytes(out)

    def msm_plan(self, dev_bases: int, n_table: int, dev_scalars: int, n: int, scalars_mont: bool, window: int = 0,
                 fold: bool = False):
        c = window or 20
        off_cap = (1 << (c - 1)) + 1
        seg_cap = 3 * (n * ((255 + c - 1) // c) + 1)
        info, off, seg = (c_uint32 * 4)(), (c_uint32 * off_cap)(), (c_uint32 * seg_cap)()
        out = _out(64)
        err = _Err()
        _check(self.lib.nzcb_debug_msm_plan(self.h, dev_bases, n_table, dev_scalars, n, int(scalars_mont), int(window),
                                            int(fold), info, off, off_cap, seg, seg_cap, out, ctypes.byref(err)), err)
        if not info[0]:
            return bytes(out), None
        nk, ns = info[1], info[2]
        return bytes(out), {"seg_max": info[3], "offsets": off[:nk + 1], "start": seg[:ns], "len": seg[ns:2 * ns],
                            "bucket": seg[2 * ns:3 * ns]}

    def msm_sets_dev(self, dev_bases: int, n_table: int, dev_scalars: list, n: int, scalars_mont: bool, *,
                     sparse: bool) -> list:
        k = len(dev_scalars)
        out = _out(64 * k)
        err = _Err()
        arr = (c_void_p * k)(*dev_scalars)
        _check(self.lib.nzcb_engine_msm_sets_dev(self.h, dev_bases, n_table, arr, k, n, int(scalars_mont),
                                                 int(bool(sparse)), out, ctypes.byref(err)), err)
        return [bytes(out)[64 * i:64 * i + 64] for i in range(k)]

    def msm_dev(self, dev_bases: int, dev_scalars: int, n: int, scalars_mont: bool) -> bytes:
        out = _out(64)
        err = _Err()
        _check(self.lib.nzcb_engine_msm_dev(self.h, dev_bases, dev_scalars, n, int(scalars_mont), out,
                                            ctypes.byref(err)), err)
        return bytes(out)

    @staticmethod
    def g1_lincomb(points: bytes, scalars: bytes, group_end, device: int = 0) -> list:
        groups = len(group_end)
        n = group_end[-1] if groups else 0
# ... 1251 lines not shown
```

Measured before the change: 49.69 proofs/s.

## Move linear-combination prover kernels to lazy 9x29-bit multiply-sum arithmetic

Rewrites the gate check, t-combine, pol_r and pol_wxi kernels, plus the polynomial evaluation kernel, to use 9x29-bit limb dot products (mulsum29) with a single final reduction instead of chained Montgomery multiplies. The evaluation kernel replaces its serial Horner loop with a dot product against precomputed powers x^(kT*m) stored in an enlarged power table. Debug entry points are added for each rewritten kernel. The intent is to cut per-element modular reductions in these bandwidth- and ALU-heavy elementwise passes, at the cost of more register pressure and extra power-table setup.

Result: no change. 49.32 proofs/s (-0.7%).

```diff
diff --git a/include/nzcb_internal.h b/include/nzcb_internal.h
--- a/include/nzcb_internal.h
+++ b/include/nzcb_internal.h
@@ -39,6 +39,16 @@
                         const uint8_t* l , const uint8_t* apub , const uint8_t* beta,
                         const uint8_t* gamma, const uint8_t* alpha, const uint8_t* k1, const uint8_t* k2,
                         uint8_t* t_out , nzcb_err* err);
+int nzcb_debug_pol_r(int device, const uint8_t* pz , const uint8_t* q ,
+                     const uint8_t* s3 , size_t n, const uint8_t* consts ,
+                     uint8_t* out , nzcb_err* err);
+int nzcb_debug_pol_wxi(int device, const uint8_t* t , const uint8_t* r ,
+                       const uint8_t* abc , const uint8_t* s12 , size_t n,
+                       const uint8_t* consts , uint8_t* out , nzcb_err* err);
+int nzcb_debug_t_combine(int device, const uint8_t* v , size_t n, const uint8_t* corr ,
+                         const uint8_t* consts , uint8_t* t_out , nzcb_err* err);
+int nzcb_debug_gate_h(int device, const uint8_t* abc , const uint8_t* qh , size_t n,
+                      uint32_t npub, int* violated_out, nzcb_err* err);
 
 int nzcb_synth_setup(int power, int n_public, int n_inputs, uint64_t seed, uint32_t n_constraints,
                      const uint8_t* tau, int device, uint8_t** zkey_out, size_t* zkey_len, uint8_t** wtns_out,
diff --git a/nzcb-circom_amd/csrc/coef29.h b/nzcb-circom_amd/csrc/coef29.h
--- /dev/null
+++ b/nzcb-circom_amd/csrc/coef29.h
@@ -0,0 +1,132 @@
+#pragma once
+#include "f29.h"
+
+namespace nzcb {
+
+NZ_HD F29 fr29_operand(Fr c) {
+#pragma unroll
+  for (int k = 0; k < 5; k++) c = c + c;
+  return split29(c);
+}
+
+NZ_HD F29 f29_zero() {
+  F29 r;
+#pragma unroll
+  for (int l = 0; l < 9; l++) r.v[l] = 0;
+  return r;
+}
+
+NZ_HD F29 add29_nn(const F29& a, const F29& b) {
+  F29 r;
+#pragma unroll
+  for (int l = 0; l < 9; l++) r.v[l] = a.v[l] + b.v[l];
+  return r;
+}
+
+NZ_HD Fr canon_sum29(const F29& x) { return canon_fr29(x); }
+
+struct PolRArgs {
+  F29 c[6];
+};
+NZ_HD PolRArgs pol_r_args(const Fr& coefz, const Fr& coef_ab, const Fr& ea, const Fr& eb, const Fr& ec,
+                          const Fr& coefs3) {
+  PolRArgs a;
+  a.c[0] = fr29_operand(coefz);
+  a.c[1] = fr29_operand(coef_ab);
+  a.c[2] = fr29_operand(ea);
+  a.c[3] = fr29_operand(eb);
+  a.c[4] = fr29_operand(ec);
+  a.c[5] = fr29_operand(neg(coefs3));
+  return a;
+}
+NZ_HD Fr pol_r_elem(const PolRArgs& r, const Fr& pz, const Fr& qm, const Fr& ql, const Fr& qr, const Fr& qo,
+                    const Fr& qc, const Fr& s3) {
+  const F29 x[6] = {split29(pz), split29(qm), split29(ql), split29(qr), split29(qo), split29(s3)};
+  return canon_sum29(add29_nn(mulsum29<Fr29, 6>(x, r.c), split29(qc)));
+}
+
+struct PolWxiArgs {
+  F29 c[8];
+  F29 negw0;
+};
+NZ_HD PolWxiArgs pol_wxi_args(const Fr& xim, const Fr& xi2m, const Fr (&v)[7], const Fr& w0sub) {
+  PolWxiArgs a;
+  a.c[0] = fr29_operand(xi2m);
+  a.c[1] = fr29_operand(xim);
+#pragma unroll
+  for (int k = 1; k <= 6; k++) a.c[k + 1] = fr29_operand(v[k]);
+  a.negw0 = split29(neg(w0sub));
+  return a;
+}
+NZ_HD Fr pol_wxi_elem(const PolWxiArgs& w, const Fr& t2, const Fr& t1, const Fr& t0, const Fr& pr, const Fr& pa,
+                      const Fr& pb, const Fr& pc, const Fr& s1, const Fr& s2, bool first) {
+  const F29 x[4] = {split29(t2), split29(t1), split29(pr), split29(pa)};
+  const F29 y[4] = {split29(pb), split29(pc), split29(s1), split29(s2)};
+  const F29 cx[4] = {w.c[0], w.c[1], w.c[2], w.c[3]}, cy[4] = {w.c[4], w.c[5], w.c[6], w.c[7]};
+  F29 s = add29_nn(add29_nn(mulsum29<Fr29, 4>(x, cx), mulsum29<Fr29, 4>(y, cy)), split29(t0));
+  if (first) s = add29_nn(s, w.negw0);
+  return canon_sum29(s);
+}
+
+struct TCombArgs {
+  F29 negi4, two_over_d, inv_d2, i4_inv_d2;
+};
+NZ_HD TCombArgs t_combine_args(const Fr& i4, const Fr& two_over_d, const Fr& inv_d2) {
+  TCombArgs a;
+  a.negi4 = fr29_operand(neg(i4));
+  a.two_over_d = fr29_operand(two_over_d);
+  a.inv_d2 = fr29_operand(inv_d2);
+  a.i4_inv_d2 = fr29_operand(i4 * inv_d2);
+  return a;
+}
+NZ_HD void t_combine_elem(const TCombArgs& a, const Fr& v0, const Fr& v1, const Fr& v2, Fr& o0, Fr& o1, Fr& o2) {
+  const Fr sm = v0 + v2, dl = v0 - v2, v12 = v1 + v1;
+  const F29 d = split29(dl);
+  o0 = canon_sum29(add29_nn(mul29<Fr29>(d, a.negi4), split29(sm + v12)));
+  o1 = join_fr29(mul29<Fr29>(d, a.two_over_d));
+  const F29 x[2] = {split29(sm - v12), d}, c[2] = {a.inv_d2, a.i4_inv_d2};
+  o2 = join_fr29(mulsum29<Fr29, 2>(x, c));
+}
+
+NZ_HD bool gate_h_violated(const Fr& qm, const Fr& ql, const Fr& qr, const Fr& qo, const Fr& qc, const Fr& a,
+                           const Fr& b, const Fr& c, bool is_public) {
+  const F29 a5 = fr_to261(a), b5 = fr_to261(b), c5 = fr_to261(c);
+  const F29 x[4] = {mul29<Fr29>(split29(qm), a5), split29(ql), split29(qr), split29(qo)};
+  const F29 y[4] = {b5, a5, b5, c5};
+  F29 s = add29_nn(mulsum29<Fr29, 4>(x, y), split29(qc));
+  if (is_public) s = add29_nn(s, split29(neg(a)));
+  const uint32_t k = s.v[0] & 3u;
+  uint32_t any = 0;
+  int64_t carry = 0;
+#pragma unroll
+  for (int l = 0; l < 9; l++) {
+    const int64_t t = (int64_t)s.v[l] + carry - (int64_t)((uint64_t)k * Fr29::P[l]);
+    any |= l < 8 ? ((uint32_t)t & Fr29::MASK) : ((uint32_t)t | (uint32_t)((uint64_t)t >> 32));
+    carry = t >> 29;
+  }
+  return any != 0;
+}
+
+static constexpr int kEvalTerms = 16;
+template <class C>
+NZ_HD F29 eval_terms29(C&& coef, const F29* ypow, int nterms) {
+  F29 g0 = f29_zero(), g1 = f29_zero(), g2 = f29_zero();
+  if (nterms > 0) {
+    const F29 x[6] = {coef(0), coef(1), coef(2), coef(3), coef(4), coef(5)};
+    const F29 y[6] = {ypow[0], ypow[1], ypow[2], ypow[3], ypow[4], ypow[5]};
+    g0 = mulsum29<Fr29, 6>(x, y);
+  }
+  if (nterms > 6) {
+    const F29 x[6] = {coef(6), coef(7), coef(8), coef(9), coef(10), coef(11)};
+    const F29 y[6] = {ypow[6], ypow[7], ypow[8], ypow[9], ypow[10], ypow[11]};
+    g1 = mulsum29<Fr29, 6>(x, y);
+  }
+  if (nterms > 12) {
+    const F29 x[4] = {coef(12), coef(13), coef(14), coef(15)};
+    const F29 y[4] = {ypow[12], ypow[13], ypow[14], ypow[15]};
+    g2 = mulsum29<Fr29, 4>(x, y);
+  }
+  return add3_29(g0, g1, g2);
+}
+
+}
diff --git a/nzcb-circom_amd/csrc/prover.hip b/nzcb-circom_amd/csrc/prover.hip
--- a/nzcb-circom_amd/csrc/prover.hip
+++ b/nzcb-circom_amd/csrc/prover.hip
@@ -1,4 +1,5 @@
 #include <rocprofiler-sdk-roctx/roctx.h>
+#include "coef29.h"
 #include "devcall.h"
 #include "lagrange.h"
 #include "prover.h"
@@ -152,11 +153,6 @@
   for (int k = 0; k < 5; k++) m = m + m;
   w = split29(from_mont(c));
   ws = mul_lo261(split29(m), f29_const(Fr29::NINV));
-}
-
-static F29 fr29_operand(Fr c) {
-  for (int k = 0; k < 5; k++) c = c + c;
-  return split29(c);
 }
 
 #ifndef NZ_KPER
@@ -631,15 +627,13 @@
          size_t n, uint32_t npub, uint32_t* __restrict__ flags) {
   const size_t m = (size_t)blockIdx.x * blockDim.x + threadIdx.x;
   if (m >= n) return;
-  const Fr a = A[m], b = B[m], c = C[m];
-  Fr g = qh[m] * a * b + qh[n + m] * a + qh[2 * n + m] * b + qh[3 * n + m] * c + qh[4 * n + m];
-  if (m < npub) g = g - a;
-  if (!g.is_zero()) atomicOr(flags, 1u);
+  if (gate_h_violated(qh[m], qh[n + m], qh[2 * n + m], qh[3 * n + m], qh[4 * n + m], A[m], B[m], C[m], m < npub))
+    atomicOr(flags, 1u);
 }
 
 struct T3Args {
   Fr c0[6], c1[6], c2[6], q3[6];
-  Fr i4, two_over_d, inv_d2;
+  TCombArgs k;
 };
 __global__ void __launch_bounds__(kT)
 k_t_combine(const Fr* __restrict__ V, size_t n, T3Args a, Fr* __restrict__ t) {
@@ -651,10 +645,11 @@
     v1 = v1 - a.c1[k];
     v2 = v2 - a.c2[k];
   }
-  const Fr sm = v0 + v2, dl = v0 - v2, im = dl * a.i4, v12 = v1 + v1;
-  t[k] = sm + v12 - im;
-  t[n + k] = dl * a.two_over_d;
-  t[2 * n + k] = (sm - v12 + im) * a.inv_d2;
+  Fr o0, o1, o2;
+  t_combine_elem(a.k, v0, v1, v2, o0, o1, o2);
+  t[k] = o0;
+  t[n + k] = o1;
+  t[2 * n + k] = o2;
   if (k < 6) t[3 * n + k] = a.q3[k];
 }
 
@@ -688,27 +683,28 @@
   Fr x[kEvalMax];
   Fr x4096[kEvalMax];
   F29 x29[kEvalMax];
-  F29 y29[kEvalMax];
   int np;
   int nbits;
 };
 
-__device__ __forceinline__ F29 fr29_operand_dev(Fr c) {
-#pragma unroll
-  for (int k = 0; k < 5; k++) c = c + c;
-  return split29(c);
-}
-
 static constexpr int kEvalChunk2 = 16;
+static_assert(kEvalChunk2 == kEvalTerms, "eval_terms29 takes a thread's kEvalChunk2 coefficients");
+static constexpr size_t kEvalYpow = (size_t)kEvalMax * kT;
+static constexpr size_t kEvalPw = kEvalYpow + (size_t)kEvalMax * kEvalChunk2;
 
 __global__ void __launch_bounds__(kT) k_eval_pows(EvalSet es, F29* __restrict__ pw, Fr* __restrict__ pw2) {
   const int j = blockIdx.x, t = threadIdx.x;
-  Fr a = Fr::one(), q = es.x[j];
-  for (int e = t; e; e >>= 1) {
-    if (e & 1) a = a * q;
-    q = q * q;
-  }
-  pw[(size_t)j * kT + t] = fr29_operand_dev(a);
+  const Fr xj = es.x[j];
+  auto x_pow = [xj](int e) {
+    Fr a = Fr::one(), q = xj;
+    for (; e; e >>= 1) {
+      if (e & 1) a = a * q;
+      q = q * q;
+    }
+    return fr29_operand(a);
+  };
+  pw[(size_t)j * kT + t] = x_pow(t);
+  if (t < kEvalChunk2) pw[kEvalYpow + j * kEvalChunk2 + t] = x_pow(kT * t);
   if (t < es.nbits) {
     Fr z = es.x4096[j];
     for (int k = 0; k < t; k++) z = z * z;
@@ -744,24 +740,17 @@
     if (j < NP && k == 0) bpow[j] = f;
   }
   const size_t s = (size_t)blockIdx.x * kT * kEvalChunk2 + threadIdx.x;
-  F29 acc[NP];
-#pragma unroll
-  for (int j = 0; j < NP; j++)
-#pragma unroll
-    for (int l = 0; l < 9; l++) acc[j].v[l] = 0;
-  for (int m = kEvalChunk2 - 1; m >= 0; m--) {
-    const size_t i = s + (size_t)m * kT;
-#pragma unroll
-    for (int j = 0; j < NP; j++)
-      if (i < es.len[j]) {
-        const F29 t = mul29<Fr29>(acc[j], es.y29[j]), c = split29(es.p[j][i]);
-#pragma unroll
-        for (int l = 0; l < 9; l++) acc[j].v[l] = t.v[l] + c.v[l];
-      }
-  }
-#pragma unroll
   for (int j = 0; j < NP; j++) {
-    const Fr r = block_sum_fr(join_fr29(mul29<Fr29>(acc[j], pw[(size_t)j * kT + threadIdx.x])), sh);
+    const uint64_t len = es.len[j];
+    const Fr* __restrict__ p = es.p[j];
+    const int nterms = s < len ? (int)min((uint64_t)kEvalChunk2, (len - s + kT - 1) / kT) : 0;
+    const F29 acc = eval_terms29(
+        [&](int m) {
+          const size_t i = s + (size_t)m * kT;
+          return i < len ? split29(p[i]) : f29_zero();
+        },
+        pw + kEvalYpow + j * kEvalChunk2, nterms);
+    const Fr r = block_sum_fr(join_fr29(mul29<Fr29>(acc, pw[(size_t)j * kT + threadIdx.x])), sh);
     if (threadIdx.x == 0) bsum[j] = r;
   }
   if (threadIdx.x < NP) partial[(size_t)threadIdx.x * nblocks + blockIdx.x] = bsum[threadIdx.x] * bpow[threadIdx.x];
@@ -783,35 +772,32 @@
   Fr coefz, coef_ab, ea, eb, ec, coefs3;
 };
 
-__global__ void k_pol_r(const Fr* __restrict__ pz, const Fr* __restrict__ qm, const Fr* __restrict__ ql,
-                        const Fr* __restrict__ qr, const Fr* __restrict__ qo, const Fr* __restrict__ qc,
-                        const Fr* __restrict__ s3, size_t n, RArgs r, Fr* __restrict__ out) {
+__global__ void __launch_bounds__(kT)
+k_pol_r(const Fr* __restrict__ pz, const Fr* __restrict__ qm, const Fr* __restrict__ ql, const Fr* __restrict__ qr,
+        const Fr* __restrict__ qo, const Fr* __restrict__ qc, const Fr* __restrict__ s3, size_t n, PolRArgs r,
+        Fr* __restrict__ out) {
   size_t i = (size_t)blockIdx.x * blockDim.x + threadIdx.x;
   if (i >= n + 3) return;
-  Fr v = r.coefz * pz[i];
-  if (i < n) {
-    v = v + r.coef_ab * qm[i] + r.ea * ql[i] + r.eb * qr[i] + r.ec * qo[i] + qc[i];
-    v = v - r.coefs3 * s3[i];
-  }
-  out[i] = v;
+  const Fr z = Fr::zero();
+  const bool in = i < n;
+  out[i] = pol_r_elem(r, pz[i], in ? qm[i] : z, in ? ql[i] : z, in ? qr[i] : z, in ? qo[i] : z, in ? qc[i] : z,
+                      in ? s3[i] : z);
 }
 
 struct WArgs {
   Fr xim, xi2m, v[7], w0sub;
 };
 
-__global__ void k_pol_wxi(const Fr* __restrict__ t, const Fr* __restrict__ pr, const Fr* __restrict__ pa,
-                          const Fr* __restrict__ pb, const Fr* __restrict__ pc, const Fr* __restrict__ s1,
-                          const Fr* __restrict__ s2, size_t n, WArgs wa, Fr* __restrict__ out) {
+__global__ void __launch_bounds__(kT)
+k_pol_wxi(const Fr* __restrict__ t, const Fr* __restrict__ pr, const Fr* __restrict__ pa, const Fr* __restrict__ pb,
+          const Fr* __restrict__ pc, const Fr* __restrict__ s1, const Fr* __restrict__ s2, size_t n, PolWxiArgs wa,
+          Fr* __restrict__ out) {
   size_t i = (size_t)blockIdx.x * blockDim.x + threadIdx.x;
   if (i >= n + 6) return;
-  Fr w = wa.xi2m * t[2 * n + i];
-  if (i < n) w = w + wa.xim * t[n + i] + t[i];
-  if (i < n + 3) w = w + wa.v[1] * pr[i];
-  if (i < n + 2) w = w + wa.v[2] * pa[i] + wa.v[3] * pb[i] + wa.v[4] * pc[i];
-  if (i < n) w = w + wa.v[5] * s1[i] + wa.v[6] * s2[i];
-  if (i == 0) w = w - wa.w0sub;
-  out[i] = w;
+  const Fr z = Fr::zero();
+  const bool in = i < n, in2 = i < n + 2, in3 = i < n + 3;
+  out[i] = pol_wxi_elem(wa, t[2 * n + i], in ? t[n + i] : z, in ? t[i] : z, in3 ? pr[i] : z, in2 ? pa[i] : z,
+                        in2 ? pb[i] : z, in2 ? pc[i] : z, in ? s1[i] : z, in ? s2[i] : z, i == 0);
 }
 
 __global__ void k_div_check(const Fr* __restrict__ src, Fr p0_adjust, const Fr* __restrict__ q, Fr d,
@@ -989,7 +975,6 @@
     es.len[j] = lens[j];
     es.x[j] = xs[j];
     es.x29[j] = fr29_operand(xs[j]);
-    es.y29[j] = fr29_operand(pow_u64(xs[j], kT));
     es.x4096[j] = pow_u64(xs[j], (uint64_t)kT * kEvalChunk2);
     maxlen = std::max(maxlen, lens[j]);
   }
@@ -1045,6 +1030,32 @@
   hipLaunchKernelGGL(k_lin_tile<true>, dim3((unsigned)ntiles), dim3(kT), 0, s, src, m, lt, (const Fr*)heads, dst);
   hipLaunchKernelGGL(k_div_check, dim3(1), dim3(64), 0, s, src, p0_adjust, (const Fr*)dst, d, flags, flag_bit,
                      mb_flags);
+  NZ_HIP(hipGetLastError());
+}
+
+static void gate_h_launch(const Fr* A, const Fr* B, const Fr* C, const Fr* qh, size_t n, uint32_t npub,
+                          uint32_t* flags, hipStream_t s) {
+  hipLaunchKernelGGL(k_gate_h, dim3(grid_for(n, kT, 1u << 30)), dim3(kT), 0, s, A, B, C, qh, n, npub, flags);
+  NZ_HIP(hipGetLastError());
+}
+
+static void t_combine_launch(const Fr* V, size_t n, T3Args& ta, const Fr& i4, const Fr& two_over_d, const Fr& inv_d2,
+                             Fr* t, hipStream_t s) {
+  ta.k = t_combine_args(i4, two_over_d, inv_d2);
+  hipLaunchKernelGGL(k_t_combine, dim3(grid_for(n, kT, 1u << 30)), dim3(kT), 0, s, V, n, ta, t);
+  NZ_HIP(hipGetLastError());
+}
+
+static void pol_r_launch(const Fr* pz, const Fr* qm, const Fr* ql, const Fr* qr, const Fr* qo, const Fr* qc,
+                         const Fr* s3, size_t n, const RArgs& r, Fr* out, hipStream_t s) {
+  hipLaunchKernelGGL(k_pol_r, dim3(grid_for(n + 3, kT, 1u << 30)), dim3(kT), 0, s, pz, qm, ql, qr, qo, qc, s3, n,
+                     pol_r_args(r.coefz, r.coef_ab, r.ea, r.eb, r.ec, r.coefs3), out);
+  NZ_HIP(hipGetLastError());
+}
+static void pol_wxi_launch(const Fr* t, const Fr* pr, const Fr* pa, const Fr* pb, const Fr* pc, const Fr* s1,
+                           const Fr* s2, size_t n, const WArgs& w, Fr* out, hipStream_t s) {
+  hipLaunchKernelGGL(k_pol_wxi, dim3(grid_for(n + 6, kT, 1u << 30)), dim3(kT), 0, s, t, pr, pa, pb, pc, s1, s2, n,
+                     pol_wxi_args(w.xim, w.xi2m, w.v, w.w0sub), out);
   NZ_HIP(hipGetLastError());
 }
 
@@ -1400,7 +1411,8 @@
   lin_host.resize(2 * sizeof(LinTab) / sizeof(Fr));
   size_t nblocks = ((size_t)3 * n + 6 + (size_t)kT * kEvalChunk2 - 1) / ((size_t)kT * kEvalChunk2) + 1;
   eval_part.alloc((size_t)kEvalMax * nblocks + kEvalMax);
-  eval_pw.alloc((size_t)kEvalMax * kT + (kEvalMax * kEvalBits * sizeof(Fr) + sizeof(F29) - 1) / sizeof(F29));
+  static_assert(kEvalPw * sizeof(F29) % alignof(Fr) == 0, "the Fr table starts aligned");
+  eval_pw.alloc(kEvalPw + (kEvalMax * kEvalBits * sizeof(Fr) + sizeof(F29) - 1) / sizeof(F29));
   host_part.resize(std::max<size_t>(nblocks, kEvalMax));
   flags.p = (uint32_t*)(blind.p + 12);
   flags.n = 1;
@@ -1455,9 +1467,7 @@
 }
 
 void Prover::launch_gate_check(hipStream_t s) {
-  hipLaunchKernelGGL(k_gate_h, dim3(grid_for(n, kT, 1u << 30)), dim3(kT), 0, s, A.p, B.p, C.p, q_h.p, (size_t)n,
-                     nPublic, flags.p);
-  NZ_HIP(hipGetLastError());
+  gate_h_launch(A.p, B.p, C.p, q_h.p, (size_t)n, nPublic, flags.p, s);
 }
 
 void Prover::copy_tops(hipStream_t s) {
@@ -1523,11 +1533,7 @@
     ta.c1[k] = neg(i4 * c);
     ta.c2[k] = neg(c);
   }
-  ta.i4 = i4;
-  ta.two_over_d = fr_small(2) * inverse(D);
-  ta.inv_d2 = inverse(D * D);
-  hipLaunchKernelGGL(k_t_combine, dim3(grid_for(n, kT, 1u << 30)), dim3(kT), 0, s, Tz.p, (size_t)n, ta, t.p);
-  NZ_HIP(hipGetLastError());
+  t_combine_launch(Tz.p, (size_t)n, ta, i4, fr_small(2) * inverse(D), inverse(D * D), t.p, s);
 }
 
 void Prover::to4t(const Fr* evals, Fr* coefs, Fr* evals4, const int* bidx, int nb, hipStream_t s) {
@@ -1770,7 +1776,7 @@
   size_t nblocks = 0;
   const EvalSet es = eval_set(np, polys, lens, xs, &nblocks);
   if ((size_t)np * nblocks + kEvalMax > eval_part.n) throw Error(NZCB_ERR_INTERNAL, "eval partial buffer too small");
-  eval_launch(es, nblocks, eval_part.p, eval_pw.p, (Fr*)(eval_pw.p + (size_t)kEvalMax * kT),
+  eval_launch(es, nblocks, eval_part.p, eval_pw.p, (Fr*)(eval_pw.p + kEvalPw),
               top_host + kMbEvals, s);
   if (overlap) overlap();
   NZ_HIP(hipStreamSynchronize(s));
@@ -2078,9 +2084,7 @@
     Fr eval_l1 = (xim - Fr::one()) * inverse((xi - Fr::one()) * fr_small(n));
     Fr e4 = eval_l1 * (alpha * alpha);
     RArgs ra{e2 + e4, coef_ab, ea, eb, ec, e3};
-    hipLaunchKernelGGL(k_pol_r, dim3(grid_for(n + 3, kT, 1u << 30)), dim3(kT), 0, s, pol_z.p, qm.p, ql.p, qr.p,
-                       qo.p, qc.p, sigma.p + 10 * (size_t)n, (size_t)n, ra, pol_r.p);
-    NZ_HIP(hipGetLastError());
+    pol_r_launch(pol_z.p, qm.p, ql.p, qr.p, qo.p, qc.p, sigma.p + 10 * (size_t)n, (size_t)n, ra, pol_r.p, s);
     {
       const Fr* polys[1] = {pol_r.p};
       const size_t lens[1] = {n + 3};
@@ -2114,9 +2118,7 @@
     wa.xim = xim;
     wa.xi2m = xim * xim;
     wa.w0sub = et + wa.v[1] * er + wa.v[2] * ea + wa.v[3] * eb + wa.v[4] * ec + wa.v[5] * es1 + wa.v[6] * es2;
-    hipLaunchKernelGGL(k_pol_wxi, dim3(grid_for(n + 6, kT, 1u << 30)), dim3(kT), 0, s, t.p, pol_r.p, pol_a.p,
-                       pol_b.p, pol_c.p, sigma.p, sigma.p + 5 * (size_t)n, (size_t)n, wa, T.p);
-    NZ_HIP(hipGetLastError());
+    pol_wxi_launch(t.p, pol_r.p, pol_a.p, pol_b.p, pol_c.p, sigma.p, sigma.p + 5 * (size_t)n, (size_t)n, wa, T.p, s);
     div_pol1(T.p, n + 6, 0, Fr::zero(), pol_wxi.p, 4u);
     lg("multiexp Wxi");
     commit_start(0, pol_wxi.p, n + 6);
@@ -2263,7 +2265,7 @@
   size_t nblocks = 0;
   const EvalSet es = eval_set(np, dp, lens, xv, &nblocks);
   Fr* part = cs.alloc<Fr>((size_t)np * nblocks * sizeof(Fr));
-  F29* pw = cs.alloc<F29>((size_t)kEvalMax * kT * sizeof(F29));
+  F29* pw = cs.alloc<F29>(kEvalPw * sizeof(F29));
   Fr* pw2 = cs.alloc<Fr>((size_t)kEvalMax * kEvalBits * sizeof(Fr));
   eval_launch(es, nblocks, part, pw, pw2, mail.p, cs.st);
   NZ_HIP(hipStreamSynchronize(cs.st));
@@ -2311,6 +2313,100 @@
   }
 }
 
+void need_n(size_t n, const char* what) {
+  if (n < 1 || n > kDebugMax) throw Error(NZCB_ERR_ARG, std::string(what) + ": n outside 1..2^26");
+}
+
+void debug_pol_r(int device, const uint8_t* pz, const uint8_t* q, const uint8_t* s3, size_t n, const uint8_t* consts,
+                 uint8_t* out) {
+  if (!pz || !q || !s3 || !consts || !out) throw Error(NZCB_ERR_ARG, "pol_r: null argument");
+  need_n(n, "pol_r");
+  need_canonical(pz, n + 3, "pol_r: pz");
+  need_canonical(q, 5 * n, "pol_r: q");
+  need_canonical(s3, n, "pol_r: s3");
+  need_canonical(consts, 6, "pol_r: consts");
+  Fr k[6];
+  std::memcpy(k, consts, sizeof(k));
+  const RArgs ra{k[0], k[1], k[2], k[3], k[4], k[5]};
+  CallScope cs(device, nullptr, 0);
+  const Fr* dz = upload(cs, pz, n + 3);
+  const Fr* dq = upload(cs, q, 5 * n);
+  const Fr* ds = upload(cs, s3, n);
+  Fr* dout = cs.alloc<Fr>((n + 3) * sizeof(Fr));
+  pol_r_launch(dz, dq, dq + n, dq + 2 * n, dq + 3 * n, dq + 4 * n, ds, n, ra, dout, cs.st);
+  NZ_HIP(hipMemcpyAsync(out, dout, (n + 3) * sizeof(Fr), hipMemcpyDeviceToHost, cs.st));
+  NZ_HIP(hipStreamSynchronize(cs.st));
+}
+
+void debug_pol_wxi(int device, const uint8_t* t, const uint8_t* pr, const uint8_t* abc, const uint8_t* s12, size_t n,
+                   const uint8_t* consts, uint8_t* out) {
+  if (!t || !pr || !abc || !s12 || !consts || !out) throw Error(NZCB_ERR_ARG, "pol_wxi: null argument");
+  need_n(n, "pol_wxi");
+  need_canonical(t, 3 * n + 6, "pol_wxi: t");
+  need_canonical(pr, n + 3, "pol_wxi: r");
+  need_canonical(abc, 3 * (n + 2), "pol_wxi: abc");
+  need_canonical(s12, 2 * n, "pol_wxi: s12");
+  need_canonical(consts, 9, "pol_wxi: consts");
+  Fr k[9];
+  std::memcpy(k, consts, sizeof(k));
+  WArgs wa;
+  wa.xim = k[0];
+  wa.xi2m = k[1];
+  wa.v[0] = Fr::zero();
+  for (int i = 1; i <= 6; i++) wa.v[i] = k[1 + i];
+  wa.w0sub = k[8];
+  CallScope cs(device, nullptr, 0);
+  const Fr* dt = upload(cs, t, 3 * n + 6);
+  const Fr* dr = upload(cs, pr, n + 3);
+  const Fr* dabc = upload(cs, abc, 3 * (n + 2));
+  const Fr* ds = upload(cs, s12, 2 * n);
+  Fr* dout = cs.alloc<Fr>((n + 6) * sizeof(Fr));
+  pol_wxi_launch(dt, dr, dabc, dabc + (n + 2), dabc + 2 * (n + 2), ds, ds + n, n, wa, dout, cs.st);
+  NZ_HIP(hipMemcpyAsync(out, dout, (n + 6) * sizeof(Fr), hipMemcpyDeviceToHost, cs.st));
+  NZ_HIP(hipStreamSynchronize(cs.st));
+}
+
+void debug_t_combine(int device, const uint8_t* v, size_t n, const uint8_t* corr, const uint8_t* consts,
+                     uint8_t* t_out) {
+  if (!v || !corr || !consts || !t_out) throw Error(NZCB_ERR_ARG, "t_combine: null argument");
+  need_n(n, "t_combine");
+  need_canonical(v, 3 * n, "t_combine: v");
+  need_canonical(corr, 24, "t_combine: corr");
+  need_canonical(consts, 3, "t_combine: consts");
+  T3Args ta;
+  std::memcpy(ta.c0, corr, sizeof(ta.c0));
+  std::memcpy(ta.c1, corr + 6 * 32, sizeof(ta.c1));
+  std::memcpy(ta.c2, corr + 12 * 32, sizeof(ta.c2));
+  std::memcpy(ta.q3, corr + 18 * 32, sizeof(ta.q3));
+  Fr k[3];
+  std::memcpy(k, consts, sizeof(k));
+  CallScope cs(device, nullptr, 0);
+  const Fr* dv = upload(cs, v, 3 * n);
+  Fr* dt = cs.alloc<Fr>((3 * n + 6) * sizeof(Fr));
+  NZ_HIP(hipMemsetAsync(dt, 0, (3 * n + 6) * sizeof(Fr), cs.st));
+  t_combine_launch(dv, n, ta, k[0], k[1], k[2], dt, cs.st);
+  NZ_HIP(hipMemcpyAsync(t_out, dt, (3 * n + 6) * sizeof(Fr), hipMemcpyDeviceToHost, cs.st));
+  NZ_HIP(hipStreamSynchronize(cs.st));
+}
+
+void debug_gate_h(int device, const uint8_t* abc, const uint8_t* qh, size_t n, uint32_t npub, int* violated_out) {
+  if (!abc || !qh || !violated_out) throw Error(NZCB_ERR_ARG, "gate_h: null argument");
+  need_n(n, "gate_h");
+  if (npub > n) throw Error(NZCB_ERR_ARG, "gate_h: more public rows than rows");
+  need_canonical(abc, 3 * n, "gate_h: abc");
+  need_canonical(qh, 5 * n, "gate_h: qh");
+  CallScope cs(device, nullptr, 0);
+  const Fr* dabc = upload(cs, abc, 3 * n);
+  const Fr* dq = upload(cs, qh, 5 * n);
+  uint32_t* flags = cs.alloc<uint32_t>(sizeof(uint32_t));
+  uint32_t host_flags = 0;
+  NZ_HIP(hipMemsetAsync(flags, 0, sizeof(uint32_t), cs.st));
+  gate_h_launch(dabc, dabc + n, dabc + 2 * n, dq, n, npub, flags, cs.st);
+  NZ_HIP(hipMemcpyAsync(&host_flags, flags, sizeof(uint32_t), hipMemcpyDeviceToHost, cs.st));
+  NZ_HIP(hipStreamSynchronize(cs.st));
+  *violated_out = (host_flags & 1u) ? 1 : 0;
+}
+
 }
 
 }
@@ -2341,3 +2437,23 @@
     debug_quotient(device, power, three, npub, abcz, q, s, l, apub, beta, gamma, alpha, k1, k2, t_out);
   });
 }
+
+extern "C" int nzcb_debug_pol_r(int device, const uint8_t* pz, const uint8_t* q, const uint8_t* s3, size_t n,
+                                const uint8_t* consts, uint8_t* out, nzcb_err* err) {
+  return guarded(err, [&] { debug_pol_r(device, pz, q, s3, n, consts, out); });
+}
+
+extern "C" int nzcb_debug_pol_wxi(int device, const uint8_t* t, const uint8_t* r, const uint8_t* abc,
+                                  const uint8_t* s12, size_t n, const uint8_t* consts, uint8_t* out, nzcb_err* err) {
+  return guarded(err, [&] { debug_pol_wxi(device, t, r, abc, s12, n, consts, out); });
+}
+
+extern "C" int nzcb_debug_t_combine(int device, const uint8_t* v, size_t n, const uint8_t* corr, const uint8_t* consts,
+                                    uint8_t* t_out, nzcb_err* err) {
+  return guarded(err, [&] { debug_t_combine(device, v, n, corr, consts, t_out); });
+}
+
+extern "C" int nzcb_debug_gate_h(int device, const uint8_t* abc, const uint8_t* qh, size_t n, uint32_t npub,
+                                 int* violated_out, nzcb_err* err) {
+  return guarded(err, [&] { debug_gate_h(device, abc, qh, n, npub, violated_out); });
+}
diff --git a/nzcb-circom_amd/nzcb/__init__.py b/nzcb-circom_amd/nzcb/__init__.py
--- a/nzcb-circom_amd/nzcb/__init__.py
+++ b/nzcb-circom_amd/nzcb/__init__.py
@@ -52,6 +52,7 @@
     "nzcb_debug_groth16_schedule", "nzcb_debug_groth16_timings",
     "nzcb_debug_signal_basis_cap", "nzcb_debug_signal_basis_info", "nzcb_debug_commit_abc", "nzcb_debug_signal_rows",
     "nzcb_debug_grand_product", "nzcb_debug_div_pol1", "nzcb_debug_eval_many", "nzcb_debug_quotient",
+    "nzcb_debug_pol_r", "nzcb_debug_pol_wxi", "nzcb_debug_t_combine", "nzcb_debug_gate_h",
 ]
 
 NZCB_FAULT_QUOTIENT = 1
@@ -147,6 +148,39 @@
     _check(load().nzcb_debug_quotient(device, power, int(three), npub, abcz, q, s, l, apub, beta, gamma, alpha, k1, k2,
                                       out, ctypes.byref(err)), err)
     return bytes(out)[:32 * pts]
+
+
+def debug_pol_r(pz: bytes, q: bytes, s3: bytes, consts: bytes, device: int = 0) -> bytes:
+    n = len(s3) // 32
+    assert len(s3) == 32 * n and len(pz) == 32 * (n + 3) and len(q) == 160 * n and len(consts) == 192
+    out, err = _out(32 * (n + 3)), _Err()
+    _check(load().nzcb_debug_pol_r(device, pz, q, s3, n, consts, out, ctypes.byref(err)), err)
+    return bytes(out)[:32 * (n + 3)]
+
+
+def debug_pol_wxi(t: bytes, r: bytes, abc: bytes, s12: bytes, consts: bytes, device: int = 0) -> bytes:
+    n = len(s12) // 64
+    assert len(s12) == 64 * n and len(t) == 32 * (3 * n + 6) and len(r) == 32 * (n + 3)
+    assert len(abc) == 96 * (n + 2) and len(consts) == 288
+    out, err = _out(32 * (n + 6)), _Err()
+    _check(load().nzcb_debug_pol_wxi(device, t, r, abc, s12, n, consts, out, ctypes.byref(err)), err)
+    return bytes(out)[:32 * (n + 6)]
+
+
+def debug_t_combine(v: bytes, corr: bytes, consts: bytes, device: int = 0) -> bytes:
+    n = len(v) // 96
+    assert len(v) == 96 * n and len(corr) == 32 * 24 and len(consts) == 96
+    out, err = _out(32 * (3 * n + 6)), _Err()
+    _check(load().nzcb_debug_t_combine(device, v, n, corr, consts, out, ctypes.byref(err)), err)
+    return bytes(out)[:32 * (3 * n + 6)]
+
+
+def debug_gate_h(abc: bytes, qh: bytes, npub: int, device: int = 0) -> bool:
+    n = len(abc) // 96
+    assert len(abc) == 96 * n and len(qh) == 160 * n
+    bad, err = c_int(-1), _Err()
+    _check(load().nzcb_debug_gate_h(device, abc, qh, n, npub, ctypes.byref(bad), ctypes.byref(err)), err)
+    return bool(bad.value)
 
 
 def guard_selftest(device: int = 0) -> None:
@@ -389,6 +423,14 @@
                                         ctypes.c_char_p, ctypes.c_char_p, ctypes.c_char_p, ctypes.c_char_p,
                                         ctypes.c_char_p, ctypes.c_char_p, ctypes.c_char_p, ctypes.c_char_p, u8p,
                                         POINTER(_Err)]),
+        "nzcb_debug_pol_r": (c_int, [c_int, ctypes.c_char_p, ctypes.c_char_p, ctypes.c_char_p, c_size_t,
+                                     ctypes.c_char_p, u8p, POINTER(_Err)]),
+        "nzcb_debug_pol_wxi": (c_int, [c_int, ctypes.c_char_p, ctypes.c_char_p, ctypes.c_char_p, ctypes.c_char_p,
+                                       c_size_t, ctypes.c_char_p, u8p, POINTER(_Err)]),
+        "nzcb_debug_t_combine": (c_int, [c_int, ctypes.c_char_p, c_size_t, ctypes.c_char_p, ctypes.c_char_p, u8p,
+                                         POINTER(_Err)]),
+        "nzcb_debug_gate_h": (c_int, [c_int, ctypes.c_char_p, ctypes.c_char_p, c_size_t, c_uint32, POINTER(c_int),
+                                      POINTER(_Err)]),
     }
     lib.missing_symbols = []
     for name, (res, args) in sigs.items():
```
